# npit/video-learning-tf

Measured on AMD Instinct MI355X. Metric: clips/sec (16-frame 227x227) LRCN train step, higher is better.
Workload: dtype f32; 1 GPU; LRCN AlexNet(fc6)+LSTM(256) 16-frame 227x227x3 clips, 101 classes, UCF-101-shaped synthetic, full train step; global_batch=64, clips_per_gpu=64, frames_per_clip=16, parallelism=dp1, optimizer=sgd+clip_by_global_norm(10), init=reference (sigma 0.05), dist_world_size=1

## Files before the change

### include/vltf.h

```cpp
#ifndef VLTF_H
#define VLTF_H

#include <stddef.h>
#include <stdint.h>

#ifdef __cplusplus
extern "C" {
#endif

typedef void* vl_stream_t;
typedef struct vl_conv_desc vl_conv_desc;

typedef struct vl_step_state {
    int64_t step;
    float lr;
    uint32_t tag_origin;
    float adam_lr;
    uint32_t reserved[3];
} vl_step_state;

const char* vl_last_error(void);
int vl_version(void);
int vl_device_count(void);

int vl_input_prep_u8(const uint8_t* src, float* dst, int n, int raw_h, int raw_w, int out_h, int out_w,
                     const int32_t* crop_y, const int32_t* crop_x, const uint8_t* mirror,
                     const float* mean_bgr, int dst_halo, int dst_phase, vl_stream_t stream);
int vl_nhwc_to_nchw(const float* src, float* dst, int n, int h, int w, int c, int dst_halo, int dst_phase, vl_stream_t stream);
int vl_nchw_to_nhwc(const float* src, float* dst, int n, int c, int h, int w, vl_stream_t stream);

int vl_conv_create(vl_conv_desc** out, int cin, int h, int w, int cout, int kh, int kw, int stride, int groups);
void vl_conv_destroy(vl_conv_desc* d);
int vl_conv_out_hw(const vl_conv_desc* d, int* oh, int* ow);
int vl_conv_set_halo(vl_conv_desc* d, int x_halo, int y_halo, int dy_halo, int dx_halo);
int vl_conv_set_x_phase_split(vl_conv_desc* d, int on);
int vl_conv_x_phase(const vl_conv_desc* d);
int vl_set_conv_math(int math);
int vl_conv_math(void);
int vl_conv_fwd(const vl_conv_desc* d, const float* x, const float* w_hwio, const float* bias, float* y,
                int n, int relu, vl_stream_t stream);
int vl_conv_wt_transpose(const vl_conv_desc* d, const float* w_hwio, float* wt, vl_stream_t stream);
int vl_conv_dgrad(const vl_conv_desc* d, const float* dy, const float* wt, float* dx, const float* relu_mask,
                  int n, vl_stream_t stream);
size_t vl_conv_wgrad_ws_bytes(const vl_conv_desc* d, int n);
int vl_conv_wgrad_fuses_bias(const vl_conv_desc* d);
int vl_conv_wgrad(const vl_conv_desc* d, const float* x, const float* dy, float* dw, float* db, void* ws,
                  size_t ws_bytes, int n, vl_stream_t stream);
size_t vl_c8_bytes(int n, int c, int h, int w, int halo);
int vl_pack_c8(const float* x, void* xb, int n, int c, int h, int w, int x_halo, int xb_halo, vl_stream_t stream);
size_t vl_conv_c8_w_bytes(const vl_conv_desc* d, int bwd);
int vl_conv_c8_pack_w(const vl_conv_desc* d, const float* w_hwio, void* wb, int bwd, vl_stream_t stream);
int vl_conv_c8_fwd(vl_conv_desc* d, const void* xb, const void* wb, const float* bias, float* y, void* yb, int n, int relu,
                   vl_stream_t stream);
int vl_conv_c8_dgrad(vl_conv_desc* d, const void* dyb, const void* wbt, float* dx, void* dxb, const float* relu_mask,
                     const void* relu_mask_c8, int n, vl_stream_t stream);
size_t vl_conv_c8_wgrad_ws_bytes(const vl_conv_desc* d, int n);
int vl_conv_c8_wgrad(vl_conv_desc* d, const void* xb, const void* dyb, float* dw, void* ws, size_t ws_bytes, int n,
                     vl_stream_t stream);
int vl_bias_grad_c8(const void* dyb, float* db, float* ws, int n, int c, int h, int w, int halo, vl_stream_t stream);
int vl_pack_kc8(const float* src, void* dst, int64_t positions, int channels, int64_t pos_stride, int64_t ch_stride, vl_stream_t stream);
size_t vl_gemm_kc8_ws_bytes(int m, int n, int k);
int vl_gemm_kc8(const void* a_kc8, const void* b_kc8, float* c, int m, int n, int k, const float* bias, int relu, void* ws,
                size_t ws_bytes, vl_stream_t stream);
int vl_s2d_c8_from_x0(const vl_conv_desc* d, const float* x0, void* xb, int n, vl_stream_t stream);
int vl_input_prep_u8_s2d(const vl_conv_desc* d, const uint8_t* src, void* xb, int n, int raw_h, int raw_w, const int32_t* crop_y,
                         const int32_t* crop_x, const uint8_t* mirror, const float* mean_bgr, vl_stream_t stream);
int vl_s2d_weights(const vl_conv_desc* d, const float* src, float* dst, int grad, vl_stream_t stream);
int vl_bias_grad_nchw(const float* dy, float* db, float* ws, int n, int c, int hw, vl_stream_t stream);

int vl_lrn_fwd(const float* x, float* y, int n, int c, int hw, int radius, float alpha, float beta, float bias,
               vl_stream_t stream);
int vl_lrn_bwd(const float* x, const float* dy, float* dx, int n, int c, int hw, int radius, float alpha,
               float beta, float bias, int relu_fused, int w, int dx_halo, vl_stream_t stream);

int vl_pool_lrn_bwd(const float* x, const float* dp, const uint8_t* argmax, float* dx, int n, int c, int h, int w,
                    int p_halo, int radius, float alpha, float beta, float bias, int relu_fused, int dx_halo,
                    vl_stream_t stream);

int vl_pool_lrn_bwd_c8(const void* x, int x_packed, const float* dp, const uint8_t* argmax, void* dxb, int n, int c, int h, int w,
                       int p_halo, int radius, float alpha, float beta, float bias, int relu_fused, int dxb_halo, vl_stream_t stream);

int vl_pool_lrn_bwd_test_ranges(int ranges);

int vl_lrn_pool_fwd(const float* x, float* p, uint8_t* argmax, int n, int c, int h, int w, int p_halo, int radius,
                    float alpha, float beta, float bias, vl_stream_t stream);

int vl_lrn_pool_fwd_c8(const void* x, int x_packed, void* pb, uint8_t* argmax, int n, int c, int h, int w, int p_halo, int radius,
                       float alpha, float beta, float bias, vl_stream_t stream);

int vl_maxpool_fwd(const float* x, float* y, uint8_t* argmax, int n, int c, int h, int w, int k, int s,
                   int64_t ys_n, int64_t ys_c, int64_t ys_h, int64_t ys_w, vl_stream_t stream);
int vl_maxpool_bwd(const float* dy, const uint8_t* argmax, float* dx, const float* relu_mask, int n, int c,
                   int h, int w, int k, int s, int64_t ys_n, int64_t ys_c, int64_t ys_h, int64_t ys_w,
                   int dx_halo, vl_stream_t stream);

int vl_gemm(int transa, int transb, int m, int n, int k, const float* a, int64_t lda, const float* b, int64_t ldb,
            float* c, int64_t ldc, const float* bias, int relu, const float* relu_mask, void* ws, size_t ws_bytes,
            vl_stream_t stream);
size_t vl_gemm_split_ws_bytes(int m, int n, int k);
int vl_colsum(const float* a, int64_t lda, float* out, float* ws, int m, int n, vl_stream_t stream);

int vl_lstm_step_fwd(const float* gx, const float* gh, float* act, float* cseq, float* hseq, float* hprev,
                     int batch, int T, int t, int H, float forget_bias, vl_stream_t stream);
int vl_lstm_step_bwd(const float* dout, const float* dh_next, const float* act, const float* cseq, float* dc,
                     float* dz, int batch, int T, int t, int H, vl_stream_t stream);

size_t vl_lstm_seq_ws_bytes(int batch, int T, int H);
int vl_lstm_seq_fwd(const float* gx, const float* kh, const float* h0, const float* c0, float* act, float* cseq, float* hseq,
                    float* hprev, int batch, int T, int H, float forget_bias, void* ws, size_t ws_bytes, vl_stream_t stream);
int vl_lstm_seq_bwd(const float* dout, const float* kh, const float* act, const float* cseq, const float* c0, float* dz,
                    float* dh0, float* dc0, int batch, int T, int H, void* ws, size_t ws_bytes, vl_stream_t stream);
int vl_lstm_seq_fwd_len(const float* gx, const float* kh, const float* h0, const float* c0, float* act, float* cseq, float* hseq,
                        float* hprev, int batch, int T, int H, float forget_bias, const int32_t* seq_len, void* ws, size_t ws_bytes,
                        vl_stream_t stream);
int vl_lstm_seq_bwd_len(const float* dout, const float* kh, const float* act, const float* cseq, const float* c0, float* dz,
                        float* dh0, float* dc0, int batch, int T, int H, const int32_t* seq_len, void* ws, size_t ws_bytes,
                        vl_stream_t stream);
size_t vl_lstm_seq_tag_span(int batch, int T, int H);
int vl_lstm_seq_fwd_st(const float* gx, const float* kh, const float* h0, const float* c0, float* act, float* cseq, float* hseq,
                       float* hprev, int batch, int T, int H, float forget_bias, void* ws, size_t ws_bytes, const vl_step_state* state,
                       uint32_t tag_offset, vl_stream_t stream);
int vl_lstm_seq_bwd_st(const float* dout, const float* kh, const float* act, const float* cseq, const float* c0, float* dz,
                       float* dh0, float* dc0, int batch, int T, int H, void* ws, size_t ws_bytes, const vl_step_state* state,
                       uint32_t tag_offset, vl_stream_t stream);
int vl_lstm_seq_ws_clear(void* ws, size_t ws_bytes, vl_stream_t stream);
int vl_lstm_seq_status(void* ws, int* timed_out);
int vl_lstm_seq_test_hooks(unsigned spin_limit, int mute_workgroup);
int vl_transpose(const float* src, int64_t ld, float* dst, int rows, int cols, vl_stream_t stream);

int vl_temporal_fusion_fwd(const float* x, float* y, int batch, int T, int H, int method, vl_stream_t stream);
int vl_temporal_fusion_bwd(const float* dy, float* dx, int batch, int T, int H, int method, vl_stream_t stream);
int vl_temporal_fusion_fwd_len(const float* x, float* y, int batch, int T, int H, int method, const int32_t* seq_len,
                               vl_stream_t stream);
int vl_temporal_fusion_bwd_len(const float* dy, float* dx, int batch, int T, int H, int method, const int32_t* seq_len,
                               vl_stream_t stream);

typedef struct vl_resize_desc vl_resize_desc;
int vl_resize_create(vl_resize_desc** out, int h, int w, int oh, int ow, int channels);
void vl_resize_destroy(vl_resize_desc* d);
size_t vl_resize_tmp_bytes(const vl_resize_desc* d, int n);
int vl_resize_u8(const vl_resize_desc* d, const uint8_t* src, uint8_t* tmp, uint8_t* dst, int n, vl_stream_t stream);

int vl_copy2d(const float* src, int64_t src_ld, float* dst, int64_t dst_ld, int rows, int cols, vl_stream_t stream);
int vl_eltwise2(const float* a, const float* b, float* out, int64_t count, int op, vl_stream_t stream);
int vl_max2_grad(const float* a, const float* b, const float* d, float* da, float* db, int64_t count, vl_stream_t stream);
int vl_fuse_n(const float* const* ins, int n, float* out, int64_t count, int op, vl_stream_t stream);
int vl_fuse_n_grad(const float* const* ins, int n, const float* d, float* const* dins, int64_t count, int op, vl_stream_t stream);

int vl_dropout_fwd(const float* x, float* y, uint8_t* mask, int64_t count, float keep, uint64_t seed, vl_stream_t stream);
int vl_dropout_bwd(const float* dy, const uint8_t* mask, float* dx, int64_t count, float keep, vl_stream_t stream);
int vl_dropout_fwd_st(const float* x, float* y, uint8_t* mask, int64_t count, float keep, const vl_step_state* state,
                      vl_stream_t stream);

int vl_softmax_xent(const float* logits, const int32_t* labels, float* dlogits, float* stats, float* rows,
                    int batch, int classes, float grad_scale, vl_stream_t stream);
int vl_softmax_xent_len(const float* logits, const int32_t* labels, float* dlogits, float* stats, float* rows,
                        int batch, int classes, float grad_scale, const int32_t* seq_len, int T, vl_stream_t stream);

int vl_sumsq(const float* g, int64_t count, float* out, float* ws, int accumulate, vl_stream_t stream);
int vl_sgd_apply(float* w, const float* g, int64_t count, float lr, float clip_norm, const float* sumsq,
                 float gscale, const uint32_t* skip, vl_stream_t stream);
int vl_adam_apply(float* w, const float* g, float* m, float* v, int64_t count, float lr, float clip_norm,
                  const float* sumsq, float gscale, int step, const uint32_t* skip, vl_stream_t stream);
int vl_status_or(uint32_t* dst, const void* lstm_ws, int init, vl_stream_t stream);

size_t vl_step_state_bytes(void);
int vl_step_state_set(vl_step_state* state, int64_t step, float lr, uint32_t tag_origin, vl_stream_t stream);
int vl_sgd_apply_st(float* w, const float* g, int64_t count, const vl_step_state* state, float clip_norm, const float* sumsq,
                    float gscale, const uint32_t* skip, vl_stream_t stream);
int vl_adam_apply_st(float* w, const float* g, float* m, float* v, int64_t count, const vl_step_state* state, float clip_norm,
                     const float* sumsq, float gscale, const uint32_t* skip, vl_stream_t stream);

int vl_fill(float* p, int64_t count, float value, vl_stream_t stream);
int vl_relu_grad(float* d, const float* y, int64_t count, vl_stream_t stream);

#ifdef __cplusplus
}
#endif
#endif
```

### video-learning-tf_amd/_ffi.py

```python
import ctypes as C
import os

_HERE = os.path.dirname(os.path.abspath(__file__))
LIB_PATH = os.environ.get("VLTF_HIP_LIB") or os.path.join(_HERE, "libvltf_hip.so")

p = C.c_void_p
i32, i64, f32, u32, u64, sz = C.c_int, C.c_int64, C.c_float, C.c_uint32, C.c_uint64, C.c_size_t

SIGNATURES = {
    "vl_last_error": (C.c_char_p, []),
    "vl_version": (i32, []),
    "vl_device_count": (i32, []),
    "vl_input_prep_u8": (i32, [p, p, i32, i32, i32, i32, i32, p, p, p, p, i32, i32, p]),
    "vl_nhwc_to_nchw": (i32, [p, p, i32, i32, i32, i32, i32, i32, p]),
    "vl_nchw_to_nhwc": (i32, [p, p, i32, i32, i32, i32, p]),
    "vl_conv_create": (i32, [C.POINTER(p), i32, i32, i32, i32, i32, i32, i32, i32]),
    "vl_conv_destroy": (None, [p]),
    "vl_conv_out_hw": (i32, [p, C.POINTER(i32), C.POINTER(i32)]),
    "vl_conv_set_halo": (i32, [p, i32, i32, i32, i32]),
    "vl_conv_set_x_phase_split": (i32, [p, i32]),
    "vl_conv_x_phase": (i32, [p]),
    "vl_set_conv_math": (i32, [i32]),
    "vl_conv_math": (i32, []),
    "vl_gemm_split_ws_bytes": (C.c_size_t, [i32, i32, i32]),
    "vl_conv_fwd": (i32, [p, p, p, p, p, i32, i32, p]),
    "vl_conv_wt_transpose": (i32, [p, p, p, p]),
    "vl_conv_dgrad": (i32, [p, p, p, p, p, i32, p]),
    "vl_conv_wgrad_ws_bytes": (sz, [p, i32]),
    "vl_conv_wgrad_fuses_bias": (i32, [p]),
    "vl_conv_wgrad": (i32, [p, p, p, p, p, p, sz, i32, p]),
    "vl_c8_bytes": (sz, [i32, i32, i32, i32, i32]),
    "vl_pack_c8": (i32, [p, p, i32, i32, i32, i32, i32, i32, p]),
    "vl_conv_c8_w_bytes": (sz, [p, i32]),
    "vl_conv_c8_pack_w": (i32, [p, p, p, i32, p]),
    "vl_conv_c8_fwd": (i32, [p, p, p, p, p, p, i32, i32, p]),
    "vl_conv_c8_dgrad": (i32, [p, p, p, p, p, p, p, i32, p]),
    "vl_pack_kc8": (i32, [p, p, i64, i32, i64, i64, p]),
    "vl_gemm_kc8_ws_bytes": (sz, [i32, i32, i32]),
    "vl_gemm_kc8": (i32, [p, p, p, i32, i32, i32, p, i32, p, sz, p]),
    "vl_s2d_c8_from_x0": (i32, [p, p, p, i32, p]),
    "vl_input_prep_u8_s2d": (i32, [p, p, p, i32, i32, i32, p, p, p, p, p]),
    "vl_s2d_weights": (i32, [p, p, p, i32, p]),
    "vl_bias_grad_c8": (i32, [p, p, p, i32, i32, i32, i32, i32, p]),
    "vl_conv_c8_wgrad_ws_bytes": (sz, [p, i32]),
    "vl_conv_c8_wgrad": (i32, [p, p, p, p, p, sz, i32, p]),
    "vl_bias_grad_nchw": (i32, [p, p, p, i32, i32, i32, p]),
    "vl_lrn_fwd": (i32, [p, p, i32, i32, i32, i32, f32, f32, f32, p]),
    "vl_lrn_bwd": (i32, [p, p, p, i32, i32, i32, i32, f32, f32, f32, i32, i32, i32, p]),
    "vl_lrn_pool_fwd": (i32, [p, p, p, i32, i32, i32, i32, i32, i32, f32, f32, f32, p]),
    "vl_pool_lrn_bwd": (i32, [p, p, p, p, i32, i32, i32, i32, i32, i32, f32, f32, f32, i32, i32, p]),
    "vl_pool_lrn_bwd_test_ranges": (i32, [i32]),
    "vl_lrn_pool_fwd_c8": (i32, [p, i32, p, p, i32, i32, i32, i32, i32, i32, f32, f32, f32, p]),
    "vl_pool_lrn_bwd_c8": (i32, [p, i32, p, p, p, i32, i32, i32, i32, i32, i32, f32, f32, f32, i32, i32, p]),
    "vl_maxpool_fwd": (i32, [p, p, p, i32, i32, i32, i32, i32, i32, i64, i64, i64, i64, p]),
    "vl_maxpool_bwd": (i32, [p, p, p, p, i32, i32, i32, i32, i32, i32, i64, i64, i64, i64, i32, p]),
    "vl_gemm": (i32, [i32, i32, i32, i32, i32, p, i64, p, i64, p, i64, p, i32, p, p, sz, p]),
    "vl_colsum": (i32, [p, i64, p, p, i32, i32, p]),
    "vl_lstm_step_fwd": (i32, [p, p, p, p, p, p, i32, i32, i32, i32, f32, p]),
    "vl_lstm_step_bwd": (i32, [p, p, p, p, p, p, i32, i32, i32, i32, p]),
    "vl_lstm_seq_ws_bytes": (sz, [i32, i32, i32]),
    "vl_lstm_seq_fwd": (i32, [p, p, p, p, p, p, p, p, i32, i32, i32, f32, p, sz, p]),
    "vl_lstm_seq_bwd": (i32, [p, p, p, p, p, p, p, p, i32, i32, i32, p, sz, p]),
    "vl_lstm_seq_fwd_len": (i32, [p, p, p, p, p, p, p, p, i32, i32, i32, f32, p, p, sz, p]),
    "vl_lstm_seq_bwd_len": (i32, [p, p, p, p, p, p, p, p, i32, i32, i32, p, p, sz, p]),
    "vl_lstm_seq_tag_span": (sz, [i32, i32, i32]),
    "vl_lstm_seq_fwd_st": (i32, [p, p, p, p, p, p, p, p, i32, i32, i32, f32, p, sz, p, u32, p]),
    "vl_lstm_seq_bwd_st": (i32, [p, p, p, p, p, p, p, p, i32, i32, i32, p, sz, p, u32, p]),
    "vl_lstm_seq_ws_clear": (i32, [p, sz, p]),
    "vl_lstm_seq_status": (i32, [p, C.POINTER(i32)]),
    "vl_lstm_seq_test_hooks": (i32, [C.c_uint, i32]),
    "vl_transpose": (i32, [p, i64, p, i32, i32, p]),
    "vl_temporal_fusion_fwd": (i32, [p, p, i32, i32, i32, i32, p]),
    "vl_temporal_fusion_bwd": (i32, [p, p, i32, i32, i32, i32, p]),
    "vl_temporal_fusion_fwd_len": (i32, [p, p, i32, i32, i32, i32, p, p]),
    "vl_temporal_fusion_bwd_len": (i32, [p, p, i32, i32, i32, i32, p, p]),
    "vl_dropout_fwd": (i32, [p, p, p, i64, f32, u64, p]),
    "vl_dropout_bwd": (i32, [p, p, p, i64, f32, p]),
    "vl_dropout_fwd_st": (i32, [p, p, p, i64, f32, p, p]),
    "vl_softmax_xent": (i32, [p, p, p, p, p, i32, i32, f32, p]),
    "vl_softmax_xent_len": (i32, [p, p, p, p, p, i32, i32, f32, p, i32, p]),
    "vl_sumsq": (i32, [p, i64, p, p, i32, p]),
    "vl_sgd_apply": (i32, [p, p, i64, f32, f32, p, f32, p, p]),
    "vl_adam_apply": (i32, [p, p, p, p, i64, f32, f32, p, f32, i32, p, p]),
    "vl_status_or": (i32, [p, p, i32, p]),
    "vl_step_state_bytes": (sz, []),
    "vl_step_state_set": (i32, [p, i64, f32, u32, p]),
    "vl_sgd_apply_st": (i32, [p, p, i64, p, f32, p, f32, p, p]),
    "vl_adam_apply_st": (i32, [p, p, p, p, i64, p, f32, p, f32, p, p]),
    "vl_fill": (i32, [p, i64, f32, p]),
    "vl_resize_create": (i32, [C.POINTER(p), i32, i32, i32, i32, i32]),
    "vl_resize_destroy": (None, [p]),
    "vl_resize_tmp_bytes": (sz, [p, i32]),
    "vl_resize_u8": (i32, [p, p, p, p, i32, p]),
    "vl_copy2d": (i32, [p, i64, p, i64, i32, i32, p]),
    "vl_eltwise2": (i32, [p, p, p, i64, i32, p]),
    "vl_max2_grad": (i32, [p, p, p, p, p, i64, p]),
    "vl_fuse_n": (i32, [p, i32, p, i64, i32, p]),
    "vl_fuse_n_grad": (i32, [p, i32, p, p, i64, i32, p]),
    "vl_relu_grad": (i32, [p, p, i64, p]),
}


class VltfError(RuntimeError):
    pass


_lib = None


def lib():
    global _lib
    if _lib is None:
        if not os.path.exists(LIB_PATH):
            raise VltfError("libvltf_hip.so not found at %s -- build it with "
                            "`python -c 'import __graft_entry__ as g; g.build()'` "
                            "(there is no CPU fallback)" % LIB_PATH)
        import torch
        tl = os.path.join(os.path.dirname(torch.__file__), "lib", "libamdhip64.so")
        if os.path.exists(tl):
            C.CDLL(tl, mode=C.RTLD_GLOBAL)
        try:
            l = C.CDLL(LIB_PATH)
        except OSError as ex:
            raise VltfError("cannot load %s: %s" % (LIB_PATH, ex))
        for name, (res, args) in SIGNATURES.items():
            try:
                fn = getattr(l, name)
            except AttributeError:
                raise VltfError("libvltf_hip.so does not export %s (stale build?)" % name)
            fn.restype = res
            fn.argtypes = args
        _lib = l
    return _lib


def check(rc, what):
    if rc != 0:
        msg = lib().vl_last_error()
        raise VltfError("%s failed (rc=%d): %s" % (what, rc, msg.decode() if msg else "?"))


def call(name, *args):
    check(getattr(lib(), name)(*args), name)
```

### video-learning-tf_amd/csrc/conv_desc.h

```cpp
#pragma once
#include <hip/hip_runtime.h>
#include <stdint.h>

struct vl_conv_desc {
    int cin, h, w, cout, kh, kw, stride, groups;
    int oh, ow, pt, pl, pb, pr;
    int cig, cog;
    int K;
    int Kd;
    int x_halo, y_halo, dy_halo, dx_halo;
    int x_phase;
    int2* ktab2_fwd;
    int* ktab_fwd;
    int2* ptab2_fwd;
    int2* ptab2_bwd;
    int* ptab_fwd;
    int* ptab_bwd;
    int* rowtab_fwd;
    int* rowtab_bwd;
    int fwd_padded, bwd_padded;
    uint32_t* wsplit_fwd;
    uint32_t* wsplit_bwd;
    int* c8_toff_fwd;
    int* c8_toff_bwd;
};

void conv_c8_free_tables(vl_conv_desc* d);
int conv_c8_build_tables(vl_conv_desc* d);
```

### video-learning-tf_amd/csrc/mfma_gemm.hip

```cpp
#include <stdlib.h>
#include <string.h>

#include "common.h"
#include "conv_desc.h"

typedef float f32x16 __attribute__((ext_vector_type(16)));
typedef const __attribute__((address_space(4))) int* const_int_ptr;
__device__ __forceinline__ const_int_ptr as_const(const int* p) { return (const_int_ptr)(uintptr_t)p; }
static constexpr int NT = 256;
static constexpr int KBLK = 16;

static constexpr uint32_t OOB_OFF = 0xF0000000u;
static constexpr int64_t MAX_BUF_BYTES = 0xE0000000ll;

__device__ __forceinline__ __amdgpu_buffer_rsrc_t make_rsrc(const float* base, int64_t bytes) {
    return __builtin_amdgcn_make_buffer_rsrc(const_cast<float*>(base), 0, (int)(uint32_t)bytes, 0x00020000);
}
__device__ __forceinline__ float buf_load(__amdgpu_buffer_rsrc_t r, uint32_t voff, int soff) {
    return __builtin_bit_cast(float, __builtin_amdgcn_raw_buffer_load_b32(r, (int)voff, soff, 0));
}

template <int BX, int BR>
struct LdsTile {
    static constexpr int STR = BR + 2;
// ... 567 lines not shown
    i32x4 p[3];
};
template <int NPC>
__device__ __forceinline__ void split_pieces(float x0, float x1, int (&out)[3]) {
    f32x2 r = {x0, x1};
#pragma unroll
    for (int k = 0; k < NPC; ++k) {
        const uint32_t h = __builtin_bit_cast(uint32_t, __builtin_convertvector(r, bf16x2));
        out[k] = (int)h;
        if (k + 1 < NPC) r = f32x2{r[0] - __uint_as_float(h << 16), r[1] - __uint_as_float(h & 0xffff0000u)};
    }
}
__device__ constexpr int kProdA[6] = {0, 0, 1, 1, 0, 2};
__device__ constexpr int kProdB[6] = {0, 1, 0, 1, 2, 0};
constexpr int split_products(int math) { return math == 6 ? 6 : math == 3 ? 3 : 1; }
constexpr int split_pieces_of(int math) { return math == 6 ? 3 : math == 3 ? 2 : 1; }
__device__ __forceinline__ f32x16 mfma_bf16(const i32x4& a, const i32x4& b, const f32x16& c) {
    return __builtin_amdgcn_mfma_f32_32x32x16_bf16(__builtin_bit_cast(bf16x8, a), __builtin_bit_cast(bf16x8, b), c, 0, 0, 0);
}

template <int BN, int WM, int WN, int MATH = 0, bool X4 = false>
__global__ __launch_bounds__(NT, 1) void wgrad_dma_kernel(const ConvGeom g, const DyParams d, const EpiRowMajor::Params pe,
                                                          int tiles_i, int tiles_j, int groups, int units, int rtiles,
                                                          int rt_per_split, float* db_slabs, int db_stride) {
    using C = WgradDmaCfg<BN>;
    constexpr int BM = C::BM, STR = C::STR, SA = BM * STR, BUF = C::BUF;
    constexpr int TM = BM / WM / 32, TN = BN / WN / 32;
    constexpr int RA = BM / 4, RB = BN / 4;
    static_assert(WM * WN == 4 && TM * WM * 32 == BM && TN * WN * 32 == BN, "tile shape");
    static_assert(RA + RB <= 10 * 2 * TM * TN, "row fetches must leave the last third of a tile's MFMAs to cover their latency");
    static_assert(!X4 || (MATH != 0 && BN == 128 && BM == 128), "the 16-byte fetch form: split-product modes, 128 x 128 tiles");
    constexpr int GSTR = 258, SA4 = 32 * GSTR, BUF4 = 64 * GSTR;
    extern __shared__ __attribute__((aligned(16))) float ldsw[];

    const int tiles = tiles_i * tiles_j;
    const int k8 = blockIdx.x >> 3;
    const int unit = (k8 / tiles) * 8 + (blockIdx.x & 7);
    if (unit >= units) return;
    const int tile_id = k8 % tiles;
    const int ti_blk = tile_id % tiles_i, tj_blk = tile_id / tiles_i;
    const int zg = unit % groups, zs = unit / groups;
    const int i0 = ti_blk * BM, j0 = tj_blk * BN;
    const int lane = threadIdx.x & 63;
    const int wave = __builtin_amdgcn_readfirstlane(threadIdx.x >> 6);
    const int wi0 = (wave / WN) * (BM / WM), wj0 = (wave % WN) * (BN / WN);

    const i32x4 rs_x = rsrc_words(g.x + (int64_t)zg * g.grp_stride, (g.total - (int64_t)zg * g.grp_stride) * 4);
    const int64_t goff = (int64_t)zg * d.Cog * d.plane;
    const i32x4 rs_dy = rsrc_words(d.dy + goff, (d.total - goff) * 4);
    const int* tab = g.ktab + i0 + wave * RA;
    const uint32_t lds0 = (uint32_t)(uintptr_t)(__attribute__((address_space(3))) float*)ldsw;
    const int row_bytes = (int)(d.plane * 4);
    const int b_row0 = j0 + wave * RB;
    const int b_last = d.Cog - 1;
    const int64_t dy_img = (int64_t)d.Cout_total * d.plane;

    uint32_t voff_x, voff_dy;
    auto decode = [&](int rt) __attribute__((always_inline)) {
        const int m = X4 ? rt * 64 + 4 * (lane & 15) : rt * 64 + lane;
        const bool vm = m < g.M;
        const uint32_t mm = vm ? m : 0;
        const uint32_t n = fd_div(mm, g.dOHW);
        const uint32_t p = mm - n * g.OHW;
        const uint32_t oh = fd_div(p, g.dOW);
        const uint32_t ow = p - oh * g.OW;
        const int ih0 = (int)oh * g.stride - g.pt + g.halo, iw0 = (int)ow * g.col_mul + g.col_add;
        const uint32_t vx = (uint32_t)((int64_t)n * g.img_stride + (int64_t)ih0 * g.Wp + iw0) * 4u;
        const uint32_t vd = (uint32_t)((int64_t)n * dy_img + (int64_t)(oh + d.halo) * d.OWp + ow + d.halo) * 4u;
        voff_x = vm ? vx : OOB_OFF;
        voff_dy = vm ? vd : OOB_OFF;
        asm volatile("" : "+v"(voff_x), "+v"(voff_dy));
    };
    int tabv[RA];
    auto load_table = [&](int rt) __attribute__((always_inline)) {
        const const_int_ptr tt = (const_int_ptr)(uintptr_t)(tab + rt * g.zero);
#pragma unroll
        for (int f = 0; f < RA; ++f) tabv[f] = tt[f];
    };
    auto pin_table = [&]() __attribute__((always_inline)) {
#pragma unroll
        for (int f = 0; f < RA; ++f) asm volatile("" : "+s"(tabv[f]));
    };
    auto dma = [&](const int nb, const int f, int rt_next) __attribute__((always_inline)) {
        const int z = rt_next * g.zero;
        if (f < RA) {
            const uint32_t la = lds0 + (uint32_t)(wave * (RA * STR) + z) * 4u;
            lds_dma_row(rs_x, la + (uint32_t)(nb * BUF + f * STR) * 4u, voff_x, tabv[f]);
        } else {
            const int r = f - RA;
            const uint32_t lb = lds0 + (uint32_t)(SA + wave * (RB * STR) + z) * 4u;
            lds_dma_row(rs_dy, lb + (uint32_t)(nb * BUF + r * STR) * 4u, voff_dy, min(b_row0 + z + r, b_last) * row_bytes);
        }
    };
    uint32_t vrow_a[8], vrow_b[8];
    if constexpr (X4) {
#pragma unroll
        for (int j = 0; j < 8; ++j) {
            const int rl = wave * 8 + j + 32 * (lane >> 4);
            vrow_a[j] = i0 + rl < g.K ? (uint32_t)g.ktab[i0 + rl] : OOB_OFF;
            vrow_b[j] = j0 + rl < d.Cog ? (uint32_t)(j0 + rl) * (uint32_t)row_bytes : OOB_OFF;
        }
    }
    auto dma_x4 = [&](const int nb, const int f, int rt_next) __attribute__((always_inline)) {
        const int z = rt_next * g.zero;
        if (f < 8) {
            const uint32_t vo = (vrow_a[f] == OOB_OFF || voff_x == OOB_OFF) ? OOB_OFF : vrow_a[f] + voff_x;
            lds_dma_row4(rs_x, lds0 + (uint32_t)(nb * BUF4 + (wave * 8 + f) * GSTR + z) * 4u, vo, 0);
        } else {
            const uint32_t vo = (vrow_b[f - 8] == OOB_OFF || voff_dy == OOB_OFF) ? OOB_OFF : vrow_b[f - 8] + voff_dy;
            lds_dma_row4(rs_dy, lds0 + (uint32_t)(nb * BUF4 + SA4 + (wave * 8 + f - 8) * GSTR + z) * 4u, vo, 0);
        }
    };
    const int ones_row = (db_slabs != nullptr && g.K >= i0 && g.K < i0 + BM) ? g.K - i0 : -1;
    auto finish_tile = [&](const int nb) __attribute__((always_inline)) {
        asm volatile("s_waitcnt vmcnt(0)" ::: "memory");
        if constexpr (X4) {
            if (ones_row >= 0 && ((ones_row & 31) >> 3) == wave) ldsw[nb * BUF4 + (ones_row & 31) * GSTR + (ones_row >> 5) * 64 + lane] = 1.0f;
        } else {
            if (ones_row >= 0 && (ones_row / RA) == wave) ldsw[nb * BUF + ones_row * STR + lane] = 1.0f;
        }
        __syncthreads();
    };

    f32x16 acc[TM][TN];
#pragma unroll
    for (int a = 0; a < TM; ++a)
#pragma unroll
        for (int b = 0; b < TN; ++b)
#pragma unroll
            for (int q = 0; q < 16; ++q) acc[a][b][q] = 0.f;

    const int rt0 = zs * rt_per_split;
    const int rt1 = min(rtiles, rt0 + rt_per_split);
    const int ntiles = rt1 - rt0;
    if (ntiles > 0) {
        decode(rt0);
        load_table(rt0);
        pin_table();
        if constexpr (X4) {
#pragma unroll
            for (int f = 0; f < 16; ++f) dma_x4(0, f, rt0);
        } else {
#pragma unroll
            for (int f = 0; f < RA + RB; ++f) dma(0, f, rt0);
        }
        decode(rt0 + 1);
        finish_tile(0);
    }
    const float* fa = ldsw + (wi0 + (lane & 31)) * STR + 2 * (lane >> 5);
    const float* fb = ldsw + SA + (wj0 + (lane & 31)) * STR + 2 * (lane >> 5);

    auto tile = [&](const int cur, int rt_next) __attribute__((always_inline)) {
        float2 af[2][TM], bf[2][TN];
#pragma unroll
        for (int a = 0; a < TM; ++a) af[0][a] = *reinterpret_cast<const float2*>(fa + cur * BUF + a * 32 * STR);
#pragma unroll
        for (int b = 0; b < TN; ++b) bf[0][b] = *reinterpret_cast<const float2*>(fb + cur * BUF + b * 32 * STR);
#pragma unroll
        for (int t = 0; t < 16; ++t) {
            const int c = t & 1, nx = c ^ 1;
            if (t + 1 < 16) {
#pragma unroll
                for (int a = 0; a < TM; ++a) af[nx][a] = *reinterpret_cast<const float2*>(fa + cur * BUF + a * 32 * STR + 4 * (t + 1));
#pragma unroll
                for (int b = 0; b < TN; ++b) bf[nx][b] = *reinterpret_cast<const float2*>(fb + cur * BUF + b * 32 * STR + 4 * (t + 1));
            }
#pragma unroll
            for (int m = 0; m < 2 * TM * TN; ++m) {
                const int a = (m % (TM * TN)) / TN, b = m % TN;
                if (m < TM * TN) acc[a][b] = __builtin_amdgcn_mfma_f32_32x32x2f32(af[c][a].x, bf[c][b].x, acc[a][b], 0, 0, 0);
                else acc[a][b] = __builtin_amdgcn_mfma_f32_32x32x2f32(af[c][a].y, bf[c][b].y, acc[a][b], 0, 0, 0);
                const int f = t * (2 * TM * TN) + m;
                if (f < RA + RB) {
                    dma(cur ^ 1, f, rt_next);
                    __builtin_amdgcn_sched_barrier(0);
                }
            }
            if (t == 10) {
                load_table(rt_next + 1);
                __builtin_amdgcn_sched_barrier(0);
            }
            if (t == 13) {
                int rtn = rt_next + 1;
                asm volatile("" : "+s"(rtn));
                decode(rtn);
                pin_table();
                __builtin_amdgcn_sched_barrier(0);
            }
        }
        finish_tile(cur ^ 1);
    };
    const float* fa3 = ldsw + (wi0 + (lane & 31)) * STR + 8 * (lane >> 5);
    const float* fb3 = ldsw + SA + (wj0 + (lane & 31)) * STR + 8 * (lane >> 5);
    auto tile_split = [&](const int cur, int rt_next) __attribute__((always_inline)) {
        constexpr int NP = split_products(MATH), NPC = split_pieces_of(MATH);
        constexpr int NMS = NP * TM * TN, NTOT = 4 * NMS, NF = X4 ? 16 : RA + RB;
        constexpr int FSPAN = NTOT >= 28 ? NTOT - 14 : NTOT / 2;
        constexpr int FPM = (NF + FSPAN - 1) / FSPAN, FEND = (NF + FPM - 1) / FPM;
        constexpr int LT = FEND > NTOT - 12 ? FEND : NTOT - 12;
        constexpr int PIN = LT + 2 > NTOT - 6 ? LT + 2 : NTOT - 6;
        static_assert(PIN < NTOT, "the tile must leave room to load and pin the next table");
        SplitBf16 As[2][TM], Bs[2][TN];
        auto load_split = [&](const int st, SplitBf16 (&A)[TM], SplitBf16 (&B)[TN]) __attribute__((always_inline)) {
#pragma unroll
            for (int a = 0; a < TM; ++a)
#pragma unroll
                for (int q = 0; q < 4; ++q) {
                    const float2 v = X4 ? *reinterpret_cast<const float2*>(ldsw + cur * BUF4 + (lane & 31) * GSTR + (wi0 / 32 + a) * 64 + 16 * st +
                                                                            8 * (lane >> 5) + 2 * q)
                                        : *reinterpret_cast<const float2*>(fa3 + cur * BUF + a * 32 * STR + 16 * st + 2 * q);
                    int pc[3] = {0, 0, 0};
                    split_pieces<NPC>(v.x, v.y, pc);
#pragma unroll
                    for (int k = 0; k < NPC; ++k) A[a].p[k][q] = pc[k];
                }
#pragma unroll
            for (int b = 0; b < TN; ++b)
#pragma unroll
                for (int q = 0; q < 4; ++q) {
                    const float2 v = X4 ? *reinterpret_cast<const float2*>(ldsw + cur * BUF4 + SA4 + (lane & 31) * GSTR + (wj0 / 32 + b) * 64 +
                                                                            16 * st + 8 * (lane >> 5) + 2 * q)
                                        : *reinterpret_cast<const float2*>(fb3 + cur * BUF + b * 32 * STR + 16 * st + 2 * q);
                    int pc[3] = {0, 0, 0};
                    split_pieces<NPC>(v.x, v.y, pc);
#pragma unroll
                    for (int k = 0; k < NPC; ++k) B[b].p[k][q] = pc[k];
                }
        };
        load_split(0, As[0], Bs[0]);
        static_for<0, 4>([&](auto SI) __attribute__((always_inline)) {
            constexpr int st = decltype(SI)::value, c = st & 1;
            if constexpr (st + 1 < 4) load_split(st + 1, As[c ^ 1], Bs[c ^ 1]);
            static_for<0, NMS>([&](auto MI) __attribute__((always_inline)) {
                constexpr int m = decltype(MI)::value;
                constexpr int prod = m / (TM * TN), a = (m % (TM * TN)) / TN, b = m % TN;
                acc[a][b] = mfma_bf16(As[c][a].p[kProdA[prod]], Bs[c][b].p[kProdB[prod]], acc[a][b]);
                constexpr int idx = st * NMS + m;
                static_for<0, FPM>([&](auto EI) __attribute__((always_inline)) {
                    constexpr int f = idx * FPM + decltype(EI)::value;
                    if constexpr (f < NF) {
                        if constexpr (X4) dma_x4(cur ^ 1, f, rt_next);
                        else dma(cur ^ 1, f, rt_next);
                    }
                });
                __builtin_amdgcn_sched_barrier(0x106);
                if constexpr (idx == LT) load_table(rt_next + 1);
                if constexpr (idx == PIN) {
                    int rtn = rt_next + 1;
                    asm volatile("" : "+s"(rtn));
                    decode(rtn);
                    pin_table();
                }
            });
        });
        finish_tile(cur ^ 1);
    };
    auto run_tile = [&](const int cur, int rt_next) __attribute__((always_inline)) {
        if constexpr (MATH != 0) tile_split(cur, rt_next);
        else tile(cur, rt_next);
    };
    int rt = rt0;
    for (int i = 0; i + 1 < ntiles; i += 2, rt += 2) {
        run_tile(0, rt + 1);
        run_tile(1, rt + 2);
    }
    if (ntiles > 0 && (ntiles & 1)) run_tile(0, rt + 1);

    EpiRowMajor::template apply<TM, TN>(pe, zg, zs, i0 + wi0, j0 + wj0, acc);
    if (ones_row >= 0) {
        float* dbs = db_slabs + (int64_t)zs * db_stride + zg * d.Cog;
        const int lr = ones_row - wi0;
        if (lr >= 0 && lr < BM / WM) {
            const int a = lr >> 5, rr = lr & 31;
            const int q = (rr & 3) + 4 * (rr >> 3);
            if (((rr >> 2) & 1) == (lane >> 5)) {
#pragma unroll
                for (int b = 0; b < TN; ++b) {
                    const int j = j0 + wj0 + 32 * b + (lane & 31);
                    float v = 0.f;
#pragma unroll
                    for (int aa = 0; aa < TM; ++aa)
#pragma unroll
                        for (int qq = 0; qq < 16; ++qq)
                            if (aa == a && qq == q) v = acc[aa][b][qq];
                    if (j < d.Cog) dbs[j] = v;
                }
            }
        }
    }
}

typedef float f32x4 __attribute__((ext_vector_type(4)));
typedef float f32x4u __attribute__((ext_vector_type(4), aligned(4)));

struct ConvDmaParams {
    const float* w;
    int64_t w_ld;
    int64_t w_grp_stride;
    int64_t w_bytes;
    const int* row_tab;
    int nblk;
};

template <int SR>
__global__ __launch_bounds__(NT, 64 / SR) void conv_dma_kernel(const ConvDmaParams pa, const ConvGeom g, const EpiConvNCHW::Params pe,
                                                               int tiles_i, int wide) {
    constexpr int BM = 128, BN = 128;
    constexpr int ABUF = SR * BM, BUF = SR * (BM + BN);
    constexpr int RW = SR / 4;
    constexpr int NF = RW * 4;
    constexpr int NT2 = SR / 4;
    constexpr int FPM = 1;
    static_assert(SR == 64 || SR == 32, "stage depth");
    extern __shared__ __attribute__((aligned(16))) float ldsc[];
    const int bid = xcd_swizzle(blockIdx.x, gridDim.x);
    const int ti_blk = bid % tiles_i, tj_blk = bid / tiles_i;
    const int zg = blockIdx.y;
    const int i0 = ti_blk * BM, j0 = tj_blk * BN;
    const int lane = threadIdx.x & 63;
    const int wave = __builtin_amdgcn_readfirstlane(threadIdx.x >> 6);
    const int wm = wave >> 1, wn = wave & 1;

    const i32x4 rs_w = rsrc_words(pa.w + (int64_t)zg * pa.w_grp_stride, pa.w_bytes - (int64_t)zg * pa.w_grp_stride * 4);
    const i32x4 rs_x = rsrc_words(g.x + (int64_t)zg * g.grp_stride, (g.total - (int64_t)zg * g.grp_stride) * 4);
    uint32_t voff_a[2], voff_b[2];
#pragma unroll
    for (int hf = 0; hf < 2; ++hf) {
        const int co = i0 + hf * 64 + lane;
        voff_a[hf] = co < pe.Cog ? (uint32_t)co * 4u : OOB_OFF;
        const int m = j0 + hf * 64 + lane;
        const bool vm = m < g.M;
        const uint32_t mm = vm ? m : 0;
        const uint32_t n = fd_div(mm, g.dOHW);
        const uint32_t p = mm - n * g.OHW;
        const uint32_t oh = fd_div(p, g.dOW);
        const uint32_t ow = p - oh * g.OW;
        const int ih0 = (int)oh * g.stride - g.pt + g.halo, iw0 = (int)ow * g.col_mul + g.col_add;
        voff_b[hf] = vm ? (uint32_t)((int64_t)n * g.img_stride + (int64_t)ih0 * g.Wp + iw0) * 4u : OOB_OFF;
    }
    const uint32_t lds0 = (uint32_t)(uintptr_t)(__attribute__((address_space(3))) float*)ldsc;
    const int ld_bytes = (int)(pa.w_ld * 4);

    int tabv[RW];
    int row0 = 0;
    bool blk_ok = false;
    const int wrow = wave * RW;
    auto load_table = [&](int st) {
        const int k0 = st * SR + wrow;
        const const_int_ptr tt = as_const(g.ktab) + k0 + st * g.zero;
#pragma unroll
        for (int f = 0; f < RW; ++f) tabv[f] = tt[f];
        row0 = as_const(pa.row_tab)[k0 / KBLK + st * g.zero] + k0 % KBLK;
        blk_ok = k0 / KBLK < pa.nblk;
    };
    auto pin_table = [&]() {
#pragma unroll
        for (int f = 0; f < RW; ++f) asm volatile("" : "+s"(tabv[f]));
        asm volatile("" : "+s"(row0));
    };
    auto dma = [&](const int nb, const int f, int st) {
        const int rr = f >> 2, kind = f & 3, hf = kind & 1;
        const int z = st * g.zero;
        const uint32_t row_lds = lds0 + (uint32_t)(nb * BUF + (wrow + rr) * 128 + hf * 64 + z) * 4u;
        const bool live = blk_ok && st * SR + wrow + rr < g.K;
        if (kind < 2) lds_dma_row(rs_w, row_lds, voff_a[hf], min(row0 + rr, g.K - 1) * ld_bytes);
        else lds_dma_row(rs_x, row_lds + ABUF * 4u, live ? voff_b[hf] : OOB_OFF, tabv[rr]);
    };
    int a_soff = 0;
    auto dma_fast = [&](const int nb, const int f, int st) {
        const int rr = f >> 2, kind = f & 3, hf = kind & 1;
        const uint32_t row_lds = lds0 + (uint32_t)(nb * BUF + (wrow + rr) * 128 + hf * 64 + st * g.zero) * 4u;
        if (f == 0) a_soff = row0 * ld_bytes;
        if (kind < 2) lds_dma_row(rs_w, row_lds, voff_a[hf], a_soff);
        else lds_dma_row(rs_x, row_lds + ABUF * 4u, voff_b[hf], tabv[rr]);
        if (kind == 1) a_soff += ld_bytes;
    };
    auto finish_stage = [&]() {
        asm volatile("s_waitcnt vmcnt(0)" ::: "memory");
        __syncthreads();
    };

    f32x16 acc[2][2];
#pragma unroll
    for (int a = 0; a < 2; ++a)
#pragma unroll
        for (int b = 0; b < 2; ++b)
#pragma unroll
            for (int q = 0; q < 16; ++q) acc[a][b][q] = 0.f;

    const int nstages = (pa.nblk * KBLK + SR - 1) / SR;
    load_table(0);
    pin_table();
#pragma unroll
    for (int f = 0; f < NF; ++f) dma(0, f, 0);
    load_table(1);
    pin_table();
    finish_stage();

    float bias_r[2][16];
#pragma unroll
    for (int a = 0; a < 2; ++a)
#pragma unroll
        for (int q = 0; q < 16; ++q) {
            const int co = i0 + wm * 64 + 2 * ((q & 3) + 8 * (q >> 2) + 4 * (lane >> 5)) + a;
            bias_r[a][q] = (pe.bias && co < pe.Cog) ? pe.bias[zg * pe.Cog + co] : 0.f;
        }

    const float* fa = ldsc + (lane >> 5) * 128 + wm * 64 + 2 * (lane & 31);
    const float* fb = ldsc + ABUF + (lane >> 5) * 128 + wn * 64 + (lane & 31);

    auto stage = [&](const int cur, const bool fast, int st_next) {
        float2 af[2], bf[2], an[2], bn[2];
        auto read_b = [&](int step) {
            const float* q = fb + cur * BUF + step * 256;
            return float2{q[0], q[32]};
        };
        af[0] = *reinterpret_cast<const float2*>(fa + cur * BUF);
        bf[0] = read_b(0);
        af[1] = *reinterpret_cast<const float2*>(fa + cur * BUF + 256);
        bf[1] = read_b(1);
#pragma unroll
        for (int t = 0; t < NT2; ++t) {
            if (t + 1 < NT2) {
#pragma unroll
                for (int u = 0; u < 2; ++u) {
                    an[u] = *reinterpret_cast<const float2*>(fa + cur * BUF + (2 * (t + 1) + u) * 256);
                    bn[u] = read_b(2 * (t + 1) + u);
                }
            }
#pragma unroll
            for (int m = 0; m < 8; ++m) {
                const int u = m >> 2, a = (m >> 1) & 1, b = m & 1;
                acc[a][b] = __builtin_amdgcn_mfma_f32_32x32x2f32(a ? af[u].y : af[u].x, b ? bf[u].y : bf[u].x, acc[a][b], 0, 0, 0);
                const int f = (t * 8 + m) * FPM;
                if (f < NF) {
#pragma unroll
                    for (int e = 0; e < FPM; ++e) {
                        if (fast) dma_fast(cur ^ 1, f + e, st_next);
                        else dma(cur ^ 1, f + e, st_next);
                    }
                    __builtin_amdgcn_sched_barrier(0);
                }
            }
            static_assert(NF / FPM / 8 <= NT2 - 4, "fetches must end before the table is replaced");
            if (t == NT2 - 4) {
                load_table(st_next + 1);
                __builtin_amdgcn_sched_barrier(0);
            }
            if (t == NT2 - 2) {
                pin_table();
                __builtin_amdgcn_sched_barrier(0);
            }
#pragma unroll
            for (int u = 0; u < 2; ++u) {
                af[u] = an[u];
                bf[u] = bn[u];
            }
        }
        finish_stage();
    };
    const int nfull = g.K / SR;
    int st = 0;
    for (; st + 2 < nfull; st += 2) {
        stage(0, true, st + 1);
        stage(1, true, st + 2);
    }
    for (; st < nstages; ++st) {
        if (st & 1) stage(1, false, st + 1);
        else stage(0, false, st + 1);
    }

    if (wide) {
        constexpr int SP = BN + 4;
        float* T = ldsc;
#pragma unroll
        for (int b = 0; b < 2; ++b)
#pragma unroll
            for (int a = 0; a < 2; ++a)
#pragma unroll
                for (int q = 0; q < 16; ++q) {
                    const int i = (q & 3) + 8 * (q >> 2) + 4 * (lane >> 5);
                    float v = acc[a][b][q] + bias_r[a][q];
                    if (pe.relu) v = fmaxf(v, 0.f);
                    T[(wm * 64 + 2 * i + a) * SP + wn * 64 + 32 * b + (lane & 31)] = v;
                }
        __syncthreads();
        const int px = 4 * (lane & 31);
        const int m = j0 + px;
        const uint32_t n = fd_div((uint32_t)min(m, pe.M - 1), pe.dOHW);
        const int p = m - (int)n * pe.OHW;
        const bool run4 = m + 3 < pe.M && p + 3 < pe.OHW;
        const int64_t cbase = ((int64_t)n * pe.Cout_total + (int64_t)zg * pe.Cog) * pe.y_plane + p;
#pragma unroll
        for (int i = 0; i < BM / 8; ++i) {
            const int cl = wave * (BM / 4) + 2 * i + (lane >> 5);
            const int co = i0 + cl;
            const f32x4 v = *reinterpret_cast<const f32x4*>(T + cl * SP + px);
            if (co >= pe.Cog) continue;
            float* dst = pe.y + cbase + (int64_t)co * pe.y_plane;
            if (run4) {
                *reinterpret_cast<f32x4u*>(dst) = v;
            } else {
#pragma unroll
                for (int e = 0; e < 4; ++e) {
                    const int me = m + e;
                    if (me < pe.M) {
                        const uint32_t ne = fd_div((uint32_t)me, pe.dOHW);
                        const int pe_ = me - (int)ne * pe.OHW;
                        pe.y[((int64_t)ne * pe.Cout_total + (int64_t)zg * pe.Cog + co) * pe.y_plane + pe_] = v[e];
                    }
                }
            }
        }
        return;
    }
#pragma unroll
    for (int b = 0; b < 2; ++b) {
        const int m = j0 + wn * 64 + 32 * b + (lane & 31);
        if (m >= pe.M) continue;
        const uint32_t n = fd_div((uint32_t)m, pe.dOHW);
        const uint32_t p = m - n * pe.OHW;
        const uint32_t oh = fd_div(p, pe.dOW);
        const uint32_t ow = p - oh * pe.OW;
        const int64_t c0 = (int64_t)n * pe.Cout_total + (int64_t)zg * pe.Cog;
        const int64_t ybase = c0 * pe.y_plane + (int64_t)(oh + pe.y_halo) * pe.y_wp + ow + pe.y_halo;
        const int64_t mbase = c0 * pe.m_plane + (int64_t)(oh + pe.m_halo) * pe.m_wp + ow + pe.m_halo;
#pragma unroll
        for (int a = 0; a < 2; ++a) {
            float mk[16];
            if (pe.mask) {
#pragma unroll
                for (int q = 0; q < 16; ++q) {
                    const int co = i0 + wm * 64 + 2 * ((q & 3) + 8 * (q >> 2) + 4 * (lane >> 5)) + a;
                    mk[q] = co < pe.Cog ? pe.mask[mbase + (int64_t)co * pe.m_plane] : 0.f;
                }
            }
#pragma unroll
            for (int q = 0; q < 16; ++q) {
                const int i = (q & 3) + 8 * (q >> 2) + 4 * (lane >> 5);
                const int co = i0 + wm * 64 + 2 * i + a;
                if (co < pe.Cog) {
                    float v = acc[a][b][q] + bias_r[a][q];
                    if (pe.relu) v = fmaxf(v, 0.f);
                    if (pe.mask) v = mk[q] > 0.f ? v : 0.f;
                    pe.y[ybase + (int64_t)co * pe.y_plane] = v;
                }
            }
        }
    }
}


__global__ void conv_wsplit_kernel(const float* __restrict__ w, int64_t w_ld, int64_t w_grp_stride, const int* __restrict__ row_tab,
                                   int K, int Cog, int CogP, int nstages, int planes, uint32_t* __restrict__ out) {
    const int st = blockIdx.x, zg = blockIdx.y;
    const int row0 = row_tab[st];
    uint32_t* o = out + ((int64_t)zg * nstages + st) * planes * 8 * CogP;
    for (int idx = threadIdx.x; idx < 8 * CogP; idx += blockDim.x) {
        const int q = idx & 3, co = (idx >> 2) % CogP, h = idx / (4 * CogP);
        const int r = 8 * h + 2 * q, p = st * 16 + r;
        float x0 = 0.f, x1 = 0.f;
        if (co < Cog) {
            const float* src = w + (int64_t)(row0 + r) * w_ld + zg * w_grp_stride + co;
            if (p < K) x0 = src[0];
            if (p + 1 < K) x1 = src[w_ld];
        }
        int pc[3] = {0, 0, 0};
        split_pieces<3>(x0, x1, pc);
        for (int k = 0; k < planes; ++k) o[(int64_t)((2 * k + h) * CogP + co) * 4 + q] = (uint32_t)pc[k];
    }
}

struct ConvRingParams {
    const uint32_t* wsplit;
    int CogP;
    int nstages;
};

template <int MATH, int BM>
__global__ __launch_bounds__(512, 1) void conv_ring_kernel(const ConvRingParams pa, const ConvGeom g, const EpiConvNCHW::Params pe,
                                                           int tiles_i, int OWp, int Mp, FastDiv dOHWp, FastDiv dOWp) {
    constexpr int BN = BM == 128 ? 256 : 512, SR = 16, NBUF = BM == 128 ? 5 : 4;
    constexpr int NH = BN / 256;
    static_assert(BM == 128 || BM == 64, "channel tile");
    constexpr int NPL = MATH == 6 ? 3 : 2;
    constexpr int ABUF = NPL * 8 * BM, BUF = ABUF + SR * BN;
    constexpr int NAF = (NPL * 2 * (BM / 64) + 7) / 8;
    constexpr int FW = NAF + 2 * NH;
    constexpr int VMW = (NBUF - 3) * FW;
    constexpr int NP = split_products(MATH), NPC = split_pieces_of(MATH);
    constexpr int NM = (BM / 32) * (BN / 256) * NP;
    static_assert(SR == KBLK, "one stage = one block of the reduction order");
    extern __shared__ __attribute__((aligned(16))) float ldsr[];
    const int bid = xcd_swizzle(blockIdx.x, gridDim.x);
    const int ti_blk = bid % tiles_i, tj_blk = bid / tiles_i;
    const int zg = blockIdx.y;
    const int i0 = ti_blk * BM, j0 = tj_blk * BN;
    const int lane = threadIdx.x & 63;
    const int wave = __builtin_amdgcn_readfirstlane(threadIdx.x >> 6);
    constexpr int TA = BM / 32, TB = BN / 8 / 32, WPX = 32 * TB;
    const int OHWp = g.OHW / g.OW * OWp;
    const int nstages = pa.nstages;

    const int64_t stage_dw = (int64_t)NPL * 8 * pa.CogP;
    const uint32_t* wbase = pa.wsplit + (int64_t)zg * nstages * stage_dw;
    const i32x4 rs_w = rsrc_words(reinterpret_cast<const float*>(wbase), nstages * stage_dw * 4);
    constexpr int NPIECE = NPL * 2 * (BM / 64);
    int piece[NAF];
    uint32_t voff_a[NAF];
#pragma unroll
    for (int e = 0; e < NAF; ++e) {
        piece[e] = e == 0 ? wave % NPIECE : 8 + (wave & 3);
        voff_a[e] = BM == 128 ? (uint32_t)(((piece[e] >> 1) * pa.CogP + i0 + (piece[e] & 1) * 64 + lane) * 16)
                              : (uint32_t)((piece[e] * pa.CogP + i0 + lane) * 16);
    }
    const int stage_bytes = (int)(stage_dw * 4);
    const i32x4 rs_x = rsrc_words(g.x + (int64_t)zg * g.grp_stride, (g.total - (int64_t)zg * g.grp_stride) * 4);
    uint32_t voff_b[NH];
#pragma unroll
    for (int hf = 0; hf < NH; ++hf) {
        const int m = j0 + 256 * hf + 4 * lane;
        const bool vm = m < Mp;
        const uint32_t mm = vm ? m : 0;
        const uint32_t n = fd_div(mm, dOHWp);
        const uint32_t p = mm - n * OHWp;
        const uint32_t oh = fd_div(p, dOWp);
        const uint32_t ow = p - oh * OWp;
        const int ih0 = (int)oh * g.stride - g.pt + g.halo, iw0 = (int)ow * g.col_mul + g.col_add;
        voff_b[hf] = vm ? (uint32_t)((int64_t)n * g.img_stride + (int64_t)ih0 * g.Wp + iw0) * 4u : OOB_OFF;
    }
    const uint32_t lds0 = (uint32_t)(uintptr_t)(__attribute__((address_space(3))) float*)ldsr;

    int tab0 = 0, tab1 = 0;
    const int wrow = wave * 2;
    auto load_table = [&](int st) __attribute__((always_inline)) {
        const int sc = min(st, nstages - 1) + st * g.zero;
        const const_int_ptr tt = as_const(g.ktab) + sc * SR + wrow;
        tab0 = tt[0];
        tab1 = tt[1];
    };
    auto pin_table = [&]() __attribute__((always_inline)) {
        asm volatile("" : "+s"(tab0));
        asm volatile("" : "+s"(tab1));
    };
    auto dma = [&](const uint32_t wr, const int f, int st) __attribute__((always_inline)) {
        if (f < NAF) {
            lds_dma_row4(rs_w, lds0 + wr + (uint32_t)piece[f] * 1024u, voff_a[f], st * stage_bytes);
        } else {
            const int r = (f - NAF) / NH, hf = (f - NAF) % NH;
            const bool live = st * SR + wrow + r < g.K;
            lds_dma_row4(rs_x, lds0 + wr + (uint32_t)(ABUF + (wrow + r) * BN + 256 * hf) * 4u, live ? voff_b[hf] : OOB_OFF,
                         r == 0 ? tab0 : tab1);
        }
    };
    auto dma_fast = [&](const uint32_t wr, const int f, int st) __attribute__((always_inline)) {
        if (f < NAF) {
            lds_dma_row4(rs_w, lds0 + wr + (uint32_t)piece[f] * 1024u, voff_a[f], st * stage_bytes);
        } else {
            const int r = (f - NAF) / NH, hf = (f - NAF) % NH;
            lds_dma_row4(rs_x, lds0 + wr + (uint32_t)(ABUF + (wrow + r) * BN + 256 * hf) * 4u, voff_b[hf], r == 0 ? tab0 : tab1);
        }
    };

    f32x16 acc[TA][TB];
#pragma unroll
    for (int a = 0; a < TA; ++a)
#pragma unroll
        for (int b = 0; b < TB; ++b)
#pragma unroll
            for (int q = 0; q < 16; ++q) acc[a][b][q] = 0.f;

    const float* fa = ldsr + ((lane >> 5) * BM + (lane & 31)) * 4;
    const float* fb = ldsr + ABUF + (lane >> 5) * 8 * BN + wave * WPX + (lane & 31);
    struct Raw {
        float b[TB][8];
    };
    auto load_raw = [&](int rd, Raw& r) __attribute__((always_inline)) {
#pragma unroll
        for (int j = 0; j < 8; ++j) {
            const float* q = fb + rd + j * BN;
#pragma unroll
            for (int b = 0; b < TB; ++b) r.b[b][j] = q[32 * b];
        }
    };
    auto load_a = [&](int rd, SplitBf16 (&A)[TA]) __attribute__((always_inline)) {
#pragma unroll
        for (int a = 0; a < TA; ++a) {
#pragma unroll
            for (int k = 0; k < NPC; ++k) A[a].p[k] = *reinterpret_cast<const i32x4*>(fa + rd + k * 2 * BM * 4 + a * 32 * 4);
        }
    };
    auto split = [&](const Raw& r, SplitBf16 (&B)[TB]) __attribute__((always_inline)) {
#pragma unroll
        for (int j = 0; j < 4; ++j)
#pragma unroll
            for (int b = 0; b < TB; ++b) {
                int pc[3] = {0, 0, 0};
                split_pieces<NPC>(r.b[b][2 * j], r.b[b][2 * j + 1], pc);
#pragma unroll
                for (int k = 0; k < NPC; ++k) B[b].p[k][j] = pc[k];
            }
    };

    for (int s0 = 0; s0 < NBUF; ++s0) {
        load_table(s0);
        pin_table();
        if (s0 < nstages) {
#pragma unroll
            for (int f = 0; f < FW; ++f) dma((uint32_t)(s0 * BUF * 4), f, s0);
        }
    }
    load_table(NBUF);
    pin_table();
    if (nstages >= NBUF) asm volatile("s_waitcnt vmcnt(%0)" ::"n"(VMW) : "memory");
    else asm volatile("s_waitcnt vmcnt(0)" ::: "memory");
    __syncthreads();
    SplitBf16 A[TA] = {}, B[TB] = {}, An[TA] = {}, Bn[TB] = {};
    Raw R0 = {}, R1 = {};
    load_a(0, A);
    load_raw(0, R0);
    load_raw(BUF, R1);
    split(R0, B);
    asm volatile("s_waitcnt lgkmcnt(0)" ::: "memory");
    __syncthreads();

    int rda = BUF, rdb = 2 * BUF;
    uint32_t wr = 0;
    constexpr int D = NBUF;
    auto stage = [&](const bool fast, int st, SplitBf16 (&Ac)[TA], SplitBf16 (&Bc)[TB], SplitBf16 (&An)[TA], SplitBf16 (&Bn)[TB],
                     const Raw& Rc, Raw& Rn) __attribute__((always_inline)) {
        load_a(rda, An);
        load_raw(rdb, Rn);
        static_for<0, (NM > FW ? NM : FW)>([&](auto MI) __attribute__((always_inline)) {
            constexpr int m = decltype(MI)::value;
            if constexpr (m < NM) {
                constexpr int prod = m / (TA * TB), a = (m % (TA * TB)) / TB, b = m % TB;
                acc[a][b] = mfma_bf16(Ac[a].p[kProdA[prod]], Bc[b].p[kProdB[prod]], acc[a][b]);
            }
            if constexpr (m < FW) {
                if (fast) dma_fast(wr, m, st + D);
                else if (st + D < nstages) dma(wr, m, st + D);
            }
            __builtin_amdgcn_sched_barrier(0x106);
        });
        split(Rc, Bn);
        load_table(st + D + 1);
        pin_table();
        rda = rda + BUF == NBUF * BUF ? 0 : rda + BUF;
        rdb = rdb + BUF == NBUF * BUF ? 0 : rdb + BUF;
        wr = wr + BUF * 4 == NBUF * BUF * 4 ? 0u : wr + BUF * 4;
    };
    auto finish = [&](int st) __attribute__((always_inline)) {
        const int after = min(st + D, nstages - 1) - (st + 3);
        if (after >= 2 && NBUF - 3 >= 2) asm volatile("s_waitcnt vmcnt(%0) lgkmcnt(0)" ::"n"(2 * FW) : "memory");
        else if (after >= 1) asm volatile("s_waitcnt vmcnt(%0) lgkmcnt(0)" ::"n"(FW) : "memory");
        else asm volatile("s_waitcnt vmcnt(0) lgkmcnt(0)" ::: "memory");
        __syncthreads();
    };
    const int nfull = g.K / SR;
    int st = 0;
    for (; st + 1 + D < nfull; st += 2) {
        stage(true, st, A, B, An, Bn, R1, R0);
        asm volatile("s_waitcnt vmcnt(%0) lgkmcnt(0)" ::"n"(VMW) : "memory");
        __syncthreads();
        stage(true, st + 1, An, Bn, A, B, R0, R1);
        asm volatile("s_waitcnt vmcnt(%0) lgkmcnt(0)" ::"n"(VMW) : "memory");
        __syncthreads();
    }
    for (; st < nstages; st += 2) {
        stage(false, st, A, B, An, Bn, R1, R0);
        finish(st);
        if (st + 1 < nstages) {
            stage(false, st + 1, An, Bn, A, B, R0, R1);
            finish(st + 1);
        }
    }

#pragma unroll
    for (int b = 0; b < TB; ++b) {
        const int m = j0 + wave * WPX + 32 * b + (lane & 31);
        if (m >= Mp) continue;
        const uint32_t n = fd_div((uint32_t)m, dOHWp);
        const uint32_t p = m - n * OHWp;
        const uint32_t oh = fd_div(p, dOWp);
        const uint32_t ow = p - oh * OWp;
        if ((int)ow >= pe.OW) continue;
        const int64_t c0 = (int64_t)n * pe.Cout_total + (int64_t)zg * pe.Cog;
        const int64_t ybase = c0 * pe.y_plane + (int64_t)(oh + pe.y_halo) * pe.y_wp + ow + pe.y_halo;
        const int64_t mbase = c0 * pe.m_plane + (int64_t)(oh + pe.m_halo) * pe.m_wp + ow + pe.m_halo;
#pragma unroll
        for (int a = 0; a < TA; ++a) {
#pragma unroll
            for (int q = 0; q < 16; ++q) {
                const int i = (q & 3) + 8 * (q >> 2) + 4 * (lane >> 5);
                const int co = i0 + 32 * a + i;
                if (co < pe.Cog) {
                    float v = acc[a][b][q];
                    if (pe.bias) v += pe.bias[zg * pe.Cog + co];
                    if (pe.relu) v = fmaxf(v, 0.f);
                    if (pe.mask) v = pe.mask[mbase + (int64_t)co * pe.m_plane] > 0.f ? v : 0.f;
                    pe.y[ybase + (int64_t)co * pe.y_plane] = v;
                }
            }
        }
    }
}

template <int MATH>
__global__ __launch_bounds__(256, 2) void conv_ring4_kernel(const ConvRingParams pa, const ConvGeom g, const EpiConvNCHW::Params pe,
                                                            int tiles_i, int OWp, int Mp, FastDiv dOHWp, FastDiv dOWp) {
    constexpr int BM = 128, BN = 256, SR = 16, NBUF = 3, D = 3;
    constexpr int ABUF = SR * BM, BUF = SR * (BM + BN);
    constexpr int TA = 4, TB = 2, WPX = 64;
    constexpr int FW = 6;
    constexpr int NP = split_products(MATH), NPC = split_pieces_of(MATH);
    static_assert(NPC <= 2, "the two-workgroup form has LDS for two weight planes");
    constexpr int NM = TA * TB * NP;
    static_assert(SR == KBLK, "one stage = one block of the reduction order");
    extern __shared__ __attribute__((aligned(16))) float ldsq[];
    const int bid = xcd_swizzle(blockIdx.x, gridDim.x);
    const int ti_blk = bid % tiles_i, tj_blk = bid / tiles_i;
    const int zg = blockIdx.y;
    const int i0 = ti_blk * BM, j0 = tj_blk * BN;
    const int lane = threadIdx.x & 63;
    const int wave = __builtin_amdgcn_readfirstlane(threadIdx.x >> 6);
    const int OHWp = g.OHW / g.OW * OWp;
    const int nstages = pa.nstages;

    const int64_t stage_dw = (int64_t)16 * pa.CogP;
    const uint32_t* wbase = pa.wsplit + (int64_t)zg * nstages * stage_dw;
    const i32x4 rs_w = rsrc_words(reinterpret_cast<const float*>(wbase), nstages * stage_dw * 4);
    uint32_t voff_a[2];
#pragma unroll
    for (int hf = 0; hf < 2; ++hf) voff_a[hf] = (uint32_t)((wave * pa.CogP + i0 + hf * 64 + lane) * 16);
    const int stage_bytes = (int)(stage_dw * 4);
    const i32x4 rs_x = rsrc_words(g.x + (int64_t)zg * g.grp_stride, (g.total - (int64_t)zg * g.grp_stride) * 4);
    uint32_t voff_b;
    {
        const int m = j0 + 4 * lane;
        const bool vm = m < Mp;
        const uint32_t mm = vm ? m : 0;
        const uint32_t n = fd_div(mm, dOHWp);
        const uint32_t p = mm - n * OHWp;
        const uint32_t oh = fd_div(p, dOWp);
        const uint32_t ow = p - oh * OWp;
        const int ih0 = (int)oh * g.stride - g.pt + g.halo, iw0 = (int)ow * g.col_mul + g.col_add;
        voff_b = vm ? (uint32_t)((int64_t)n * g.img_stride + (int64_t)ih0 * g.Wp + iw0) * 4u : OOB_OFF;
    }
    const uint32_t lds0 = (uint32_t)(uintptr_t)(__attribute__((address_space(3))) float*)ldsq;

    int tab[4] = {0, 0, 0, 0};
    const int wrow = wave * 4;
    auto load_table = [&](int st) __attribute__((always_inline)) {
        const int sc = min(st, nstages - 1) + st * g.zero;
        const const_int_ptr tt = as_const(g.ktab) + sc * SR + wrow;
#pragma unroll
        for (int r = 0; r < 4; ++r) tab[r] = tt[r];
    };
    auto pin_table = [&]() __attribute__((always_inline)) {
#pragma unroll
        for (int r = 0; r < 4; ++r) asm volatile("" : "+s"(tab[r]));
    };
    auto dma = [&](const uint32_t wr, const int f, int st, const bool fast) __attribute__((always_inline)) {
        if (f < 2) {
            lds_dma_row4(rs_w, lds0 + wr + (uint32_t)(2 * wave + f) * 1024u, voff_a[f], st * stage_bytes);
        } else {
            const int r = f - 2;
            const bool live = fast || st * SR + wrow + r < g.K;
            lds_dma_row4(rs_x, lds0 + wr + (uint32_t)(ABUF + (wrow + r) * BN) * 4u, live ? voff_b : OOB_OFF, tab[r]);
        }
    };

    f32x16 acc[TA][TB];
#pragma unroll
    for (int a = 0; a < TA; ++a)
#pragma unroll
        for (int b = 0; b < TB; ++b)
#pragma unroll
            for (int q = 0; q < 16; ++q) acc[a][b][q] = 0.f;

    const float* fa = ldsq + ((lane >> 5) * BM + (lane & 31)) * 4;
    const float* fb = ldsq + ABUF + (lane >> 5) * 8 * BN + wave * WPX + (lane & 31);
    auto load_ops = [&](int rd, SplitBf16 (&A)[TA], float (&rb)[TB][8]) __attribute__((always_inline)) {
#pragma unroll
        for (int a = 0; a < TA; ++a) {
#pragma unroll
            for (int k = 0; k < NPC; ++k) A[a].p[k] = *reinterpret_cast<const i32x4*>(fa + rd + k * 2 * BM * 4 + a * 32 * 4);
        }
#pragma unroll
        for (int j = 0; j < 8; ++j)
#pragma unroll
            for (int b = 0; b < TB; ++b) rb[b][j] = fb[rd + j * BN + 32 * b];
    };
    auto split = [&](const float (&rb)[TB][8], SplitBf16 (&B)[TB]) __attribute__((always_inline)) {
#pragma unroll
        for (int j = 0; j < 4; ++j)
#pragma unroll
            for (int b = 0; b < TB; ++b) {
                int pc[3] = {0, 0, 0};
                split_pieces<NPC>(rb[b][2 * j], rb[b][2 * j + 1], pc);
#pragma unroll
                for (int k = 0; k < NPC; ++k) B[b].p[k][j] = pc[k];
            }
    };

    for (int s0 = 0; s0 < NBUF; ++s0) {
        load_table(s0);
        pin_table();
        if (s0 < nstages) {
#pragma unroll
            for (int f = 0; f < FW; ++f) dma((uint32_t)(s0 * BUF * 4), f, s0, false);
        }
    }
    load_table(NBUF);
    pin_table();
    if (nstages >= NBUF) asm volatile("s_waitcnt vmcnt(%0)" ::"n"(2 * FW) : "memory");
    else asm volatile("s_waitcnt vmcnt(0)" ::: "memory");
    __syncthreads();
    SplitBf16 A[TA] = {}, B[TB] = {}, An[TA] = {}, Bn[TB] = {};
    {
        float rb[TB][8];
        load_ops(0, A, rb);
        split(rb, B);
    }
    if (nstages >= NBUF) asm volatile("s_waitcnt vmcnt(%0) lgkmcnt(0)" ::"n"(FW) : "memory");
    else asm volatile("s_waitcnt vmcnt(0) lgkmcnt(0)" ::: "memory");
    __syncthreads();

    int rd = BUF;
    uint32_t wr = 0;
    auto stage = [&](const bool fast, int st, SplitBf16 (&Ac)[TA], SplitBf16 (&Bc)[TB], SplitBf16 (&An)[TA], SplitBf16 (&Bn)[TB])
                     __attribute__((always_inline)) {
        float rb[TB][8];
        load_ops(rd, An, rb);
        static_assert(NM >= FW, "a fetch rides on each of the first FW MFMAs");
        static_for<0, NM>([&](auto MI) __attribute__((always_inline)) {
            constexpr int m = decltype(MI)::value;
            constexpr int prod = m / (TA * TB), a = (m % (TA * TB)) / TB, b = m % TB;
            acc[a][b] = mfma_bf16(Ac[a].p[kProdA[prod]], Bc[b].p[kProdB[prod]], acc[a][b]);
            if constexpr (m < FW) {
                if (fast || st + D < nstages) dma(wr, m, st + D, fast);
            }
            __builtin_amdgcn_sched_barrier(0x106);
        });
        split(rb, Bn);
        load_table(st + D + 1);
        pin_table();
        rd = rd + BUF == NBUF * BUF ? 0 : rd + BUF;
        wr = wr + BUF * 4 == NBUF * BUF * 4 ? 0u : wr + BUF * 4;
    };
    auto finish = [&](int st) __attribute__((always_inline)) {
        if (min(st + D, nstages - 1) - (st + 2) >= 1) asm volatile("s_waitcnt vmcnt(%0) lgkmcnt(0)" ::"n"(FW) : "memory");
        else asm volatile("s_waitcnt vmcnt(0) lgkmcnt(0)" ::: "memory");
        __syncthreads();
    };
    const int nfull = g.K / SR;
    int st = 0;
    for (; st + 1 + D < nfull; st += 2) {
        stage(true, st, A, B, An, Bn);
        asm volatile("s_waitcnt vmcnt(%0) lgkmcnt(0)" ::"n"(FW) : "memory");
        __syncthreads();
        stage(true, st + 1, An, Bn, A, B);
        asm volatile("s_waitcnt vmcnt(%0) lgkmcnt(0)" ::"n"(FW) : "memory");
        __syncthreads();
    }
    for (; st < nstages; st += 2) {
        stage(false, st, A, B, An, Bn);
        finish(st);
        if (st + 1 < nstages) {
            stage(false, st + 1, An, Bn, A, B);
            finish(st + 1);
        }
    }

#pragma unroll
    for (int b = 0; b < TB; ++b) {
        const int m = j0 + wave * WPX + 32 * b + (lane & 31);
        if (m >= Mp) continue;
        const uint32_t n = fd_div((uint32_t)m, dOHWp);
        const uint32_t p = m - n * OHWp;
        const uint32_t oh = fd_div(p, dOWp);
        const uint32_t ow = p - oh * OWp;
        if ((int)ow >= pe.OW) continue;
        const int64_t c0 = (int64_t)n * pe.Cout_total + (int64_t)zg * pe.Cog;
        const int64_t ybase = c0 * pe.y_plane + (int64_t)(oh + pe.y_halo) * pe.y_wp + ow + pe.y_halo;
        const int64_t mbase = c0 * pe.m_plane + (int64_t)(oh + pe.m_halo) * pe.m_wp + ow + pe.m_halo;
#pragma unroll
        for (int a = 0; a < TA; ++a) {
#pragma unroll
            for (int q = 0; q < 16; ++q) {
                const int i = (q & 3) + 8 * (q >> 2) + 4 * (lane >> 5);
                const int co = i0 + 32 * a + i;
                if (co < pe.Cog) {
                    float v = acc[a][b][q];
                    if (pe.bias) v += pe.bias[zg * pe.Cog + co];
                    if (pe.relu) v = fmaxf(v, 0.f);
                    if (pe.mask) v = pe.mask[mbase + (int64_t)co * pe.m_plane] > 0.f ? v : 0.f;
                    pe.y[ybase + (int64_t)co * pe.y_plane] = v;
                }
            }
        }
    }
}

template <int WAYS>
__global__ __launch_bounds__(256) void reduce_slabs_kernel(const float* __restrict__ ws, float* __restrict__ out, int64_t count, int splits,
                                                          int64_t slab_stride, const float* __restrict__ bias, int ncols, int64_t ldc,
                                                          int relu, const float* __restrict__ mask) {
    __shared__ float part[3][64];
    const int lane = threadIdx.x & 63, w = threadIdx.x >> 6;
    constexpr int EPB = WAYS == 4 ? 64 : 256;
    const int per = WAYS == 4 ? (splits + 3) >> 2 : splits;
    const int z0 = WAYS == 4 ? w * per : 0, z1 = min(splits, z0 + per);
    for (int64_t e0 = (int64_t)blockIdx.x * EPB; e0 < count; e0 += (int64_t)gridDim.x * EPB) {
        const int64_t e = e0 + (WAYS == 4 ? lane : (int)threadIdx.x);
        float s = 0.f;
        if (e < count) {
            const float* p = ws + (int64_t)z0 * slab_stride + e;
            int z = z0;
            for (; z + 4 <= z1; z += 4, p += 4 * slab_stride) {
                const float a = p[0], b = p[slab_stride], c = p[2 * slab_stride], d = p[3 * slab_stride];
                s += a; s += b; s += c; s += d;
            }
            for (; z < z1; ++z, p += slab_stride) s += p[0];
        }
        if constexpr (WAYS == 4) {
            if (w > 0) part[w - 1][lane] = s;
            __syncthreads();
            if (w == 0) s = (s + part[0][lane]) + (part[1][lane] + part[2][lane]);
        }
        if ((WAYS == 1 || w == 0) && e < count) {
            int64_t o = e;
            if (ncols > 0) {
                const int64_t row = e / ncols;
                const int col = (int)(e - row * ncols);
                if (bias) s += bias[col];
                o = row * ldc + col;
            }
            if (relu) s = fmaxf(s, 0.f);
            if (mask) s = mask[o] > 0.f ? s : 0.f;
            out[o] = s;
        }
        if constexpr (WAYS == 4) __syncthreads();
    }
}

static void launch_reduce_slabs(hipStream_t s, const float* ws, float* out, int64_t count, int splits, int64_t slab_stride, const float* bias,
                                int ncols, int64_t ldc, int relu, const float* mask) {
    static const int force = vl_exp_env("VL_REDUCE_WAYS") ? atoi(vl_exp_env("VL_REDUCE_WAYS")) : 0;
    const bool four = force ? force == 4 : (splits >= 16 && count * 4 <= (int64_t)splits * 65536);
    if (four) {
        const int blocks = (int)((count + 63) / 64 < 16384 ? (count + 63) / 64 : 16384);
        hipLaunchKernelGGL(reduce_slabs_kernel<4>, dim3(blocks), dim3(256), 0, s, ws, out, count, splits, slab_stride, bias, ncols, ldc, relu, mask);
    } else {
        const int blocks = (int)((count + 255) / 256 < 4096 ? (count + 255) / 256 : 4096);
        hipLaunchKernelGGL(reduce_slabs_kernel<1>, dim3(blocks), dim3(256), 0, s, ws, out, count, splits, slab_stride, bias, ncols, ldc, relu, mask);
    }
}

static const bool kConvStaged = vl_exp_env("VL_CONV_STAGED") != nullptr;
static const bool kGemmNoSplit = vl_exp_env("VL_GEMM_NOSPLIT") != nullptr;
static const bool kConvNoWideStore = vl_exp_env("VL_CONV_NO_WIDE_STORE") != nullptr;
static const bool kConvNoTailSplit = vl_exp_env("VL_CONV_NO_TAIL_SPLIT") != nullptr;
static const bool kConvNoLoadPick = vl_exp_env("VL_CONV_NO_LOAD_PICK") != nullptr;
static const bool kWgradDword = vl_exp_env("VL_WGRAD_DWORD") != nullptr;
static const bool kRing8 = vl_exp_env("VL_CONV_RING8") != nullptr;

static int g_conv_math = [] {
    const char* e = vl_exp_env("VL_CONV_MATH");
    return e == nullptr ? 0 : strcmp(e, "bf16x3") == 0 ? 3 : strcmp(e, "bf16x6") == 0 ? 6 : strcmp(e, "bf16") == 0 ? 1 : 0;
}();

extern "C" int vl_set_conv_math(int math) {
    VL_CHECK(math == 0 || math == 1 || math == 3 || math == 6, "vl_set_conv_math: 0 (fp32), 1 (bf16), 3 (bf16x3) or 6 (bf16x6)");
    g_conv_math = math;
    return 0;
}

extern "C" int vl_conv_math(void) { return g_conv_math; }


static void tf_same_pad(int in, int k, int s, int* out, int* before, int* after) {
    *out = (in + s - 1) / s;
    int total = (*out - 1) * s + k - in;
    if (total < 0) total = 0;
    *before = total / 2;
    *after = total - *before;
}


static void k_to_row(int k, int kh, int kw, int cg, bool permuted, int* ky, int* kx, int* c) {
    if (permuted) {
        const int cl = k % KBLK, t = k / KBLK;
        *kx = t % kw;
        *ky = (t / kw) % kh;
        *c = (t / (kw * kh)) * KBLK + cl;
    } else {
        *c = k % cg;
        *kx = (k / cg) % kw;
        *ky = k / (cg * kw);
    }
}

static void free_dev(void* p) {
    if (p) (void)hipFree(p);
}

template <class T>
static int upload(T** dev, const T* host, size_t count) {
    free_dev(*dev);
    *dev = nullptr;
    hipError_t e = hipMalloc((void**)dev, sizeof(T) * count);
    if (e == hipSuccess) e = hipMemcpy(*dev, host, sizeof(T) * count, hipMemcpyHostToDevice);
    return e == hipSuccess ? 0 : 2;
}

static int build_ktabs(int** dev1, int2** dev2, int** rowtab, int kh, int kw, int cg, int H, int W, int halo, bool permuted,
                       int phase = 1, int col_shift = 0) {
    const int K = kh * kw * cg;
    const int pad = ((K + 127) / 128) * 128 + 256;
    const int Wp = phase > 1 ? (W + 2 * halo + phase - 1) / phase : W + 2 * halo;
    const int64_t Pp = (int64_t)(H + 2 * halo) * Wp;
    const int ntiles = pad / KBLK;
    int* h1 = (int*)malloc(sizeof(int) * pad);
    int2* h2 = (int2*)malloc(sizeof(int2) * pad);
    int* h3 = (int*)malloc(sizeof(int) * ntiles);
    if (!h1 || !h2 || !h3) {
        free(h1);
        free(h2);
        free(h3);
        return 1;
    }
    for (int k = 0; k < pad; ++k) {
        if (k < K) {
            int ky, kx, c;
            k_to_row(k, kh, kw, cg, permuted, &ky, &kx, &c);
            int64_t off = ((int64_t)c * Pp + (int64_t)ky * Wp + kx) * 4;
            if (phase > 1) off = (((int64_t)c * phase + (kx + col_shift) % phase) * Pp + (int64_t)ky * Wp + (kx + col_shift) / phase) * 4;
            h1[k] = (int)off;
            h2[k].x = (int)off;
            h2[k].y = (ky << 16) | kx;
            if (k % KBLK == 0) h3[k / KBLK] = (ky * kw + kx) * cg + c;
        } else {
            h1[k] = 0;
            h2[k].x = 0;
            h2[k].y = 0x4000 << 16;
            if (k % KBLK == 0) h3[k / KBLK] = 0;
        }
    }
    int rc = upload(dev1, h1, pad);
    if (rc == 0) rc = upload(dev2, h2, pad);
    if (rc == 0 && rowtab) rc = upload(rowtab, h3, ntiles);
    free(h1);
    free(h2);
    free(h3);
    return rc;
}

static int rebuild_tables(vl_conv_desc* d) {
    d->fwd_padded = d->x_halo >= d->pt && d->x_halo >= d->pb && d->x_halo >= d->pl && d->x_halo >= d->pr;
    if (!d->fwd_padded) d->x_phase = 1;
    const int ph = d->x_phase > 1 ? d->x_phase : 1, shift = d->x_halo - d->pl;
    int rc = build_ktabs(&d->ktab_fwd, &d->ktab2_fwd, nullptr, d->kh, d->kw, d->cig, d->h, d->w, d->x_halo, false, ph, shift);
    if (rc == 0)
        rc = build_ktabs(&d->ptab_fwd, &d->ptab2_fwd, &d->rowtab_fwd, d->kh, d->kw, d->cig, d->h, d->w, d->x_halo, d->cig % KBLK == 0, ph,
                         shift);
    if (rc == 0 && d->stride == 1) {
        rc = build_ktabs(&d->ptab_bwd, &d->ptab2_bwd, &d->rowtab_bwd, d->kh, d->kw, d->cog, d->oh, d->ow, d->dy_halo, d->cog % KBLK == 0);
        const int need = (d->kh - 1 - d->pt > d->pt ? d->kh - 1 - d->pt : d->pt);
        const int needw = (d->kw - 1 - d->pl > d->pl ? d->kw - 1 - d->pl : d->pl);
        d->bwd_padded = d->dy_halo >= need && d->dy_halo >= needw;
    }
    if (rc == 0) rc = conv_c8_build_tables(d);
    return rc;
}

extern "C" int vl_conv_create(vl_conv_desc** out, int cin, int h, int w, int cout, int kh, int kw, int stride, int groups) {
    VL_CHECK(out, "vl_conv_create: null out");
    VL_CHECK(cin > 0 && cout > 0 && h > 0 && w > 0 && kh > 0 && kw > 0 && stride > 0 && groups > 0, "vl_conv_create: bad geometry");
    VL_CHECK(cin % groups == 0 && cout % groups == 0, "vl_conv_create: channels not divisible by groups");
    VL_CHECK(h < 0x4000 && w < 0x4000 && kh < 256 && kw < 256, "vl_conv_create: plane too large");
    vl_conv_desc* d = (vl_conv_desc*)calloc(1, sizeof(vl_conv_desc));
    VL_CHECK(d, "vl_conv_create: out of host memory");
    d->cin = cin; d->h = h; d->w = w; d->cout = cout; d->kh = kh; d->kw = kw; d->stride = stride; d->groups = groups;
    tf_same_pad(h, kh, stride, &d->oh, &d->pt, &d->pb);
    tf_same_pad(w, kw, stride, &d->ow, &d->pl, &d->pr);
    d->cig = cin / groups;
    d->cog = cout / groups;
    d->K = kh * kw * d->cig;
    d->Kd = kh * kw * d->cog;
    const size_t sf = (size_t)groups * ceil_div(d->K, KBLK) * 24 * (ceil_div(d->cog, 128) * 128) * 4;
    const size_t sb = (size_t)groups * ceil_div(d->Kd, KBLK) * 24 * (ceil_div(d->cig, 128) * 128) * 4;
    const bool images = sf <= (64u << 20) && sb <= (64u << 20);
    if (rebuild_tables(d) || (images && (hipMalloc((void**)&d->wsplit_fwd, sf) != hipSuccess || hipMalloc((void**)&d->wsplit_bwd, sb) != hipSuccess))) {
        vl_conv_destroy(d);
        vl_set_error("vl_conv_create: device table allocation failed");
        return 2;
    }
    *out = d;
    return 0;
}

extern "C" int vl_conv_set_halo(vl_conv_desc* d, int x_halo, int y_halo, int dy_halo, int dx_halo) {
    VL_CHECK(d, "vl_conv_set_halo: null descriptor");
    VL_CHECK(x_halo >= 0 && y_halo >= 0 && dy_halo >= 0 && dx_halo >= 0 && x_halo < 64 && y_halo < 64 && dy_halo < 64 && dx_halo < 64,
             "vl_conv_set_halo: bad halo");
    d->x_halo = x_halo; d->y_halo = y_halo; d->dy_halo = dy_halo; d->dx_halo = dx_halo;
    VL_CHECK(rebuild_tables(d) == 0, "vl_conv_set_halo: device table allocation failed");
    return 0;
}

extern "C" int vl_conv_set_x_phase_split(vl_conv_desc* d, int on) {
    VL_CHECK(d, "vl_conv_set_x_phase_split: null descriptor");
    VL_CHECK(!on || d->fwd_padded, "vl_conv_set_x_phase_split: needs the padded x layout (set the halo first)");
    d->x_phase = (on && d->stride > 1) ? d->stride : 1;
    VL_CHECK(rebuild_tables(d) == 0, "vl_conv_set_x_phase_split: device table allocation failed");
    return 0;
}

extern "C" int vl_conv_x_phase(const vl_conv_desc* d) { return d && d->x_phase > 1 ? d->x_phase : 1; }

extern "C" void vl_conv_destroy(vl_conv_desc* d) {
    if (!d) return;
    free_dev(d->ktab_fwd);
    free_dev(d->ktab2_fwd);
    free_dev(d->ptab_fwd);
    free_dev(d->ptab2_fwd);
    free_dev(d->ptab_bwd);
    free_dev(d->ptab2_bwd);
    free_dev(d->rowtab_fwd);
    free_dev(d->rowtab_bwd);
    free_dev(d->wsplit_fwd);
    free_dev(d->wsplit_bwd);
    conv_c8_free_tables(d);
    free(d);
}

extern "C" int vl_conv_out_hw(const vl_conv_desc* d, int* oh, int* ow) {
    VL_CHECK(d, "vl_conv_out_hw: null descriptor");
    if (oh) *oh = d->oh;
    if (ow) *ow = d->ow;
    return 0;
}

struct ConvOut {
    float* y;
    const float* bias;
    const float* mask;
    int relu;
    int y_halo, m_halo, OH, OW;
};

template <int BM, int WM, int WN, bool PADDED>
static int launch_conv(const ConvGeom& g, const float* w, int64_t w_ld, int w_grp_stride, const int* row_tab, int Cog,
                       int Cout_total, const ConvOut& o, hipStream_t s) {
    constexpr int BN = 128, BR = KBLK;
    using LA = ConvWeightKX<BM, BR>;
    using LB = ConvGather<BN, BR, PADDED>;
    typename LA::Params pa{w, w_ld, Cog, g.K, (int64_t)w_grp_stride, row_tab};
    EpiConvNCHW::Params pe;
    pe.y = o.y; pe.bias = o.bias; pe.mask = o.mask; pe.relu = o.relu;
    pe.Cog = Cog; pe.Cout_total = Cout_total; pe.OHW = g.OHW; pe.OW = g.OW; pe.M = g.M;
    pe.dOHW = g.dOHW; pe.dOW = g.dOW;
    pe.y_halo = o.y_halo; pe.y_wp = o.OW + 2 * o.y_halo; pe.y_plane = (int64_t)(o.OH + 2 * o.y_halo) * pe.y_wp;
    pe.m_halo = o.m_halo; pe.m_wp = o.OW + 2 * o.m_halo; pe.m_plane = (int64_t)(o.OH + 2 * o.m_halo) * pe.m_wp;
    const int tiles_i = ceil_div(Cog, BM), tiles_j = ceil_div(g.M, BN);
    const int rtiles = ceil_div(g.K, BR);
    dim3 grid(tiles_i * tiles_j, (unsigned)(Cout_total / Cog), 1);
    hipLaunchKernelGGL((mfma_contract<BM, BN, BR, WM, WN, LA, LB, EpiConvNCHW>), grid, dim3(NT), 0, s, pa, g, pe,
                       tiles_i, rtiles, rtiles);
    VL_LAUNCH_CHECK();
    return 0;
}


template <int TA>
__global__ __launch_bounds__(NT, 2) void conv_dma16_kernel(const ConvDmaParams pa, const ConvGeom g, const EpiConvNCHW::Params pe,
                                                           int tiles_i, int wide) {
    constexpr int BM = 16 * TA, BN = 128, SR = 32;
    constexpr int NA = (BM + 63) / 64;
    constexpr int SA = NA * 64 + 16, SB = 144;
    constexpr int ABUF = SR * SA, BUF = SR * (SA + SB);
    constexpr int RW = SR / 4, FPR = NA + 2, NF = RW * FPR, NSTEP = SR / 4;
    constexpr int NM = 2 * TA;
    extern __shared__ __attribute__((aligned(16))) float ldsc[];
    const int bid = xcd_swizzle(blockIdx.x, gridDim.x);
    const int ti_blk = bid % tiles_i, tj_blk = bid / tiles_i;
    const int zg = blockIdx.y;
    const int i0 = ti_blk * BM, j0 = tj_blk * BN;
    const int lane = threadIdx.x & 63;
    const int wave = __builtin_amdgcn_readfirstlane(threadIdx.x >> 6);

    const i32x4 rs_w = rsrc_words(pa.w + (int64_t)zg * pa.w_grp_stride, pa.w_bytes - (int64_t)zg * pa.w_grp_stride * 4);
    const i32x4 rs_x = rsrc_words(g.x + (int64_t)zg * g.grp_stride, (g.total - (int64_t)zg * g.grp_stride) * 4);
    uint32_t voff_a[NA];
#pragma unroll
    for (int hf = 0; hf < NA; ++hf) {
        const int cl = hf * 64 + lane;
        voff_a[hf] = (cl < BM && i0 + cl < pe.Cog) ? (uint32_t)(i0 + cl) * 4u : OOB_OFF;
    }
    uint32_t voff_b[2];
#pragma unroll
    for (int hf = 0; hf < 2; ++hf) {
        const int m = j0 + hf * 64 + lane;
        const bool vm = m < g.M;
        const uint32_t mm = vm ? m : 0;
        const uint32_t n = fd_div(mm, g.dOHW);
        const uint32_t p = mm - n * g.OHW;
        const uint32_t oh = fd_div(p, g.dOW);
        const uint32_t ow = p - oh * g.OW;
        const int ih0 = (int)oh * g.stride - g.pt + g.halo, iw0 = (int)ow * g.col_mul + g.col_add;
        voff_b[hf] = vm ? (uint32_t)((int64_t)n * g.img_stride + (int64_t)ih0 * g.Wp + iw0) * 4u : OOB_OFF;
    }
    float bias_r[TA][4];
#pragma unroll
    for (int a = 0; a < TA; ++a)
#pragma unroll
        for (int q = 0; q < 4; ++q) {
            const int co = i0 + 16 * a + 4 * (lane >> 4) + q;
            bias_r[a][q] = (pe.bias && co < pe.Cog) ? pe.bias[zg * pe.Cog + co] : 0.f;
        }
    const uint32_t lds0 = (uint32_t)(uintptr_t)(__attribute__((address_space(3))) float*)ldsc;
    const int ld_bytes = (int)(pa.w_ld * 4);

    int tabv[RW];
    int row0 = 0;
    bool blk_ok = false;
    const int wrow = wave * RW;
    auto load_table = [&](int st) {
        const int k0 = st * SR + wrow;
        const const_int_ptr tt = as_const(g.ktab) + k0 + st * g.zero;
#pragma unroll
        for (int f = 0; f < RW; ++f) tabv[f] = tt[f];
        row0 = as_const(pa.row_tab)[k0 / KBLK + st * g.zero] + k0 % KBLK;
        blk_ok = k0 / KBLK < pa.nblk;
    };
    auto pin_table = [&]() {
#pragma unroll
        for (int f = 0; f < RW; ++f) asm volatile("" : "+s"(tabv[f]));
        asm volatile("" : "+s"(row0));
    };
    auto dma = [&](const int nb, const int f, int st) {
        const int rr = f / FPR, kind = f % FPR;
        const int z = st * g.zero;
        const bool live = blk_ok && st * SR + wrow + rr < g.K;
        if (kind < NA) {
            lds_dma_row(rs_w, lds0 + (uint32_t)(nb * BUF + (wrow + rr) * SA + kind * 64 + z) * 4u, voff_a[kind],
                        min(row0 + rr, g.K - 1) * ld_bytes);
        } else {
            const int hf = kind - NA;
            lds_dma_row(rs_x, lds0 + (uint32_t)(nb * BUF + ABUF + (wrow + rr) * SB + hf * 64 + z) * 4u, live ? voff_b[hf] : OOB_OFF,
                        tabv[rr]);
        }
    };
    int a_soff = 0;
    auto dma_fast = [&](const int nb, const int f, int st) {
        const int rr = f / FPR, kind = f % FPR;
        const int z = st * g.zero;
        if (f == 0) a_soff = row0 * ld_bytes;
        if (kind < NA) {
            lds_dma_row(rs_w, lds0 + (uint32_t)(nb * BUF + (wrow + rr) * SA + kind * 64 + z) * 4u, voff_a[kind], a_soff);
        } else {
            const int hf = kind - NA;
            lds_dma_row(rs_x, lds0 + (uint32_t)(nb * BUF + ABUF + (wrow + rr) * SB + hf * 64 + z) * 4u, voff_b[hf], tabv[rr]);
        }
        if (kind == NA - 1) a_soff += ld_bytes;
    };
    auto finish_stage = [&]() {
        asm volatile("s_waitcnt vmcnt(0)" ::: "memory");
        __syncthreads();
    };

    f32x4 acc[TA][2];
#pragma unroll
    for (int a = 0; a < TA; ++a)
#pragma unroll
        for (int b = 0; b < 2; ++b)
#pragma unroll
            for (int q = 0; q < 4; ++q) acc[a][b][q] = 0.f;

    const int nstages = (pa.nblk * KBLK + SR - 1) / SR;
    load_table(0);
    pin_table();
#pragma unroll
    for (int f = 0; f < NF; ++f) dma(0, f, 0);
    load_table(1);
    pin_table();
    finish_stage();

    const float* fa = ldsc + (lane >> 4) * SA + (lane & 15);
    const float* fb = ldsc + ABUF + (lane >> 4) * SB + wave * 32 + (lane & 15);

    auto stage = [&](const int cur, const bool fast, int st_next, const int nsteps) {
        float af[2][TA], bf[2][2];
        auto read = [&](int step, float (&a)[TA], float (&b)[2]) {
            const float* pa_ = fa + cur * BUF + step * 4 * SA;
            const float* pb_ = fb + cur * BUF + step * 4 * SB;
#pragma unroll
            for (int i = 0; i < TA; ++i) a[i] = pa_[16 * i];
#pragma unroll
            for (int i = 0; i < 2; ++i) b[i] = pb_[16 * i];
        };
        read(0, af[0], bf[0]);
#pragma unroll
        for (int t = 0; t < NSTEP; ++t) {
            const int c = t & 1;
            if (t + 1 < NSTEP) read(t + 1, af[c ^ 1], bf[c ^ 1]);
            if (t < nsteps) {
#pragma unroll
                for (int m = 0; m < NM; ++m) {
                    const int a = m >> 1, b = m & 1;
                    acc[a][b] = __builtin_amdgcn_mfma_f32_16x16x4f32(af[c][a], bf[c][b], acc[a][b], 0, 0, 0);
                    const int f = t * NM + m;
                    if (f < NF) {
                        if (fast) dma_fast(cur ^ 1, f, st_next);
                        else dma(cur ^ 1, f, st_next);
                        __builtin_amdgcn_sched_barrier(0);
                    }
                }
            } else {
#pragma unroll
                for (int m = 0; m < NM; ++m) {
                    const int f = t * NM + m;
                    if (f < NF) dma(cur ^ 1, f, st_next);
                }
            }
            static_assert(NF <= NM * (NSTEP - 3), "fetches must end before the table is replaced");
            if (t == NSTEP - 3) {
                load_table(st_next + 1);
                __builtin_amdgcn_sched_barrier(0);
            }
            if (t == NSTEP - 1) {
                pin_table();
                __builtin_amdgcn_sched_barrier(0);
            }
        }
        finish_stage();
    };
    const int nfull = g.K / SR;
    const int last_steps = (g.K - (nstages - 1) * SR + 3) / 4;
    int st = 0;
    for (; st + 2 < nfull; st += 2) {
        stage(0, true, st + 1, NSTEP);
        stage(1, true, st + 2, NSTEP);
    }
    for (; st < nstages; ++st) {
        const int ns = st == nstages - 1 ? last_steps : NSTEP;
        if (st & 1) stage(1, false, st + 1, ns);
        else stage(0, false, st + 1, ns);
    }

    if (wide) {
        constexpr int SP = BN + 4;
        float* T = ldsc;
#pragma unroll
        for (int b = 0; b < 2; ++b)
#pragma unroll
            for (int a = 0; a < TA; ++a)
#pragma unroll
                for (int q = 0; q < 4; ++q) {
                    float v = acc[a][b][q] + bias_r[a][q];
                    if (pe.relu) v = fmaxf(v, 0.f);
                    T[(16 * a + 4 * (lane >> 4) + q) * SP + wave * 32 + 16 * b + (lane & 15)] = v;
                }
        __syncthreads();
        const int px = 4 * (lane & 31);
        const int m = j0 + px;
        const uint32_t n = fd_div((uint32_t)min(m, pe.M - 1), pe.dOHW);
        const int p = m - (int)n * pe.OHW;
        const bool run4 = m + 3 < pe.M && p + 3 < pe.OHW;
        const int64_t cbase = ((int64_t)n * pe.Cout_total + (int64_t)zg * pe.Cog) * pe.y_plane + p;
#pragma unroll
        for (int i = 0; i < BM / 8; ++i) {
            const int cl = wave * (BM / 4) + 2 * i + (lane >> 5);
            const int co = i0 + cl;
            const f32x4 v = *reinterpret_cast<const f32x4*>(T + cl * SP + px);
            if (co >= pe.Cog) continue;
            float* dst = pe.y + cbase + (int64_t)co * pe.y_plane;
            if (run4) {
                *reinterpret_cast<f32x4u*>(dst) = v;
            } else {
#pragma unroll
                for (int e = 0; e < 4; ++e) {
                    const int me = m + e;
                    if (me < pe.M) {
                        const uint32_t ne = fd_div((uint32_t)me, pe.dOHW);
                        const int pe_ = me - (int)ne * pe.OHW;
                        pe.y[((int64_t)ne * pe.Cout_total + (int64_t)zg * pe.Cog + co) * pe.y_plane + pe_] = v[e];
                    }
                }
            }
        }
        return;
    }
#pragma unroll
    for (int b = 0; b < 2; ++b) {
        const int m = j0 + wave * 32 + 16 * b + (lane & 15);
        if (m >= pe.M) continue;
        const uint32_t n = fd_div((uint32_t)m, pe.dOHW);
        const uint32_t p = m - n * pe.OHW;
        const uint32_t oh = fd_div(p, pe.dOW);
        const uint32_t ow = p - oh * pe.OW;
        const int64_t c0 = (int64_t)n * pe.Cout_total + (int64_t)zg * pe.Cog;
        const int64_t ybase = c0 * pe.y_plane + (int64_t)(oh + pe.y_halo) * pe.y_wp + ow + pe.y_halo;
        const int64_t mbase = c0 * pe.m_plane + (int64_t)(oh + pe.m_halo) * pe.m_wp + ow + pe.m_halo;
        float mk[TA][4];
        if (pe.mask) {
#pragma unroll
            for (int a = 0; a < TA; ++a)
#pragma unroll
                for (int q = 0; q < 4; ++q) {
                    const int co = i0 + 16 * a + 4 * (lane >> 4) + q;
                    mk[a][q] = co < pe.Cog ? pe.mask[mbase + (int64_t)co * pe.m_plane] : 0.f;
                }
        }
#pragma unroll
        for (int a = 0; a < TA; ++a) {
#pragma unroll
            for (int q = 0; q < 4; ++q) {
                const int co = i0 + 16 * a + 4 * (lane >> 4) + q;
                if (co < pe.Cog) {
                    float v = acc[a][b][q] + bias_r[a][q];
                    if (pe.relu) v = fmaxf(v, 0.f);
                    if (pe.mask) v = mk[a][q] > 0.f ? v : 0.f;
                    pe.y[ybase + (int64_t)co * pe.y_plane] = v;
                }
            }
        }
    }
}


static int device_cus();

template <int BM>
static int launch_conv_dma(const ConvGeom& g, const float* w, int64_t w_ld, int w_grp_stride, const int* row_tab, int Cog,
                           int Cout_total, const ConvOut& o, hipStream_t s) {
    constexpr int BN = 128, SR = 32;
    constexpr size_t lds = BM == 128 ? (size_t)BM * (BN + 4) * sizeof(float)
                                     : (size_t)2 * SR * ((BM + 63) / 64 * 64 + 16 + 144) * sizeof(float);
    static_assert(BM != 128 || (size_t)2 * SR * (BM + BN) * sizeof(float) <= (size_t)BM * (BN + 4) * sizeof(float), "stage buffers fit");
    ConvDmaParams pa{w, w_ld, (int64_t)w_grp_stride, (int64_t)g.K * w_ld * 4, row_tab, ceil_div(g.K, KBLK)};
    EpiConvNCHW::Params pe;
    pe.y = o.y; pe.bias = o.bias; pe.mask = o.mask; pe.relu = o.relu;
    pe.Cog = Cog; pe.Cout_total = Cout_total; pe.OHW = g.OHW; pe.OW = g.OW; pe.M = g.M;
    pe.dOHW = g.dOHW; pe.dOW = g.dOW;
    pe.y_halo = o.y_halo; pe.y_wp = o.OW + 2 * o.y_halo; pe.y_plane = (int64_t)(o.OH + 2 * o.y_halo) * pe.y_wp;
    pe.m_halo = o.m_halo; pe.m_wp = o.OW + 2 * o.m_halo; pe.m_plane = (int64_t)(o.OH + 2 * o.m_halo) * pe.m_wp;
    static bool attr_set = false;
    if (!attr_set) {
        const void* kern;
        if constexpr (BM == 128) kern = reinterpret_cast<const void*>(conv_dma_kernel<SR>);
        else kern = reinterpret_cast<const void*>(conv_dma16_kernel<BM / 16>);
        VL_HIP(hipFuncSetAttribute(kern, hipFuncAttributeMaxDynamicSharedMemorySize, (int)lds));
        attr_set = true;
    }
    const int tiles_i = ceil_div(Cog, BM), tiles_j = ceil_div(g.M, BN);
    dim3 grid(tiles_i * tiles_j, (unsigned)(Cout_total / Cog), 1);
    const int wide = (o.y_halo == 0 && !o.mask && !kConvNoWideStore && (size_t)BM * (BN + 4) * sizeof(float) <= lds) ? 1 : 0;
    if constexpr (BM == 128) {
        hipLaunchKernelGGL(conv_dma_kernel<SR>, grid, dim3(NT), lds, s, pa, g, pe, tiles_i, wide);
    } else {
        hipLaunchKernelGGL((conv_dma16_kernel<BM / 16>), grid, dim3(NT), lds, s, pa, g, pe, tiles_i, wide);
    }
    VL_LAUNCH_CHECK();
    return 0;
}

template <int BM>
static int launch_conv_ring(const ConvGeom& g, const float* w, int64_t w_ld, int w_grp_stride, const int* row_tab, int Cog,
                            int Cout_total, const ConvOut& o, uint32_t* wsplit, hipStream_t s) {
    constexpr int BN = BM == 128 ? 256 : 512;
    const int math = g_conv_math, planes = math == 6 ? 3 : 2;
    const int groups = Cout_total / Cog, nstages = ceil_div(g.K, KBLK), CogP = ceil_div(Cog, BM) * BM;
    hipLaunchKernelGGL(conv_wsplit_kernel, dim3(nstages, groups), dim3(256), 0, s, w, w_ld, (int64_t)w_grp_stride, row_tab, g.K, Cog,
                       CogP, nstages, planes, wsplit);
    VL_LAUNCH_CHECK();
    ConvRingParams pa{wsplit, CogP, nstages};
    EpiConvNCHW::Params pe;
    pe.y = o.y; pe.bias = o.bias; pe.mask = o.mask; pe.relu = o.relu;
    pe.Cog = Cog; pe.Cout_total = Cout_total; pe.OHW = g.OHW; pe.OW = g.OW; pe.M = g.M;
    pe.dOHW = g.dOHW; pe.dOW = g.dOW;
    pe.y_halo = o.y_halo; pe.y_wp = o.OW + 2 * o.y_halo; pe.y_plane = (int64_t)(o.OH + 2 * o.y_halo) * pe.y_wp;
    pe.m_halo = o.m_halo; pe.m_wp = o.OW + 2 * o.m_halo; pe.m_plane = (int64_t)(o.OH + 2 * o.m_halo) * pe.m_wp;
    const int OH = g.OHW / g.OW, OWp = (g.OW + 3) / 4 * 4, Mp = g.M / g.OW * OWp;
    const int tiles_i = ceil_div(Cog, BM), tiles_j = ceil_div(Mp, BN);
    dim3 grid(tiles_i * tiles_j, (unsigned)groups, 1);
    if (BM == 128 && math != 6 && !kRing8) {
        constexpr size_t lds4 = (size_t)3 * 16 * (128 + 256) * sizeof(float);
        static bool attr4[2] = {false, false};
        const int v4 = math == 3;
        auto k4 = v4 ? conv_ring4_kernel<3> : conv_ring4_kernel<1>;
        if (!attr4[v4]) {
            VL_HIP(hipFuncSetAttribute(reinterpret_cast<const void*>(k4), hipFuncAttributeMaxDynamicSharedMemorySize, (int)lds4));
            attr4[v4] = true;
        }
        hipLaunchKernelGGL(k4, grid, dim3(256), lds4, s, pa, g, pe, tiles_i, OWp, Mp, make_fastdiv(OH * OWp), make_fastdiv(OWp));
        VL_LAUNCH_CHECK();
        return 0;
    }
    const size_t lds = (size_t)(BM == 128 ? 5 : 4) * (planes * 8 * BM + 16 * BN) * sizeof(float);
    static bool attr_set[3] = {false, false, false};
    const int v8 = math == 6 ? 2 : math == 3 ? 1 : 0;
    auto kern = v8 == 2 ? conv_ring_kernel<6, BM> : v8 == 1 ? conv_ring_kernel<3, BM> : conv_ring_kernel<1, BM>;
    if (!attr_set[v8]) {
        VL_HIP(hipFuncSetAttribute(reinterpret_cast<const void*>(kern), hipFuncAttributeMaxDynamicSharedMemorySize, (int)lds));
        attr_set[v8] = true;
    }
    hipLaunchKernelGGL(kern, grid, dim3(512), lds, s, pa, g, pe, tiles_i, OWp, Mp, make_fastdiv(OH * OWp), make_fastdiv(OWp));
    VL_LAUNCH_CHECK();
    return 0;
}

template <bool PADDED>
static int dispatch_conv(const ConvGeom& g, const float* w, int64_t w_ld, int w_grp_stride, const int* row_tab, int Cog,
                         int Cout_total, const ConvOut& o, uint32_t* wsplit, hipStream_t s) {
    const int w128 = ceil_div(Cog, 128) * 128, w96 = ceil_div(Cog, 96) * 96, w64 = ceil_div(Cog, 64) * 64;
    if (g_conv_math != 0 && PADDED && g.col_mul == 1 && wsplit != nullptr) {
        if (Cog >= 96) return launch_conv_ring<128>(g, w, w_ld, w_grp_stride, row_tab, Cog, Cout_total, o, wsplit, s);
        if (Cog >= 40 && Cog <= 64) return launch_conv_ring<64>(g, w, w_ld, w_grp_stride, row_tab, Cog, Cout_total, o, wsplit, s);
    }
    const int64_t px = ceil_div(g.M, 128), cus = device_cus(), ngrp = Cout_total / Cog;
    const bool few = px * ceil_div(Cog, 128) * ngrp < 8 * cus;
    if (PADDED && few && (int64_t)g.K * w_ld * 4 < MAX_BUF_BYTES && !kConvStaged && !kConvNoLoadPick) {
        const int widths[3] = {128, 96, 48};
        auto pick = [&](int64_t pxt, int64_t& load) {
            int b = 0;
            for (int i = 0; i < 3; ++i) {
                const int64_t l = ceil_div(pxt * ceil_div(Cog, widths[i]) * ngrp, cus) * widths[i];
                if (i == 0 || l < load) { b = i; load = l; }
            }
            return b;
        };
        auto run = [&](int wi, const ConvGeom& gg, const ConvOut& oo) {
            if (wi == 0) return launch_conv_dma<128>(gg, w, w_ld, w_grp_stride, row_tab, Cog, Cout_total, oo, s);
            if (wi == 1) return launch_conv_dma<96>(gg, w, w_ld, w_grp_stride, row_tab, Cog, Cout_total, oo, s);
            return launch_conv_dma<48>(gg, w, w_ld, w_grp_stride, row_tab, Cog, Cout_total, oo, s);
        };
        int64_t best_load = 0;
        const int best = pick(px, best_load);
        const int nimg = g.M / g.OHW;
        const int64_t wgs_per_px = (int64_t)ceil_div(Cog, widths[best]) * ngrp;
        const int64_t rounds = px * wgs_per_px / cus;
        if (rounds >= 6 && !kConvNoTailSplit) {
            const int64_t px_a = rounds * cus / wgs_per_px;
            const int n_a = (int)(px_a * 128 / g.OHW);
            const int n_b = nimg - n_a;
            if (n_a > 0 && n_b > 0) {
                int64_t load_b = 0;
                const int64_t px_b = ceil_div((int64_t)n_b * g.OHW, 128);
                const int wb = pick(px_b, load_b);
                const int64_t load_a = ceil_div(ceil_div((int64_t)n_a * g.OHW, 128) * wgs_per_px, cus) * widths[best];
                if ((load_a + (load_b > 64 ? load_b : 64) + 16) * 100 <= best_load * 95) {
                    ConvGeom ga = g, gb = g;
                    ga.M = n_a * g.OHW; ga.total = g.img_stride * n_a;
                    gb.x = g.x + (int64_t)n_a * g.img_stride; gb.M = n_b * g.OHW; gb.total = g.img_stride * n_b;
                    ConvOut ob = o;
                    ob.y = o.y + (int64_t)n_a * Cout_total * (o.OH + 2 * o.y_halo) * (o.OW + 2 * o.y_halo);
                    if (o.mask) ob.mask = o.mask + (int64_t)n_a * Cout_total * (o.OH + 2 * o.m_halo) * (o.OW + 2 * o.m_halo);
                    if (int rc = run(best, ga, o)) return rc;
                    return run(wb, gb, ob);
                }
            }
        }
        return run(best, g, o);
    }
    if (w128 <= w96 && w128 <= w64) {
        if (PADDED && (int64_t)g.K * w_ld * 4 < MAX_BUF_BYTES && !kConvStaged) {
            return launch_conv_dma<128>(g, w, w_ld, w_grp_stride, row_tab, Cog, Cout_total, o, s);
        }
        return launch_conv<128, 2, 2, PADDED>(g, w, w_ld, w_grp_stride, row_tab, Cog, Cout_total, o, s);
    }
    if (PADDED && ceil_div(Cog, 48) * 48 < w64 && ceil_div(Cog, 48) * 48 < w96 &&
        (int64_t)g.K * w_ld * 4 < MAX_BUF_BYTES && !kConvStaged)
        return launch_conv_dma<48>(g, w, w_ld, w_grp_stride, row_tab, Cog, Cout_total, o, s);
    if (w96 <= w64) {
        if (PADDED && (int64_t)g.K * w_ld * 4 < MAX_BUF_BYTES && !kConvStaged)
            return launch_conv_dma<96>(g, w, w_ld, w_grp_stride, row_tab, Cog, Cout_total, o, s);
        return launch_conv<96, 1, 4, PADDED>(g, w, w_ld, w_grp_stride, row_tab, Cog, Cout_total, o, s);
    }
    return launch_conv<64, 1, 4, PADDED>(g, w, w_ld, w_grp_stride, row_tab, Cog, Cout_total, o, s);
}

static void fill_geom(ConvGeom& g, const float* x, int n, int cin_total, int cig, int H, int W, int halo, int OH, int OW,
                      int stride, int pt, int pl, int K, const int* tab, const int2* tab2, int phase = 1) {
    g.x = x; g.ktab = tab; g.ktab2 = tab2; g.K = K; g.M = n * OH * OW; g.H = H; g.W = W;
    g.halo = halo;
    g.Wp = phase > 1 ? (W + 2 * halo + phase - 1) / phase : W + 2 * halo;
    g.col_mul = phase > 1 ? 1 : stride;
    g.col_add = phase > 1 ? 0 : halo - pl;
    g.stride = stride; g.pt = pt; g.pl = pl; g.OHW = OH * OW; g.OW = OW;
    g.dOHW = make_fastdiv(g.OHW); g.dOW = make_fastdiv(g.OW);
    const int64_t Pp = (int64_t)(H + 2 * halo) * g.Wp;
    g.img_stride = (int64_t)cin_total * phase * Pp;
    g.grp_stride = (int64_t)cig * phase * Pp;
    g.total = g.img_stride * n;
    g.zero = 0;
}

extern "C" int vl_conv_fwd(const vl_conv_desc* d, const float* x, const float* w, const float* bias, float* y, int n,
                           int relu, vl_stream_t stream) {
    VL_CHECK(d && x && w && y, "vl_conv_fwd: null argument");
    VL_CHECK(n > 0 && (int64_t)n * d->oh * d->ow < (1ll << 31), "vl_conv_fwd: bad batch %d", n);
    ConvGeom g;
    fill_geom(g, x, n, d->cin, d->cig, d->h, d->w, d->x_halo, d->oh, d->ow, d->stride, d->pt, d->pl, d->K, d->ptab_fwd, d->ptab2_fwd,
              d->x_phase > 1 ? d->x_phase : 1);
    VL_CHECK(g.total * 4 < MAX_BUF_BYTES, "vl_conv_fwd: input of %lld elements exceeds the buffer-offset range", (long long)g.total);
    ConvOut o{y, bias, nullptr, relu, d->y_halo, 0, d->oh, d->ow};
    if (d->fwd_padded) return dispatch_conv<true>(g, w, d->cout, d->cog, d->rowtab_fwd, d->cog, d->cout, o, d->wsplit_fwd, (hipStream_t)stream);
    return dispatch_conv<false>(g, w, d->cout, d->cog, d->rowtab_fwd, d->cog, d->cout, o, d->wsplit_fwd, (hipStream_t)stream);
}

__global__ __launch_bounds__(256) void conv_wt_transpose_kernel(const float* __restrict__ w, float* __restrict__ wt, int KH, int KW,
                                                                int cig, int cog, int groups) {
    __shared__ float tile[64][65];
    const int cin = cig * groups, cout = cog * groups;
    const int tci = (cig + 63) / 64, tco = (cog + 63) / 64;
    int b = blockIdx.x;
    const int co0 = (b % tco) * 64; b /= tco;
    const int ci0 = (b % tci) * 64; b /= tci;
    const int g = b % groups;       b /= groups;
    const int kx = b % KW, ky = b / KW;
    const int lx = threadIdx.x & 63, ly = threadIdx.x >> 6;
    const float* src = w + ((int64_t)(ky * KW + kx) * cig) * cout + g * cog;
    for (int r = ly; r < 64; r += 4) {
        const int ci = ci0 + r, co = co0 + lx;
        if (ci < cig && co < cog) tile[r][lx] = src[(int64_t)ci * cout + co];
    }
    __syncthreads();
    float* dst = wt + ((int64_t)((KH - 1 - ky) * KW + (KW - 1 - kx)) * cog) * cin + g * cig;
    for (int r = ly; r < 64; r += 4) {
        const int co = co0 + r, ci = ci0 + lx;
        if (co < cog && ci < cig) dst[(int64_t)co * cin + ci] = tile[lx][r];
    }
}

extern "C" int vl_conv_wt_transpose(const vl_conv_desc* d, const float* w, float* wt, vl_stream_t stream) {
    VL_CHECK(d && w && wt, "vl_conv_wt_transpose: null argument");
    const int blocks = d->kh * d->kw * d->groups * ((d->cig + 63) / 64) * ((d->cog + 63) / 64);
    hipLaunchKernelGGL(conv_wt_transpose_kernel, dim3(blocks), dim3(256), 0, (hipStream_t)stream, w, wt, d->kh, d->kw, d->cig,
                       d->cog, d->groups);
    VL_LAUNCH_CHECK();
    return 0;
}

extern "C" int vl_conv_dgrad(const vl_conv_desc* d, const float* dy, const float* wt, float* dx, const float* relu_mask,
                             int n, vl_stream_t stream) {
    VL_CHECK(d && dy && wt && dx, "vl_conv_dgrad: null argument");
    VL_CHECK(d->stride == 1, "vl_conv_dgrad: only stride-1 layers (conv1 needs no input gradient)");
    VL_CHECK(n > 0 && (int64_t)n * d->h * d->w < (1ll << 31), "vl_conv_dgrad: bad batch %d", n);
    ConvGeom g;
    fill_geom(g, dy, n, d->cout, d->cog, d->oh, d->ow, d->dy_halo, d->h, d->w, 1, d->kh - 1 - d->pt, d->kw - 1 - d->pl, d->Kd,
              d->ptab_bwd, d->ptab2_bwd);
    VL_CHECK(g.total * 4 < MAX_BUF_BYTES, "vl_conv_dgrad: dy of %lld elements exceeds the buffer-offset range", (long long)g.total);
    ConvOut o{dx, nullptr, relu_mask, 0, d->dx_halo, d->x_halo, d->h, d->w};
    if (d->bwd_padded) return dispatch_conv<true>(g, wt, d->cin, d->cig, d->rowtab_bwd, d->cig, d->cin, o, d->wsplit_bwd, (hipStream_t)stream);
    return dispatch_conv<false>(g, wt, d->cin, d->cig, d->rowtab_bwd, d->cig, d->cin, o, d->wsplit_bwd, (hipStream_t)stream);
}

static void dy_params(const vl_conv_desc* d, const ConvGeom& g, const float* dy, DyParams& pb) {
    pb.dy = dy; pb.M = g.M; pb.OHW = g.OHW; pb.OW = g.OW; pb.Cog = d->cog; pb.Cout_total = d->cout; pb.halo = d->dy_halo;
    pb.OWp = d->ow + 2 * d->dy_halo; pb.dOHW = g.dOHW; pb.dOW = g.dOW;
    pb.plane = (int64_t)(d->oh + 2 * d->dy_halo) * pb.OWp;
    pb.total = (int64_t)d->cout * pb.plane * (g.M / g.OHW);
    pb.zero = 0;
}

static int reduce_wgrad(const vl_conv_desc* d, float* dw, const float* ws, int splits, hipStream_t s) {
    const int64_t slab = (int64_t)d->K * d->cout;
    if (splits > 1) {
        launch_reduce_slabs(s, ws, dw, slab, splits, slab, nullptr, 0, 0, 0, nullptr);
        VL_LAUNCH_CHECK();
    }
    return 0;
}

template <int BN, int WM, int WN>
static int launch_wgrad(const vl_conv_desc* d, const ConvGeom& g, const float* dy, float* dw, float* ws, int splits,
                        hipStream_t s) {
    constexpr int BM = 128, BR = 32;
    using LA = WgradGather<BM, BR, false>;
    using LB = DyRows<BN, BR>;
    DyParams pb;
    dy_params(d, g, dy, pb);
    const int64_t slab = (int64_t)d->K * d->cout;
    EpiRowMajor::Params pe{splits > 1 ? ws : dw, d->cout, d->K, d->cog, nullptr, nullptr, 0, d->cog, splits > 1 ? slab : 0};
    const int tiles_i = ceil_div(d->K, BM), tiles_j = ceil_div(d->cog, BN);
    const int rtiles = ceil_div(g.M, BR);
    dim3 grid(tiles_i * tiles_j, d->groups, splits);
    hipLaunchKernelGGL((mfma_contract<BM, BN, BR, WM, WN, LA, LB, EpiRowMajor>), grid, dim3(NT), 0, s, g, pb, pe, tiles_i, rtiles,
                       ceil_div(rtiles, splits));
    VL_LAUNCH_CHECK();
    return reduce_wgrad(d, dw, ws, splits, s);
}

template <int BN, int WM, int WN>
static int launch_wgrad_dma(const vl_conv_desc* d, const ConvGeom& g, const float* dy, float* dw, float* db, float* ws, int splits,
                            hipStream_t s) {
    using C = WgradDmaCfg<BN>;
    DyParams pb;
    dy_params(d, g, dy, pb);
    const int64_t slab = (int64_t)d->K * d->cout;
    EpiRowMajor::Params pe{splits > 1 ? ws : dw, d->cout, d->K, d->cog, nullptr, nullptr, 0, d->cog, splits > 1 ? slab : 0};
    const int tiles_i = ceil_div(d->K, C::BM), tiles_j = ceil_div(d->cog, BN);
    const int rtiles = ceil_div(g.M, C::BR);
    static bool attr_set[8] = {false, false, false, false, false, false, false, false};
    int v = g_conv_math == 6 ? 3 : g_conv_math == 3 ? 2 : g_conv_math == 1 ? 1 : 0;
    auto kern = v == 3 ? wgrad_dma_kernel<BN, WM, WN, 6> : v == 2 ? wgrad_dma_kernel<BN, WM, WN, 3>
              : v == 1 ? wgrad_dma_kernel<BN, WM, WN, 1> : wgrad_dma_kernel<BN, WM, WN, 0>;
    if constexpr (BN == 128) {
        if (v != 0 && g.OW % 4 == 0 && g.col_mul == 1 && !kWgradDword) {
            kern = v == 3 ? wgrad_dma_kernel<BN, WM, WN, 6, true> : v == 2 ? wgrad_dma_kernel<BN, WM, WN, 3, true> : wgrad_dma_kernel<BN, WM, WN, 1, true>;
            v += 4;
        }
    }
    if (!attr_set[v]) {
        VL_HIP(hipFuncSetAttribute(reinterpret_cast<const void*>(kern), hipFuncAttributeMaxDynamicSharedMemorySize, (int)C::LDS_BYTES));
        attr_set[v] = true;
    }
    float* db_slabs = db ? (splits > 1 ? ws + (int64_t)splits * slab : db) : nullptr;
    const int units = d->groups * splits;
    dim3 grid((unsigned)(ceil_div(units, 8) * 8 * tiles_i * tiles_j), 1, 1);
    hipLaunchKernelGGL(kern, grid, dim3(NT), C::LDS_BYTES, s, g, pb, pe, tiles_i, tiles_j, d->groups, units, rtiles,
                       ceil_div(rtiles, splits), db_slabs, d->cout);
    VL_LAUNCH_CHECK();
    if (db && splits > 1) {
        launch_reduce_slabs(s, db_slabs, db, (int64_t)d->cout, splits, (int64_t)d->cout, nullptr, 0, 0, 0, nullptr);
        VL_LAUNCH_CHECK();
    }
    return reduce_wgrad(d, dw, ws, splits, s);
}

static int device_cus() {
    static int cus = 0;
    if (!cus) {
        int dev = 0;
        hipDeviceProp_t p;
        if (hipGetDevice(&dev) == hipSuccess && hipGetDeviceProperties(&p, dev) == hipSuccess) cus = p.multiProcessorCount;
        if (cus <= 0) cus = 256;
    }
    return cus;
}

static int wgrad_splits(const vl_conv_desc* d, int n) {
    const int64_t M = (int64_t)n * d->oh * d->ow;
    const int tiles = ceil_div(d->K, 128) * ceil_div(d->cog, d->cog % 128 == 0 ? 128 : 96) * d->groups;
    if (!d->fwd_padded) {
        const int rtiles = ceil_div(M, 32);
        int splits = ceil_div(2048, tiles);
        return splits > rtiles ? rtiles : (splits < 1 ? 1 : splits);
    }
    const int rtiles = ceil_div(M, 64);
    static const int forced = vl_exp_env("VL_WGRAD_SPLITS") ? atoi(vl_exp_env("VL_WGRAD_SPLITS")) : 0;
    if (forced >= 1 && forced <= rtiles) return forced;
    const int per_xcd = device_cus() / 8 > 0 ? device_cus() / 8 : 1;
    const int64_t slab_bytes = ((int64_t)d->K + 1) * d->cout * 4;
    int best = 1;
    int64_t best_cost = -1;
    for (int s = 1; s <= rtiles && s <= 4096; ++s) {
        if (s > 1 && slab_bytes * s > (512ll << 20)) break;
        const bool balanced = ((int64_t)d->groups * s) % 8 == 0;
        const int64_t wgs_xcd = (int64_t)ceil_div((int64_t)d->groups * s, 8) * (tiles / d->groups);
        const int64_t cost = (int64_t)ceil_div(wgs_xcd, per_xcd) * (ceil_div(rtiles, s) + 2) + (balanced ? 0 : 1);
        if (best_cost < 0 || cost < best_cost) {
            best_cost = cost;
            best = s;
        }
    }
    return best;
}

extern "C" size_t vl_conv_wgrad_ws_bytes(const vl_conv_desc* d, int n) {
    if (!d || n <= 0) return 0;
    return (size_t)wgrad_splits(d, n) * ((size_t)d->K + 1) * d->cout * sizeof(float);
}

extern "C" int vl_conv_wgrad_fuses_bias(const vl_conv_desc* d) { return d && d->fwd_padded && d->K % 128 != 0 ? 1 : 0; }

extern "C" int vl_conv_wgrad(const vl_conv_desc* d, const float* x, const float* dy, float* dw, float* db, void* ws,
                             size_t ws_bytes, int n, vl_stream_t stream) {
    VL_CHECK(d && x && dy && dw, "vl_conv_wgrad: null argument");
    VL_CHECK(!db || vl_conv_wgrad_fuses_bias(d), "vl_conv_wgrad: no fused bias gradient for this layer (see vl_conv_wgrad_fuses_bias)");
    VL_CHECK(n > 0 && (int64_t)n * d->oh * d->ow < (1ll << 31), "vl_conv_wgrad: bad batch %d", n);
    const int splits = wgrad_splits(d, n);
    VL_CHECK(splits == 1 || (ws && ws_bytes >= vl_conv_wgrad_ws_bytes(d, n)), "vl_conv_wgrad: workspace too small (%zu < %zu)",
             ws_bytes, vl_conv_wgrad_ws_bytes(d, n));
    ConvGeom g;
    fill_geom(g, x, n, d->cin, d->cig, d->h, d->w, d->x_halo, d->oh, d->ow, d->stride, d->pt, d->pl, d->K, d->ktab_fwd, d->ktab2_fwd,
              d->x_phase > 1 ? d->x_phase : 1);
    const int64_t dy_total = (int64_t)n * d->cout * (d->oh + 2 * d->dy_halo) * (d->ow + 2 * d->dy_halo);
    VL_CHECK(g.total * 4 < MAX_BUF_BYTES && dy_total * 4 < MAX_BUF_BYTES, "vl_conv_wgrad: operand exceeds the buffer-offset range");
    hipStream_t s = (hipStream_t)stream;
    if (d->cog % 128 == 0) {
        if (d->fwd_padded) return launch_wgrad_dma<128, 2, 2>(d, g, dy, dw, db, (float*)ws, splits, s);
        return launch_wgrad<128, 2, 2>(d, g, dy, dw, (float*)ws, splits, s);
    }
    if (d->fwd_padded) return launch_wgrad_dma<96, 4, 1>(d, g, dy, dw, db, (float*)ws, splits, s);
    return launch_wgrad<96, 4, 1>(d, g, dy, dw, (float*)ws, splits, s);
}

template <int BM, int WM, int WN, class LA, class LB>
static int launch_gemm(int m, int n, int k, const float* a, int64_t lda, const float* b, int64_t ldb, float* c, int64_t ldc,
                       const float* bias, int relu, const float* mask, float* ws, int splits, hipStream_t s) {
    constexpr int BN = 128, BR = 16;
    typename LA::Params pa{a, lda, m, k, 0};
    typename LB::Params pb{b, ldb, n, k, 0};
    const int tiles_i = ceil_div(m, BM), tiles_j = ceil_div(n, BN);
    const int rtiles = ceil_div(k, BR);
    const int per = ceil_div(rtiles, splits);
    EpiRowMajor::Params pe;
    if (splits > 1)
        pe = EpiRowMajor::Params{ws, n, m, n, nullptr, nullptr, 0, 0, (int64_t)m * n};
    else
        pe = EpiRowMajor::Params{c, ldc, m, n, bias, mask, relu, 0, 0};
    dim3 grid(tiles_i * tiles_j, 1, splits);
    hipLaunchKernelGGL((mfma_contract<BM, BN, BR, WM, WN, LA, LB, EpiRowMajor>), grid, dim3(NT), 0, s, pa, pb, pe, tiles_i, rtiles, per);
    VL_LAUNCH_CHECK();
    if (splits > 1) {
        const int64_t cnt = (int64_t)m * n;
        launch_reduce_slabs(s, ws, c, cnt, splits, cnt, bias, n, ldc, relu, mask);
        VL_LAUNCH_CHECK();
    }
    return 0;
}

template <int BM, int WM, int WN>
static int dispatch_gemm_t(int ta, int tb, int m, int n, int k, const float* a, int64_t lda, const float* b, int64_t ldb,
                           float* c, int64_t ldc, const float* bias, int relu, const float* mask, float* ws, int splits,
                           hipStream_t s) {
    constexpr int BN = 128, BR = 16;
    if (!ta && !tb) return launch_gemm<BM, WM, WN, DenseXK<BM, BR>, DenseKX<BN, BR>>(m, n, k, a, lda, b, ldb, c, ldc, bias, relu, mask, ws, splits, s);
    if (!ta && tb) return launch_gemm<BM, WM, WN, DenseXK<BM, BR>, DenseXK<BN, BR>>(m, n, k, a, lda, b, ldb, c, ldc, bias, relu, mask, ws, splits, s);
    if (ta && !tb) return launch_gemm<BM, WM, WN, DenseKX<BM, BR>, DenseKX<BN, BR>>(m, n, k, a, lda, b, ldb, c, ldc, bias, relu, mask, ws, splits, s);
    return launch_gemm<BM, WM, WN, DenseKX<BM, BR>, DenseXK<BN, BR>>(m, n, k, a, lda, b, ldb, c, ldc, bias, relu, mask, ws, splits, s);
}

__global__ void gemm_split_image_kernel(const float* __restrict__ x, int64_t sk, int64_t sr, int K, int R, int Rp, int planes,
                                        uint32_t* __restrict__ out) {
    const int st = blockIdx.y;
    uint32_t* o = out + (int64_t)st * planes * 8 * Rp;
    const int r0 = blockIdx.x * 64;
    if (sk == 1) {
        const int rr = threadIdx.x >> 2, kq = threadIdx.x & 3, r = r0 + rr, k0 = st * 16 + 4 * kq;
        float v[4] = {0.f, 0.f, 0.f, 0.f};
        if (r < R) {
#pragma unroll
            for (int e = 0; e < 4; ++e)
                if (k0 + e < K) v[e] = x[(int64_t)r * sr + k0 + e];
        }
        const int h = kq >> 1;
#pragma unroll
        for (int e = 0; e < 2; ++e) {
            int pc[3] = {0, 0, 0};
            split_pieces<3>(v[2 * e], v[2 * e + 1], pc);
            const int q = (kq & 1) * 2 + e;
            for (int pl = 0; pl < planes; ++pl) o[(int64_t)((2 * pl + h) * Rp + r) * 4 + q] = (uint32_t)pc[pl];
        }
    } else {
        for (int idx = threadIdx.x; idx < 8 * 64; idx += blockDim.x) {
            const int rr = idx & 63, hq = idx >> 6, h = hq >> 2, q = hq & 3, r = r0 + rr, k = st * 16 + 8 * h + 2 * q;
            float x0 = 0.f, x1 = 0.f;
            if (r < R) {
                if (k < K) x0 = x[(int64_t)k * sk + r];
                if (k + 1 < K) x1 = x[(int64_t)(k + 1) * sk + r];
            }
            int pc[3] = {0, 0, 0};
            split_pieces<3>(x0, x1, pc);
            for (int pl = 0; pl < planes; ++pl) o[(int64_t)((2 * pl + h) * Rp + r) * 4 + q] = (uint32_t)pc[pl];
        }
    }
}

struct GemmSplitParams {
    const uint32_t* ia;
    const uint32_t* ib;
    int Mp, Np, nstages, stages_per_split;
    float* c;
    int64_t ldc, slab_stride;
    const float* bias;
    const float* mask;
    int relu, m, n, splits;
};

template <int MATH>
__global__ __launch_bounds__(256, MATH == 6 ? 1 : 2) void gemm_split_kernel(const GemmSplitParams P) {
    constexpr int BM = 128, BN = 256, NBUF = 3, D = 3, TA = 4, TB = 2;
    constexpr int NP = split_products(MATH), NPC = split_pieces_of(MATH), NPL = MATH == 6 ? 3 : 2;
    constexpr int APC = NPL * 2 * 2, BPC = NPL * 2 * 4;
    constexpr int ABUF = APC * 256, BUF = (APC + BPC) * 256;
    constexpr int FA = APC / 4, FB = BPC / 4, FW = FA + FB;
    constexpr int NM = TA * TB * NP;
    static_assert(NM >= FW, "a fetch rides on each of the first FW MFMAs");
    extern __shared__ __attribute__((aligned(16))) float ldsg[];
    const int tiles_i = P.Mp / BM;
    const int bid = xcd_swizzle(blockIdx.x, gridDim.x);
    const int i0 = (bid % tiles_i) * BM, j0 = (bid / tiles_i) * BN;
    const int zs = blockIdx.z;
    const int lane = threadIdx.x & 63;
    const int wave = __builtin_amdgcn_readfirstlane(threadIdx.x >> 6);
    const int s_begin = zs * P.stages_per_split;
    const int nst = min(P.nstages, s_begin + P.stages_per_split) - s_begin;

    const int64_t sdw_a = (int64_t)NPL * 8 * P.Mp, sdw_b = (int64_t)NPL * 8 * P.Np;
    const i32x4 rs_a = rsrc_words(reinterpret_cast<const float*>(P.ia), P.nstages * sdw_a * 4);
    const i32x4 rs_b = rsrc_words(reinterpret_cast<const float*>(P.ib), P.nstages * sdw_b * 4);
    uint32_t voff[FW];
#pragma unroll
    for (int f = 0; f < FA; ++f) {
        const int p = wave * FA + f;
        voff[f] = (uint32_t)(((p >> 1) * P.Mp + i0 + (p & 1) * 64 + lane) * 16);
    }
#pragma unroll
    for (int f = 0; f < FB; ++f) {
        const int p = wave * FB + f;
        voff[FA + f] = (uint32_t)(((p >> 2) * P.Np + j0 + (p & 3) * 64 + lane) * 16);
    }
    const uint32_t lds0 = (uint32_t)(uintptr_t)(__attribute__((address_space(3))) float*)ldsg;
    const int sb_a = (int)(sdw_a * 4), sb_b = (int)(sdw_b * 4);
    auto dma = [&](const uint32_t wr, const int f, int st) __attribute__((always_inline)) {
        if (f < FA) lds_dma_row4(rs_a, lds0 + wr + (uint32_t)(wave * FA + f) * 1024u, voff[f], st * sb_a);
        else lds_dma_row4(rs_b, lds0 + wr + (uint32_t)(ABUF * 4 + (wave * FB + f - FA) * 1024), voff[f], st * sb_b);
    };

    f32x16 acc[TA][TB];
#pragma unroll
    for (int a = 0; a < TA; ++a)
#pragma unroll
        for (int b = 0; b < TB; ++b)
#pragma unroll
            for (int q = 0; q < 16; ++q) acc[a][b][q] = 0.f;

    const float* fa = ldsg + ((lane >> 5) * BM + (lane & 31)) * 4;
    const float* fb = ldsg + ABUF + ((lane >> 5) * BN + wave * 64 + (lane & 31)) * 4;
    auto load_ops = [&](int rd, SplitBf16 (&A)[TA], SplitBf16 (&B)[TB]) __attribute__((always_inline)) {
#pragma unroll
        for (int k = 0; k < NPC; ++k) {
#pragma unroll
            for (int a = 0; a < TA; ++a) A[a].p[k] = *reinterpret_cast<const i32x4*>(fa + rd + k * 2 * BM * 4 + a * 32 * 4);
#pragma unroll
            for (int b = 0; b < TB; ++b) B[b].p[k] = *reinterpret_cast<const i32x4*>(fb + rd + k * 2 * BN * 4 + b * 32 * 4);
        }
    };

    for (int s0 = 0; s0 < NBUF; ++s0) {
        if (s0 < nst) {
#pragma unroll
            for (int f = 0; f < FW; ++f) dma((uint32_t)(s0 * BUF * 4), f, s_begin + s0);
        }
    }
    if (nst >= NBUF) asm volatile("s_waitcnt vmcnt(%0)" ::"n"(2 * FW) : "memory");
    else asm volatile("s_waitcnt vmcnt(0)" ::: "memory");
    __syncthreads();
    SplitBf16 A[TA] = {}, B[TB] = {}, An[TA] = {}, Bn[TB] = {};
    load_ops(0, A, B);
    if (nst >= NBUF) asm volatile("s_waitcnt vmcnt(%0) lgkmcnt(0)" ::"n"(FW) : "memory");
    else asm volatile("s_waitcnt vmcnt(0) lgkmcnt(0)" ::: "memory");
    __syncthreads();

    int rd = BUF;
    uint32_t wr = 0;
// ... 130 lines not shown
```

### video-learning-tf_amd/ops.py

```python
import ctypes as C

import torch

from . import _ffi

F32 = torch.float32


def stream():
    return torch.cuda.current_stream().cuda_stream


def _p(t):
    return None if t is None else t.data_ptr()


def _f32(*ts):
    for t in ts:
        if t is None:
            continue
        if not (t.is_cuda and t.dtype == F32):
            raise _ffi.VltfError("expected a CUDA/HIP float32 tensor, got %s on %s" % (t.dtype, t.device))


# ... 304 lines not shown

def lrn_pool_fwd(x, p, argmax, p_halo=0, radius=2, alpha=2e-5, beta=0.75, bias=1.0):
    _f32(x, p); _dense(x, p, argmax)
    n, c, h, w = x.shape
    want = (n, c, pool_out(h) + 2 * p_halo, pool_out(w) + 2 * p_halo)
    if tuple(p.shape) != want or tuple(argmax.shape) != want:
        raise _ffi.VltfError("lrn_pool_fwd: shape mismatch x=%s p=%s argmax=%s" % (tuple(x.shape), tuple(p.shape), tuple(argmax.shape)))
    _ffi.call("vl_lrn_pool_fwd", _p(x), _p(p), _p(argmax), n, c, h, w, p_halo, radius, alpha, beta, bias, stream())


def _x_or_packed(x, c):
    if x.dtype == torch.bfloat16:
        if x.dim() != 5 or x.shape[4] != 8 or c is None or x.shape[1] != (c + 7) // 8 or not x.is_contiguous():
            raise _ffi.VltfError("packed pool input must be a contiguous bf16 [n][c/8][h][w][8] tensor and needs channels=")
        return 1, x.shape[0], x.shape[2], x.shape[3]
    _f32(x)
    return 0, x.shape[0], x.shape[2], x.shape[3]


def lrn_pool_fwd_c8(x, pb, argmax, p_halo=0, radius=2, alpha=2e-5, beta=0.75, bias=1.0, channels=None):
    _dense(x, pb, argmax)
    c = channels if channels is not None else x.shape[1]
    packed, n, h, w = _x_or_packed(x, c)
    oh, ow = pool_out(h), pool_out(w)
    if pb.dtype != torch.bfloat16 or tuple(pb.shape) != c8_shape(n, c, oh, ow, p_halo) or \
            tuple(argmax.shape) != (n, c, oh + 2 * p_halo, ow + 2 * p_halo):
        raise _ffi.VltfError("lrn_pool_fwd_c8: shape mismatch x=%s pb=%s argmax=%s" % (tuple(x.shape), tuple(pb.shape), tuple(argmax.shape)))
    _ffi.call("vl_lrn_pool_fwd_c8", _p(x), packed, _p(pb), _p(argmax), n, c, h, w, p_halo, radius, alpha, beta, bias, stream())


def pool_lrn_bwd(x, dp, argmax, dx, p_halo=0, dx_halo=0, radius=2, alpha=2e-5, beta=0.75, bias=1.0, relu_fused=True):
    _f32(x, dp, dx); _dense(x, dp, argmax, dx)
    n, c, h, w = x.shape
    oh, ow = pool_out(h), pool_out(w)
    if tuple(dp.shape) != (n, c, oh + 2 * p_halo, ow + 2 * p_halo) or tuple(argmax.shape) != tuple(dp.shape) or \
            tuple(dx.shape) != (n, c, h + 2 * dx_halo, w + 2 * dx_halo):
        raise _ffi.VltfError("pool_lrn_bwd: shape mismatch x=%s dp=%s dx=%s" % (tuple(x.shape), tuple(dp.shape), tuple(dx.shape)))
    _ffi.call("vl_pool_lrn_bwd", _p(x), _p(dp), _p(argmax), _p(dx), n, c, h, w, p_halo, radius, alpha, beta, bias, int(relu_fused),
              dx_halo, stream())


def pool_lrn_bwd_test_ranges(ranges=0):
    _ffi.call("vl_pool_lrn_bwd_test_ranges", int(ranges))


def pool_lrn_bwd_c8(x, dp, argmax, dxb, p_halo=0, dxb_halo=0, radius=2, alpha=2e-5, beta=0.75, bias=1.0, relu_fused=True):
    _f32(dp); _dense(x, dp, argmax, dxb)
    c = dp.shape[1]
    packed, n, h, w = _x_or_packed(x, c)
    oh, ow = pool_out(h), pool_out(w)
    if tuple(dp.shape) != (n, c, oh + 2 * p_halo, ow + 2 * p_halo) or tuple(argmax.shape) != tuple(dp.shape) or \
            dxb.dtype != torch.bfloat16 or tuple(dxb.shape) != c8_shape(n, c, h, w, dxb_halo):
        raise _ffi.VltfError("pool_lrn_bwd_c8: shape mismatch x=%s dp=%s dxb=%s" % (tuple(x.shape), tuple(dp.shape), tuple(dxb.shape)))
    _ffi.call("vl_pool_lrn_bwd_c8", _p(x), packed, _p(dp), _p(argmax), _p(dxb), n, c, h, w, p_halo, radius, alpha, beta, bias, int(relu_fused),
              dxb_halo, stream())


def gemm(a, b, c, m, n, k, transa=False, transb=False, lda=None, ldb=None, ldc=None, bias=None, relu=False,
         relu_mask=None, ws=None):
    _f32(a, b, c, bias, relu_mask)
    lda = lda if lda is not None else (m if transa else k)
    ldb = ldb if ldb is not None else (k if transb else n)
    ldc = ldc if ldc is not None else n
    nbytes = 0 if ws is None else ws.numel() * ws.element_size()
    _ffi.call("vl_gemm", int(transa), int(transb), m, n, k, _p(a), lda, _p(b), ldb, _p(c), ldc, _p(bias), int(relu),
              _p(relu_mask), _p(ws), nbytes, stream())


def gemm_split_ws_bytes(m, n, k):
    return int(_ffi.lib().vl_gemm_split_ws_bytes(int(m), int(n), int(k)))


def colsum(a, out, ws, m, n, lda=None):
    _f32(a, out, ws)
    if ws.numel() < 64 * n:
        raise _ffi.VltfError("colsum: workspace needs 64*n floats")
    _ffi.call("vl_colsum", _p(a), lda if lda is not None else n, _p(out), _p(ws), m, n, stream())


def lstm_step_fwd(gx, gh, act, cseq, hseq, hprev, batch, T, t, H, forget_bias=1.0):
    _f32(gx, gh, act, cseq, hseq, hprev)
    _ffi.call("vl_lstm_step_fwd", _p(gx), _p(gh), _p(act), _p(cseq), _p(hseq), _p(hprev), batch, T, t, H, forget_bias,
              stream())


def lstm_step_bwd(dout, dh_next, act, cseq, dc, dz, batch, T, t, H):
    _f32(dout, dh_next, act, cseq, dc, dz)
    _ffi.call("vl_lstm_step_bwd", _p(dout), _p(dh_next), _p(act), _p(cseq), _p(dc), _p(dz), batch, T, t, H, stream())


def lstm_seq_ws(batch, T, H, device):
    n = int(_ffi.lib().vl_lstm_seq_ws_bytes(int(batch), int(T), int(H)))
    return torch.zeros((n + 3) // 4, dtype=torch.float32, device=device)


def _seq_len(seq_len, batch, what):
    if not (torch.is_tensor(seq_len) and seq_len.dtype == torch.int32 and seq_len.is_cuda and seq_len.is_contiguous()
            and seq_len.numel() >= batch):
        raise _ffi.VltfError("%s: seq_len must be a contiguous int32 device tensor of at least %d entries" % (what, batch))
    return seq_len


def lstm_seq_fwd(gx, kh, act, cseq, hseq, hprev, batch, T, H, forget_bias=1.0, ws=None, h0=None, c0=None, seq_len=None):
    _f32(gx, kh, act, cseq, hseq, hprev, h0, c0, ws)
    if ws is None:
        raise _ffi.VltfError("lstm_seq_fwd: a workspace from lstm_seq_ws() is required")
    if seq_len is not None:
        _ffi.call("vl_lstm_seq_fwd_len", _p(gx), _p(kh), _p(h0), _p(c0), _p(act), _p(cseq), _p(hseq), _p(hprev), batch, T, H,
                  forget_bias, _p(_seq_len(seq_len, batch, "lstm_seq_fwd")), _p(ws), ws.numel() * 4, stream())
        return
    _ffi.call("vl_lstm_seq_fwd", _p(gx), _p(kh), _p(h0), _p(c0), _p(act), _p(cseq), _p(hseq), _p(hprev), batch, T, H, forget_bias,
              _p(ws), ws.numel() * 4, stream())


def lstm_seq_bwd(dout, kh, act, cseq, dz, batch, T, H, ws=None, c0=None, dh0=None, dc0=None, seq_len=None):
    _f32(dout, kh, act, cseq, dz, c0, dh0, dc0, ws)
    if ws is None:
        raise _ffi.VltfError("lstm_seq_bwd: a workspace from lstm_seq_ws() is required")
    if seq_len is not None:
        _ffi.call("vl_lstm_seq_bwd_len", _p(dout), _p(kh), _p(act), _p(cseq), _p(c0), _p(dz), _p(dh0), _p(dc0), batch, T, H,
                  _p(_seq_len(seq_len, batch, "lstm_seq_bwd")), _p(ws), ws.numel() * 4, stream())
        return
    _ffi.call("vl_lstm_seq_bwd", _p(dout), _p(kh), _p(act), _p(cseq), _p(c0), _p(dz), _p(dh0), _p(dc0), batch, T, H, _p(ws),
              ws.numel() * 4, stream())


def lstm_seq_tag_span(batch, T, H):
    return int(_ffi.lib().vl_lstm_seq_tag_span(int(batch), int(T), int(H)))


def lstm_seq_fwd_st(gx, kh, act, cseq, hseq, hprev, batch, T, H, forget_bias=1.0, ws=None, state=None, tag_offset=0, h0=None, c0=None):
    _f32(gx, kh, act, cseq, hseq, hprev, h0, c0, ws)
    if ws is None or state is None:
        raise _ffi.VltfError("lstm_seq_fwd_st: a workspace from lstm_seq_ws() and a step state are required")
    _ffi.call("vl_lstm_seq_fwd_st", _p(gx), _p(kh), _p(h0), _p(c0), _p(act), _p(cseq), _p(hseq), _p(hprev), batch, T, H, forget_bias,
              _p(ws), ws.numel() * 4, _state(state), int(tag_offset), stream())


def lstm_seq_bwd_st(dout, kh, act, cseq, dz, batch, T, H, ws=None, state=None, tag_offset=0, c0=None, dh0=None, dc0=None):
    _f32(dout, kh, act, cseq, dz, c0, dh0, dc0, ws)
    if ws is None or state is None:
        raise _ffi.VltfError("lstm_seq_bwd_st: a workspace from lstm_seq_ws() and a step state are required")
    _ffi.call("vl_lstm_seq_bwd_st", _p(dout), _p(kh), _p(act), _p(cseq), _p(c0), _p(dz), _p(dh0), _p(dc0), batch, T, H, _p(ws),
              ws.numel() * 4, _state(state), int(tag_offset), stream())


def lstm_seq_ws_clear(ws):
    _f32(ws)
    _ffi.call("vl_lstm_seq_ws_clear", _p(ws), ws.numel() * 4, stream())


def lstm_seq_timed_out(ws):
    v = C.c_int(0)
    _ffi.call("vl_lstm_seq_status", _p(ws), C.byref(v))
    return bool(v.value)


def lstm_seq_check(*workspaces):
    bad = [i for i, ws in enumerate(workspaces) if ws is not None and lstm_seq_timed_out(ws)]
    if bad:
        raise _ffi.VltfError("LSTM cluster kernel timed out waiting for its peer workgroups (workspace %s): the recurrence needs "
                             "every workgroup resident at once and another kernel was holding compute units; this step's results "
                             "are invalid" % bad)


def lstm_seq_test_hooks(spin_limit=0, mute_workgroup=-1):
    _ffi.call("vl_lstm_seq_test_hooks", int(spin_limit), int(mute_workgroup))


def transpose(src, dst, rows, cols, ld=None):
    _f32(src, dst)
    _ffi.call("vl_transpose", _p(src), ld if ld is not None else cols, _p(dst), rows, cols, stream())


FUSION_CODE = {"avg": 0, "last": 1}


def temporal_fusion_fwd(x, y, batch, T, H, method, seq_len=None):
    _f32(x, y)
    if seq_len is not None:
        _ffi.call("vl_temporal_fusion_fwd_len", _p(x), _p(y), batch, T, H, FUSION_CODE[method],
                  _p(_seq_len(seq_len, batch, "temporal_fusion_fwd")), stream())
        return
    _ffi.call("vl_temporal_fusion_fwd", _p(x), _p(y), batch, T, H, FUSION_CODE[method], stream())


def temporal_fusion_bwd(dy, dx, batch, T, H, method, seq_len=None):
    _f32(dy, dx)
    if seq_len is not None:
        _ffi.call("vl_temporal_fusion_bwd_len", _p(dy), _p(dx), batch, T, H, FUSION_CODE[method],
                  _p(_seq_len(seq_len, batch, "temporal_fusion_bwd")), stream())
        return
    _ffi.call("vl_temporal_fusion_bwd", _p(dy), _p(dx), batch, T, H, FUSION_CODE[method], stream())


def dropout_fwd(x, y, mask, keep, seed):
    _f32(x, y)
    _ffi.call("vl_dropout_fwd", _p(x), _p(y), _p(mask), x.numel(), keep, seed, stream())


def dropout_fwd_st(x, y, mask, keep, state):
    _f32(x, y)
    _ffi.call("vl_dropout_fwd_st", _p(x), _p(y), _p(mask), x.numel(), keep, _state(state), stream())


def dropout_bwd(dy, mask, dx, keep):
    _f32(dy, dx)
    _ffi.call("vl_dropout_bwd", _p(dy), _p(mask), _p(dx), dy.numel(), keep, stream())


def softmax_xent(logits, labels, dlogits, stats, grad_scale, rows=None, seq_len=None, T=None):
    _f32(logits, dlogits, stats); _dense(logits, labels, dlogits)
    if labels.dtype != torch.int32:
        raise _ffi.VltfError("softmax_xent: labels must be int32 one-hot")
    b, c = logits.shape
    if rows is not None:
        _f32(rows)
        if rows.numel() < 2 * b:
            raise _ffi.VltfError("softmax_xent: rows workspace needs 2*batch floats")
    if seq_len is not None:
        if not T or T < 1 or b % int(T):
            raise _ffi.VltfError("softmax_xent: seq_len needs T with rows = clips * T (rows %d, T %s)" % (b, T))
        _ffi.call("vl_softmax_xent_len", _p(logits), _p(labels), _p(dlogits), _p(stats), _p(rows), b, c, grad_scale,
                  _p(_seq_len(seq_len, b // int(T), "softmax_xent")), int(T), stream())
        return
    _ffi.call("vl_softmax_xent", _p(logits), _p(labels), _p(dlogits), _p(stats), _p(rows), b, c, grad_scale, stream())


def sumsq(g, out, ws, accumulate=False):
    _f32(g, out, ws)
    if ws.numel() < 1024:
        raise _ffi.VltfError("sumsq: workspace needs 1024 floats")
    _ffi.call("vl_sumsq", _p(g), g.numel(), _p(out), _p(ws), int(accumulate), stream())


def _skip_word(skip):
    if skip is not None and not (skip.is_cuda and skip.dtype == torch.int32 and skip.numel() >= 1):
        raise _ffi.VltfError("skip must be a CUDA/HIP int32 tensor (one word)")
    return _p(skip)


def sgd_apply(w, g, lr, clip_norm=0.0, sumsq_t=None, gscale=1.0, skip=None):
    _f32(w, g, sumsq_t)
    _ffi.call("vl_sgd_apply", _p(w), _p(g), w.numel(), lr, clip_norm, _p(sumsq_t), gscale, _skip_word(skip), stream())


def adam_apply(w, g, m, v, lr, step, clip_norm=0.0, sumsq_t=None, gscale=1.0, skip=None):
    _f32(w, g, m, v, sumsq_t)
    _ffi.call("vl_adam_apply", _p(w), _p(g), _p(m), _p(v), w.numel(), lr, clip_norm, _p(sumsq_t), gscale, step, _skip_word(skip), stream())


def step_state(device):
    n = int(_ffi.lib().vl_step_state_bytes())
    return torch.zeros((n + 3) // 4, dtype=torch.int32, device=device)


def _state(state):
    if state is None or not (state.is_cuda and state.dtype == torch.int32 and state.numel() * 4 >= int(_ffi.lib().vl_step_state_bytes())):
        raise _ffi.VltfError("expected a step state from step_state()")
    return _p(state)


def step_state_set(state, step, lr, tag_origin):
    _ffi.call("vl_step_state_set", _state(state), int(step), lr, int(tag_origin), stream())


def sgd_apply_st(w, g, state, clip_norm=0.0, sumsq_t=None, gscale=1.0, skip=None):
    _f32(w, g, sumsq_t)
    _ffi.call("vl_sgd_apply_st", _p(w), _p(g), w.numel(), _state(state), clip_norm, _p(sumsq_t), gscale, _skip_word(skip), stream())


def adam_apply_st(w, g, m, v, state, clip_norm=0.0, sumsq_t=None, gscale=1.0, skip=None):
    _f32(w, g, m, v, sumsq_t)
    _ffi.call("vl_adam_apply_st", _p(w), _p(g), _p(m), _p(v), w.numel(), _state(state), clip_norm, _p(sumsq_t), gscale, _skip_word(skip),
              stream())


def step_guard(skip, *lstm_workspaces):
    _skip_word(skip)
    first = True
    for ws in lstm_workspaces:
        if ws is not None:
            _ffi.call("vl_status_or", _p(skip), _p(ws), int(first), stream())
            first = False
    return skip


def fill(t, value):
    _f32(t)
    _ffi.call("vl_fill", _p(t), t.numel(), value, stream())


CONV_MATH = {"f32": 0, "bf16": 1, "bf16x3": 3, "bf16x6": 6}


def set_conv_math(name):
    if name not in CONV_MATH:
        raise _ffi.VltfError("conv math must be one of %s, not %r" % (sorted(CONV_MATH), name))
    _ffi.call("vl_set_conv_math", CONV_MATH[name])


def conv_math():
    return {v: k for k, v in CONV_MATH.items()}[int(_ffi.lib().vl_conv_math())]


def relu_grad(d, y, count=None):
    _f32(d, y); _dense(d, y)
    _ffi.call("vl_relu_grad", _p(d), _p(y), d.numel() if count is None else int(count), stream())


def copy2d(src, dst, rows, cols, src_ld=None, dst_ld=None):
    _f32(src, dst)
    _ffi.call("vl_copy2d", _p(src), cols if src_ld is None else int(src_ld), _p(dst), cols if dst_ld is None else int(dst_ld),
              int(rows), int(cols), stream())


ELTWISE_OP = {"add": 0, "avg": 1, "maximum": 2}


def eltwise2(a, b, out, op, count=None):
    _f32(a, b, out)
    _ffi.call("vl_eltwise2", _p(a), _p(b), _p(out), a.numel() if count is None else int(count), ELTWISE_OP[op], stream())


def max2_grad(a, b, d, da, db, count=None):
    _f32(a, b, d, da, db)
    _ffi.call("vl_max2_grad", _p(a), _p(b), _p(d), _p(da), _p(db), a.numel() if count is None else int(count), stream())


FUSE_OP = {"avg": 0, "maximum": 1}


def _ptr_list(ts):
    arr = (C.c_void_p * len(ts))()
    for i, t in enumerate(ts):
        arr[i] = None if t is None else t.data_ptr()
    return arr


def fuse_n(ins, out, method, count=None):
    _f32(out, *ins)
    if not 1 <= len(ins) <= 8:
        raise _ffi.VltfError("fuse_n: 1..8 inputs, got %d" % len(ins))
    _ffi.call("vl_fuse_n", _ptr_list(ins), len(ins), _p(out), ins[0].numel() if count is None else int(count), FUSE_OP[method], stream())


def fuse_n_grad(ins, d, dins, method, count=None):
    _f32(d, *[t for t in list(ins) + list(dins) if t is not None])
    if len(ins) != len(dins) or not 1 <= len(ins) <= 8:
        raise _ffi.VltfError("fuse_n_grad: 1..8 inputs and as many gradient slots")
    _ffi.call("vl_fuse_n_grad", _ptr_list(ins), len(ins), _p(d), _ptr_list(dins), d.numel() if count is None else int(count),
              FUSE_OP[method], stream())


class Resize:

    def __init__(self, h, w, oh, ow):
        self.h, self.w, self.oh, self.ow = int(h), int(w), int(oh), int(ow)
        self._d = C.c_void_p()
        _ffi.check(_ffi.lib().vl_resize_create(C.byref(self._d), self.h, self.w, self.oh, self.ow, 3), "vl_resize_create")
        self._tmp = None

    def __del__(self):
        try:
            if self._d:
                _ffi.lib().vl_resize_destroy(self._d)
                self._d = None
        except Exception:
            pass

    def tmp_bytes(self, n):
        return int(_ffi.lib().vl_resize_tmp_bytes(self._d, int(n)))

    def __call__(self, src, dst=None, tmp=None):
        if src.dtype != torch.uint8 or not src.is_cuda or not src.is_contiguous() or tuple(src.shape[1:]) != (self.h, self.w, 3):
            raise _ffi.VltfError("resize: expected contiguous device uint8 [n, %d, %d, 3], got %s" % (self.h, self.w, tuple(src.shape)))
        n = src.shape[0]
        if dst is None:
            dst = torch.empty((n, self.oh, self.ow, 3), dtype=torch.uint8, device=src.device)
        elif dst.dtype != torch.uint8 or tuple(dst.shape) != (n, self.oh, self.ow, 3) or not dst.is_contiguous():
            raise _ffi.VltfError("resize: destination must be contiguous uint8 %s" % ((n, self.oh, self.ow, 3),))
        need = self.tmp_bytes(n)
        if need and tmp is not None:
            if tmp.dtype != torch.uint8 or not tmp.is_cuda or tmp.numel() < need:
                raise _ffi.VltfError("resize: tmp must be a device uint8 tensor of >= %d bytes" % need)
        elif need:
            if self._tmp is None or self._tmp.numel() < need:
                self._tmp = torch.empty(need, dtype=torch.uint8, device=src.device)
            tmp = self._tmp
        _ffi.call("vl_resize_u8", self._d, _p(src), _p(tmp) if need else None, _p(dst), n, stream())
        return dst
```

Baseline: 1871 clips/s.

## Split conv output rows into padding classes with trimmed K tables

```diff
diff --git a/include/vltf.h b/include/vltf.h
--- a/include/vltf.h
+++ b/include/vltf.h
@@ -37,6 +37,7 @@
 int vl_conv_x_phase(const vl_conv_desc* d);
 int vl_set_conv_math(int math);
 int vl_conv_math(void);
+int vl_conv_set_row_classes(int on);
 int vl_conv_fwd(const vl_conv_desc* d, const float* x, const float* w_hwio, const float* bias, float* y,
                 int n, int relu, vl_stream_t stream);
 int vl_conv_wt_transpose(const vl_conv_desc* d, const float* w_hwio, float* wt, vl_stream_t stream);
diff --git a/video-learning-tf_amd/_ffi.py b/video-learning-tf_amd/_ffi.py
--- a/video-learning-tf_amd/_ffi.py
+++ b/video-learning-tf_amd/_ffi.py
@@ -22,6 +22,7 @@
     "vl_conv_x_phase": (i32, [p]),
     "vl_set_conv_math": (i32, [i32]),
     "vl_conv_math": (i32, []),
+    "vl_conv_set_row_classes": (i32, [i32]),
     "vl_gemm_split_ws_bytes": (C.c_size_t, [i32, i32, i32]),
     "vl_conv_fwd": (i32, [p, p, p, p, p, i32, i32, p]),
     "vl_conv_wt_transpose": (i32, [p, p, p, p]),
diff --git a/video-learning-tf_amd/csrc/conv_desc.h b/video-learning-tf_amd/csrc/conv_desc.h
--- a/video-learning-tf_amd/csrc/conv_desc.h
+++ b/video-learning-tf_amd/csrc/conv_desc.h
@@ -1,6 +1,15 @@
 #pragma once
 #include <hip/hip_runtime.h>
 #include <stdint.h>
+
+struct vl_conv_rowcls {
+    int ncls;
+    int oh0[5];
+    int rows[5];
+    int K[5];
+    int tab0[5];
+    int rt0[5];
+};
 
 struct vl_conv_desc {
     int cin, h, w, cout, kh, kw, stride, groups;
@@ -19,6 +28,7 @@
     int* rowtab_fwd;
     int* rowtab_bwd;
     int fwd_padded, bwd_padded;
+    vl_conv_rowcls rc_fwd, rc_bwd;
     uint32_t* wsplit_fwd;
     uint32_t* wsplit_bwd;
     int* c8_toff_fwd;
diff --git a/video-learning-tf_amd/csrc/mfma_gemm.hip b/video-learning-tf_amd/csrc/mfma_gemm.hip
--- a/video-learning-tf_amd/csrc/mfma_gemm.hip
+++ b/video-learning-tf_amd/csrc/mfma_gemm.hip
@@ -893,8 +893,58 @@
     int nblk;
 };
 
+struct ConvRowClasses {
+    int ncls;
+    int wg0[6];
+    int S[5];
+    int oh0[5], RW[5];
+    FastDiv dRW[5];
+    int K[5], tab0[5], rt0[5];
+};
+
+struct ConvTile {
+    int bid;
+    int S, oh0, RW;
+    FastDiv dRW;
+    int K, nblk;
+    const int* ktab;
+    const int* row_tab;
+};
+
+__device__ __forceinline__ ConvTile conv_pick_tile(const ConvRowClasses& rc, const ConvGeom& g, const ConvDmaParams& pa) {
+    const int id = blockIdx.x;
+    int w0 = 0, w1 = rc.wg0[1], S = rc.S[0], oh0 = rc.oh0[0], RW = rc.RW[0], K = rc.K[0], tab0 = rc.tab0[0], rt0 = rc.rt0[0];
+    FastDiv dRW = rc.dRW[0];
+#pragma unroll
+    for (int c = 1; c < 5; ++c) {
+        if (c < rc.ncls && id >= rc.wg0[c]) {
+            w0 = rc.wg0[c]; w1 = rc.wg0[c + 1]; S = rc.S[c]; oh0 = rc.oh0[c]; RW = rc.RW[c]; K = rc.K[c]; tab0 = rc.tab0[c]; rt0 = rc.rt0[c];
+            dRW = rc.dRW[c];
+        }
+    }
+    ConvTile t;
+    t.bid = xcd_swizzle(id - w0, w1 - w0);
+    t.S = S; t.oh0 = oh0; t.RW = RW; t.dRW = dRW; t.K = K; t.nblk = (K + KBLK - 1) / KBLK;
+    t.ktab = g.ktab + tab0;
+    t.row_tab = pa.row_tab + rt0;
+    return t;
+}
+
+struct ConvPixel {
+    uint32_t n, p, oh, ow;
+};
+__device__ __forceinline__ ConvPixel conv_tile_pixel(const ConvTile& t, uint32_t m, const FastDiv& dOW, int OW) {
+    ConvPixel q;
+    q.n = fd_div(m, t.dRW);
+    q.p = m - q.n * t.RW;
+    const uint32_t r = fd_div(q.p, dOW);
+    q.ow = q.p - r * OW;
+    q.oh = r + t.oh0;
+    return q;
+}
+
 template <int SR>
-__global__ __launch_bounds__(NT, 64 / SR) void conv_dma_kernel(const ConvDmaParams pa, const ConvGeom g, const EpiConvNCHW::Params pe,
+__global__ __launch_bounds__(NT, 64 / SR) void conv_dma_kernel(const ConvDmaParams pa, const ConvGeom g, const EpiConvNCHW::Params pe, const ConvRowClasses rc,
                                                                int tiles_i, int wide) {
     constexpr int BM = 128, BN = 128;
     constexpr int ABUF = SR * BM, BUF = SR * (BM + BN);
@@ -904,8 +954,8 @@
     constexpr int FPM = 1;
     static_assert(SR == 64 || SR == 32, "stage depth");
     extern __shared__ __attribute__((aligned(16))) float ldsc[];
-    const int bid = xcd_swizzle(blockIdx.x, gridDim.x);
-    const int ti_blk = bid % tiles_i, tj_blk = bid / tiles_i;
+    const ConvTile tl = conv_pick_tile(rc, g, pa);
+    const int ti_blk = tl.bid % tiles_i, tj_blk = tl.bid / tiles_i;
     const int zg = blockIdx.y;
     const int i0 = ti_blk * BM, j0 = tj_blk * BN;
     const int lane = threadIdx.x & 63;
@@ -920,14 +970,10 @@
         const int co = i0 + hf * 64 + lane;
         voff_a[hf] = co < pe.Cog ? (uint32_t)co * 4u : OOB_OFF;
         const int m = j0 + hf * 64 + lane;
-        const bool vm = m < g.M;
-        const uint32_t mm = vm ? m : 0;
-        const uint32_t n = fd_div(mm, g.dOHW);
-        const uint32_t p = mm - n * g.OHW;
-        const uint32_t oh = fd_div(p, g.dOW);
-        const uint32_t ow = p - oh * g.OW;
-        const int ih0 = (int)oh * g.stride - g.pt + g.halo, iw0 = (int)ow * g.col_mul + g.col_add;
-        voff_b[hf] = vm ? (uint32_t)((int64_t)n * g.img_stride + (int64_t)ih0 * g.Wp + iw0) * 4u : OOB_OFF;
+        const bool vm = m < tl.S;
+        const ConvPixel q = conv_tile_pixel(tl, vm ? m : 0, g.dOW, g.OW);
+        const int ih0 = (int)q.oh * g.stride - g.pt + g.halo, iw0 = (int)q.ow * g.col_mul + g.col_add;
+        voff_b[hf] = vm ? (uint32_t)((int64_t)q.n * g.img_stride + (int64_t)ih0 * g.Wp + iw0) * 4u : OOB_OFF;
     }
     const uint32_t lds0 = (uint32_t)(uintptr_t)(__attribute__((address_space(3))) float*)ldsc;
     const int ld_bytes = (int)(pa.w_ld * 4);
@@ -938,11 +984,11 @@
     const int wrow = wave * RW;
     auto load_table = [&](int st) {
         const int k0 = st * SR + wrow;
-        const const_int_ptr tt = as_const(g.ktab) + k0 + st * g.zero;
+        const const_int_ptr tt = as_const(tl.ktab) + k0 + st * g.zero;
 #pragma unroll
         for (int f = 0; f < RW; ++f) tabv[f] = tt[f];
-        row0 = as_const(pa.row_tab)[k0 / KBLK + st * g.zero] + k0 % KBLK;
-        blk_ok = k0 / KBLK < pa.nblk;
+        row0 = as_const(tl.row_tab)[k0 / KBLK + st * g.zero] + k0 % KBLK;
+        blk_ok = k0 / KBLK < tl.nblk;
     };
     auto pin_table = [&]() {
 #pragma unroll
@@ -953,7 +999,7 @@
         const int rr = f >> 2, kind = f & 3, hf = kind & 1;
         const int z = st * g.zero;
         const uint32_t row_lds = lds0 + (uint32_t)(nb * BUF + (wrow + rr) * 128 + hf * 64 + z) * 4u;
-        const bool live = blk_ok && st * SR + wrow + rr < g.K;
+        const bool live = blk_ok && st * SR + wrow + rr < tl.K;
         if (kind < 2) lds_dma_row(rs_w, row_lds, voff_a[hf], min(row0 + rr, g.K - 1) * ld_bytes);
         else lds_dma_row(rs_x, row_lds + ABUF * 4u, live ? voff_b[hf] : OOB_OFF, tabv[rr]);
     };
@@ -979,7 +1025,7 @@
 #pragma unroll
             for (int q = 0; q < 16; ++q) acc[a][b][q] = 0.f;
 
-    const int nstages = (pa.nblk * KBLK + SR - 1) / SR;
+    const int nstages = (tl.nblk * KBLK + SR - 1) / SR;
     load_table(0);
     pin_table();
 #pragma unroll
@@ -1050,7 +1096,7 @@
         }
         finish_stage();
     };
-    const int nfull = g.K / SR;
+    const int nfull = tl.K / SR;
     int st = 0;
     for (; st + 2 < nfull; st += 2) {
         stage(0, true, st + 1);
@@ -1078,10 +1124,10 @@
         __syncthreads();
         const int px = 4 * (lane & 31);
         const int m = j0 + px;
-        const uint32_t n = fd_div((uint32_t)min(m, pe.M - 1), pe.dOHW);
-        const int p = m - (int)n * pe.OHW;
-        const bool run4 = m + 3 < pe.M && p + 3 < pe.OHW;
-        const int64_t cbase = ((int64_t)n * pe.Cout_total + (int64_t)zg * pe.Cog) * pe.y_plane + p;
+        const uint32_t n = fd_div((uint32_t)min(m, tl.S - 1), tl.dRW);
+        const int p = m - (int)n * tl.RW;
+        const bool run4 = m + 3 < tl.S && p + 3 < tl.RW; 
+        const int64_t cbase = ((int64_t)n * pe.Cout_total + (int64_t)zg * pe.Cog) * pe.y_plane + tl.oh0 * pe.OW + p;
 #pragma unroll
         for (int i = 0; i < BM / 8; ++i) {
             const int cl = wave * (BM / 4) + 2 * i + (lane >> 5);
@@ -1095,9 +1141,9 @@
 #pragma unroll
                 for (int e = 0; e < 4; ++e) {
                     const int me = m + e;
-                    if (me < pe.M) {
-                        const uint32_t ne = fd_div((uint32_t)me, pe.dOHW);
-                        const int pe_ = me - (int)ne * pe.OHW;
+                    if (me < tl.S) {
+                        const uint32_t ne = fd_div((uint32_t)me, tl.dRW);
+                        const int pe_ = me - (int)ne * tl.RW + tl.oh0 * pe.OW;
                         pe.y[((int64_t)ne * pe.Cout_total + (int64_t)zg * pe.Cog + co) * pe.y_plane + pe_] = v[e];
                     }
                 }
@@ -1108,14 +1154,11 @@
 #pragma unroll
     for (int b = 0; b < 2; ++b) {
         const int m = j0 + wn * 64 + 32 * b + (lane & 31);
-        if (m >= pe.M) continue;
-        const uint32_t n = fd_div((uint32_t)m, pe.dOHW);
-        const uint32_t p = m - n * pe.OHW;
-        const uint32_t oh = fd_div(p, pe.dOW);
-        const uint32_t ow = p - oh * pe.OW;
-        const int64_t c0 = (int64_t)n * pe.Cout_total + (int64_t)zg * pe.Cog;
-        const int64_t ybase = c0 * pe.y_plane + (int64_t)(oh + pe.y_halo) * pe.y_wp + ow + pe.y_halo;
-        const int64_t mbase = c0 * pe.m_plane + (int64_t)(oh + pe.m_halo) * pe.m_wp + ow + pe.m_halo;
+        if (m >= tl.S) continue;
+        const ConvPixel px = conv_tile_pixel(tl, m, pe.dOW, pe.OW);
+        const int64_t c0 = (int64_t)px.n * pe.Cout_total + (int64_t)zg * pe.Cog;
+        const int64_t ybase = c0 * pe.y_plane + (int64_t)(px.oh + pe.y_halo) * pe.y_wp + px.ow + pe.y_halo;
+        const int64_t mbase = c0 * pe.m_plane + (int64_t)(px.oh + pe.m_halo) * pe.m_wp + px.ow + pe.m_halo;
 #pragma unroll
         for (int a = 0; a < 2; ++a) {
             float mk[16];
@@ -1670,6 +1713,13 @@
 
 extern "C" int vl_conv_math(void) { return g_conv_math; }
 
+static int g_conv_row_classes = 1;
+
+extern "C" int vl_conv_set_row_classes(int on) {
+    g_conv_row_classes = on ? 1 : 0;
+    return 0;
+}
+
 
 static void tf_same_pad(int in, int k, int s, int* out, int* before, int* after) {
     *out = (in + s - 1) / s;
@@ -1707,15 +1757,34 @@
 }
 
 static int build_ktabs(int** dev1, int2** dev2, int** rowtab, int kh, int kw, int cg, int H, int W, int halo, bool permuted,
-                       int phase = 1, int col_shift = 0) {
+                       int phase = 1, int col_shift = 0, vl_conv_rowcls* rc = nullptr, int pt = 0, int OHout = 0) {
     const int K = kh * kw * cg;
     const int pad = ((K + 127) / 128) * 128 + 256;
     const int Wp = phase > 1 ? (W + 2 * halo + phase - 1) / phase : W + 2 * halo;
     const int64_t Pp = (int64_t)(H + 2 * halo) * Wp;
     const int ntiles = pad / KBLK;
-    int* h1 = (int*)malloc(sizeof(int) * pad);
+    int ncls = 0, c_oh0[5], c_rows[5], c_lo[5], c_hi[5];
+    if (rc) {
+        rc->ncls = 0;
+        if (permuted && kh > 1 && phase == 1 && rowtab) {
+            for (int o = 0; o < OHout; ++o) {
+                const int lo = pt - o > 0 ? pt - o : 0, hi = H - 1 + pt - o < kh - 1 ? H - 1 + pt - o : kh - 1;
+                if (lo > hi) { ncls = 0; break; }
+                if (ncls > 0 && c_lo[ncls - 1] == lo && c_hi[ncls - 1] == hi) {
+                    ++c_rows[ncls - 1];
+                } else {
+                    if (ncls == 5) { ncls = 0; break; }
+                    c_oh0[ncls] = o; c_rows[ncls] = 1; c_lo[ncls] = lo; c_hi[ncls] = hi;
+                    ++ncls;
+                }
+            }
+            if (ncls < 2) ncls = 0;
+        }
+    }
+    const int slots = ncls + 1;
+    int* h1 = (int*)calloc((size_t)pad * slots, sizeof(int));
     int2* h2 = (int2*)malloc(sizeof(int2) * pad);
-    int* h3 = (int*)malloc(sizeof(int) * ntiles);
+    int* h3 = (int*)calloc((size_t)ntiles * slots, sizeof(int));
     if (!h1 || !h2 || !h3) {
         free(h1);
         free(h2);
@@ -1739,13 +1808,44 @@
             if (k % KBLK == 0) h3[k / KBLK] = 0;
         }
     }
-    int rc = upload(dev1, h1, pad);
-    if (rc == 0) rc = upload(dev2, h2, pad);
-    if (rc == 0 && rowtab) rc = upload(rowtab, h3, ntiles);
+    size_t n1 = pad, n3 = ntiles;
+    if (ncls) {
+        int order[5];
+        for (int i = 0; i < ncls; ++i) order[i] = i;
+        for (int i = 1; i < ncls; ++i)
+            for (int j = i; j > 0 && c_hi[order[j]] - c_lo[order[j]] > c_hi[order[j - 1]] - c_lo[order[j - 1]]; --j) {
+                const int t = order[j]; order[j] = order[j - 1]; order[j - 1] = t;
+            }
+        for (int i = 0; i < ncls; ++i) {
+            const int c = order[i], Kc = (c_hi[c] - c_lo[c] + 1) * kw * cg;
+            rc->oh0[i] = c_oh0[c]; rc->rows[i] = c_rows[c]; rc->K[i] = Kc;
+            if (Kc == K) {
+                rc->tab0[i] = 0; rc->rt0[i] = 0;
+                continue;
+            }
+            rc->tab0[i] = (int)n1; rc->rt0[i] = (int)n3;
+            int kc = 0;
+            for (int k = 0; k < K; ++k) {
+                int ky, kx, ch;
+                k_to_row(k, kh, kw, cg, true, &ky, &kx, &ch);
+                if (ky < c_lo[c] || ky > c_hi[c]) continue;
+                h1[n1 + kc] = h1[k];
+                if (kc % KBLK == 0) h3[n3 + kc / KBLK] = h3[k / KBLK];
+                ++kc;
+            }
+            n1 += ((Kc + 127) / 128) * 128 + 256;
+            n3 += (((Kc + 127) / 128) * 128 + 256) / KBLK;
+        }
+        rc->ncls = ncls;
+    }
+    int rcode = upload(dev1, h1, n1);
+    if (rcode == 0) rcode = upload(dev2, h2, pad);
+    if (rcode == 0 && rowtab) rcode = upload(rowtab, h3, n3);
+    if (rcode && rc) rc->ncls = 0;
     free(h1);
     free(h2);
     free(h3);
-    return rc;
+    return rcode;
 }
 
 static int rebuild_tables(vl_conv_desc* d) {
@@ -1755,9 +1855,10 @@
     int rc = build_ktabs(&d->ktab_fwd, &d->ktab2_fwd, nullptr, d->kh, d->kw, d->cig, d->h, d->w, d->x_halo, false, ph, shift);
     if (rc == 0)
         rc = build_ktabs(&d->ptab_fwd, &d->ptab2_fwd, &d->rowtab_fwd, d->kh, d->kw, d->cig, d->h, d->w, d->x_halo, d->cig % KBLK == 0, ph,
-                         shift);
+                         shift, d->stride == 1 ? &d->rc_fwd : nullptr, d->pt, d->oh);
     if (rc == 0 && d->stride == 1) {
-        rc = build_ktabs(&d->ptab_bwd, &d->ptab2_bwd, &d->rowtab_bwd, d->kh, d->kw, d->cog, d->oh, d->ow, d->dy_halo, d->cog % KBLK == 0);
+        rc = build_ktabs(&d->ptab_bwd, &d->ptab2_bwd, &d->rowtab_bwd, d->kh, d->kw, d->cog, d->oh, d->ow, d->dy_halo, d->cog % KBLK == 0, 1,
+                         0, &d->rc_bwd, d->kh - 1 - d->pt, d->h);
         const int need = (d->kh - 1 - d->pt > d->pt ? d->kh - 1 - d->pt : d->pt);
         const int needw = (d->kw - 1 - d->pl > d->pl ? d->kw - 1 - d->pl : d->pl);
         d->bwd_padded = d->dy_halo >= need && d->dy_halo >= needw;
@@ -1866,7 +1967,7 @@
 
 
 template <int TA>
-__global__ __launch_bounds__(NT, 2) void conv_dma16_kernel(const ConvDmaParams pa, const ConvGeom g, const EpiConvNCHW::Params pe,
+__global__ __launch_bounds__(NT, 2) void conv_dma16_kernel(const ConvDmaParams pa, const ConvGeom g, const EpiConvNCHW::Params pe, const ConvRowClasses rc,
                                                            int tiles_i, int wide) {
     constexpr int BM = 16 * TA, BN = 128, SR = 32;
     constexpr int NA = (BM + 63) / 64;
@@ -1875,8 +1976,8 @@
     constexpr int RW = SR / 4, FPR = NA + 2, NF = RW * FPR, NSTEP = SR / 4;
     constexpr int NM = 2 * TA;
     extern __shared__ __attribute__((aligned(16))) float ldsc[];
-    const int bid = xcd_swizzle(blockIdx.x, gridDim.x);
-    const int ti_blk = bid % tiles_i, tj_blk = bid / tiles_i;
+    const ConvTile tl = conv_pick_tile(rc, g, pa);
+    const int ti_blk = tl.bid % tiles_i, tj_blk = tl.bid / tiles_i;
     const int zg = blockIdx.y;
     const int i0 = ti_blk * BM, j0 = tj_blk * BN;
     const int lane = threadIdx.x & 63;
@@ -1894,14 +1995,10 @@
 #pragma unroll
     for (int hf = 0; hf < 2; ++hf) {
         const int m = j0 + hf * 64 + lane;
-        const bool vm = m < g.M;
-        const uint32_t mm = vm ? m : 0;
-        const uint32_t n = fd_div(mm, g.dOHW);
-        const uint32_t p = mm - n * g.OHW;
-        const uint32_t oh = fd_div(p, g.dOW);
-        const uint32_t ow = p - oh * g.OW;
-        const int ih0 = (int)oh * g.stride - g.pt + g.halo, iw0 = (int)ow * g.col_mul + g.col_add;
-        voff_b[hf] = vm ? (uint32_t)((int64_t)n * g.img_stride + (int64_t)ih0 * g.Wp + iw0) * 4u : OOB_OFF;
+        const bool vm = m < tl.S;
+        const ConvPixel q = conv_tile_pixel(tl, vm ? m : 0, g.dOW, g.OW);
+        const int ih0 = (int)q.oh * g.stride - g.pt + g.halo, iw0 = (int)q.ow * g.col_mul + g.col_add;
+        voff_b[hf] = vm ? (uint32_t)((int64_t)q.n * g.img_stride + (int64_t)ih0 * g.Wp + iw0) * 4u : OOB_OFF;
     }
     float bias_r[TA][4];
 #pragma unroll
@@ -1920,11 +2017,11 @@
     const int wrow = wave * RW;
     auto load_table = [&](int st) {
         const int k0 = st * SR + wrow;
-        const const_int_ptr tt = as_const(g.ktab) + k0 + st * g.zero;
+        const const_int_ptr tt = as_const(tl.ktab) + k0 + st * g.zero;
 #pragma unroll
         for (int f = 0; f < RW; ++f) tabv[f] = tt[f];
-        row0 = as_const(pa.row_tab)[k0 / KBLK + st * g.zero] + k0 % KBLK;
-        blk_ok = k0 / KBLK < pa.nblk;
+        row0 = as_const(tl.row_tab)[k0 / KBLK + st * g.zero] + k0 % KBLK;
+        blk_ok = k0 / KBLK < tl.nblk;
     };
     auto pin_table = [&]() {
 #pragma unroll
@@ -1934,7 +2031,7 @@
     auto dma = [&](const int nb, const int f, int st) {
         const int rr = f / FPR, kind = f % FPR;
         const int z = st * g.zero;
-        const bool live = blk_ok && st * SR + wrow + rr < g.K;
+        const bool live = blk_ok && st * SR + wrow + rr < tl.K;
         if (kind < NA) {
             lds_dma_row(rs_w, lds0 + (uint32_t)(nb * BUF + (wrow + rr) * SA + kind * 64 + z) * 4u, voff_a[kind],
                         min(row0 + rr, g.K - 1) * ld_bytes);
@@ -1970,7 +2067,7 @@
 #pragma unroll
             for (int q = 0; q < 4; ++q) acc[a][b][q] = 0.f;
 
-    const int nstages = (pa.nblk * KBLK + SR - 1) / SR;
+    const int nstages = (tl.nblk * KBLK + SR - 1) / SR;
     load_table(0);
     pin_table();
 #pragma unroll
@@ -2028,8 +2125,8 @@
         }
         finish_stage();
     };
-    const int nfull = g.K / SR;
-    const int last_steps = (g.K - (nstages - 1) * SR + 3) / 4;
+    const int nfull = tl.K / SR;
+    const int last_steps = (tl.K - (nstages - 1) * SR + 3) / 4;
     int st = 0;
     for (; st + 2 < nfull; st += 2) {
         stage(0, true, st + 1, NSTEP);
@@ -2057,10 +2154,10 @@
         __syncthreads();
         const int px = 4 * (lane & 31);
         const int m = j0 + px;
-        const uint32_t n = fd_div((uint32_t)min(m, pe.M - 1), pe.dOHW);
-        const int p = m - (int)n * pe.OHW;
-        const bool run4 = m + 3 < pe.M && p + 3 < pe.OHW;
-        const int64_t cbase = ((int64_t)n * pe.Cout_total + (int64_t)zg * pe.Cog) * pe.y_plane + p;
+        const uint32_t n = fd_div((uint32_t)min(m, tl.S - 1), tl.dRW);
+        const int p = m - (int)n * tl.RW;
+        const bool run4 = m + 3 < tl.S && p + 3 < tl.RW;
+        const int64_t cbase = ((int64_t)n * pe.Cout_total + (int64_t)zg * pe.Cog) * pe.y_plane + tl.oh0 * pe.OW + p;
 #pragma unroll
         for (int i = 0; i < BM / 8; ++i) {
             const int cl = wave * (BM / 4) + 2 * i + (lane >> 5);
@@ -2074,9 +2171,9 @@
 #pragma unroll
                 for (int e = 0; e < 4; ++e) {
                     const int me = m + e;
-                    if (me < pe.M) {
-                        const uint32_t ne = fd_div((uint32_t)me, pe.dOHW);
-                        const int pe_ = me - (int)ne * pe.OHW;
+                    if (me < tl.S) {
+                        const uint32_t ne = fd_div((uint32_t)me, tl.dRW);
+                        const int pe_ = me - (int)ne * tl.RW + tl.oh0 * pe.OW;
                         pe.y[((int64_t)ne * pe.Cout_total + (int64_t)zg * pe.Cog + co) * pe.y_plane + pe_] = v[e];
                     }
                 }
@@ -2087,14 +2184,11 @@
 #pragma unroll
     for (int b = 0; b < 2; ++b) {
         const int m = j0 + wave * 32 + 16 * b + (lane & 15);
-        if (m >= pe.M) continue;
-        const uint32_t n = fd_div((uint32_t)m, pe.dOHW);
-        const uint32_t p = m - n * pe.OHW;
-        const uint32_t oh = fd_div(p, pe.dOW);
-        const uint32_t ow = p - oh * pe.OW;
-        const int64_t c0 = (int64_t)n * pe.Cout_total + (int64_t)zg * pe.Cog;
-        const int64_t ybase = c0 * pe.y_plane + (int64_t)(oh + pe.y_halo) * pe.y_wp + ow + pe.y_halo;
-        const int64_t mbase = c0 * pe.m_plane + (int64_t)(oh + pe.m_halo) * pe.m_wp + ow + pe.m_halo;
+        if (m >= tl.S) continue;
+        const ConvPixel px = conv_tile_pixel(tl, m, pe.dOW, pe.OW);
+        const int64_t c0 = (int64_t)px.n * pe.Cout_total + (int64_t)zg * pe.Cog;
+        const int64_t ybase = c0 * pe.y_plane + (int64_t)(px.oh + pe.y_halo) * pe.y_wp + px.ow + pe.y_halo;
+        const int64_t mbase = c0 * pe.m_plane + (int64_t)(px.oh + pe.m_halo) * pe.m_wp + px.ow + pe.m_halo;
         float mk[TA][4];
         if (pe.mask) {
 #pragma unroll
@@ -2126,7 +2220,7 @@
 
 template <int BM>
 static int launch_conv_dma(const ConvGeom& g, const float* w, int64_t w_ld, int w_grp_stride, const int* row_tab, int Cog,
-                           int Cout_total, const ConvOut& o, hipStream_t s) {
+                           int Cout_total, const ConvOut& o, hipStream_t s, const vl_conv_rowcls* rcd = nullptr) {
     constexpr int BN = 128, SR = 32;
     constexpr size_t lds = BM == 128 ? (size_t)BM * (BN + 4) * sizeof(float)
                                      : (size_t)2 * SR * ((BM + 63) / 64 * 64 + 16 + 144) * sizeof(float);
@@ -2146,13 +2240,28 @@
         VL_HIP(hipFuncSetAttribute(kern, hipFuncAttributeMaxDynamicSharedMemorySize, (int)lds));
         attr_set = true;
     }
-    const int tiles_i = ceil_div(Cog, BM), tiles_j = ceil_div(g.M, BN);
-    dim3 grid(tiles_i * tiles_j, (unsigned)(Cout_total / Cog), 1);
+    const int tiles_i = ceil_div(Cog, BM);
+    ConvRowClasses rc;
+    memset(&rc, 0, sizeof(rc));
+    if (rcd && rcd->ncls > 1 && g_conv_row_classes) {
+        const int nimg = g.M / g.OHW;
+        rc.ncls = rcd->ncls;
+        for (int c = 0; c < rc.ncls; ++c) {
+            rc.RW[c] = rcd->rows[c] * g.OW; rc.dRW[c] = make_fastdiv(rc.RW[c]); rc.S[c] = nimg * rc.RW[c];
+            rc.oh0[c] = rcd->oh0[c]; rc.K[c] = rcd->K[c]; rc.tab0[c] = rcd->tab0[c]; rc.rt0[c] = rcd->rt0[c];
+            rc.wg0[c + 1] = rc.wg0[c] + tiles_i * ceil_div(rc.S[c], BN);
+        }
+    } else {
+        rc.ncls = 1;
+        rc.RW[0] = g.OHW; rc.dRW[0] = g.dOHW; rc.S[0] = g.M; rc.K[0] = g.K;
+        rc.wg0[1] = tiles_i * ceil_div(g.M, BN);
+    }
+    dim3 grid(rc.wg0[rc.ncls], (unsigned)(Cout_total / Cog), 1);
     const int wide = (o.y_halo == 0 && !o.mask && !kConvNoWideStore && (size_t)BM * (BN + 4) * sizeof(float) <= lds) ? 1 : 0;
     if constexpr (BM == 128) {
-        hipLaunchKernelGGL(conv_dma_kernel<SR>, grid, dim3(NT), lds, s, pa, g, pe, tiles_i, wide);
+        hipLaunchKernelGGL(conv_dma_kernel<SR>, grid, dim3(NT), lds, s, pa, g, pe, rc, tiles_i, wide);
     } else {
-        hipLaunchKernelGGL((conv_dma16_kernel<BM / 16>), grid, dim3(NT), lds, s, pa, g, pe, tiles_i, wide);
+        hipLaunchKernelGGL((conv_dma16_kernel<BM / 16>), grid, dim3(NT), lds, s, pa, g, pe, rc, tiles_i, wide);
     }
     VL_LAUNCH_CHECK();
     return 0;
@@ -2205,7 +2314,7 @@
 
 template <bool PADDED>
 static int dispatch_conv(const ConvGeom& g, const float* w, int64_t w_ld, int w_grp_stride, const int* row_tab, int Cog,
-                         int Cout_total, const ConvOut& o, uint32_t* wsplit, hipStream_t s) {
+                         int Cout_total, const ConvOut& o, uint32_t* wsplit, hipStream_t s, const vl_conv_rowcls* rcd) {
     const int w128 = ceil_div(Cog, 128) * 128, w96 = ceil_div(Cog, 96) * 96, w64 = ceil_div(Cog, 64) * 64;
     if (g_conv_math != 0 && PADDED && g.col_mul == 1 && wsplit != nullptr) {
         if (Cog >= 96) return launch_conv_ring<128>(g, w, w_ld, w_grp_stride, row_tab, Cog, Cout_total, o, wsplit, s);
@@ -2258,16 +2367,16 @@
     }
     if (w128 <= w96 && w128 <= w64) {
         if (PADDED && (int64_t)g.K * w_ld * 4 < MAX_BUF_BYTES && !kConvStaged) {
-            return launch_conv_dma<128>(g, w, w_ld, w_grp_stride, row_tab, Cog, Cout_total, o, s);
+            return launch_conv_dma<128>(g, w, w_ld, w_grp_stride, row_tab, Cog, Cout_total, o, s, rcd);
         }
         return launch_conv<128, 2, 2, PADDED>(g, w, w_ld, w_grp_stride, row_tab, Cog, Cout_total, o, s);
     }
     if (PADDED && ceil_div(Cog, 48) * 48 < w64 && ceil_div(Cog, 48) * 48 < w96 &&
         (int64_t)g.K * w_ld * 4 < MAX_BUF_BYTES && !kConvStaged)
-        return launch_conv_dma<48>(g, w, w_ld, w_grp_stride, row_tab, Cog, Cout_total, o, s);
+        return launch_conv_dma<48>(g, w, w_ld, w_grp_stride, row_tab, Cog, Cout_total, o, s, rcd);
     if (w96 <= w64) {
         if (PADDED && (int64_t)g.K * w_ld * 4 < MAX_BUF_BYTES && !kConvStaged)
-            return launch_conv_dma<96>(g, w, w_ld, w_grp_stride, row_tab, Cog, Cout_total, o, s);
+            return launch_conv_dma<96>(g, w, w_ld, w_grp_stride, row_tab, Cog, Cout_total, o, s, rcd);
         return launch_conv<96, 1, 4, PADDED>(g, w, w_ld, w_grp_stride, row_tab, Cog, Cout_total, o, s);
     }
     return launch_conv<64, 1, 4, PADDED>(g, w, w_ld, w_grp_stride, row_tab, Cog, Cout_total, o, s);
@@ -2298,8 +2407,8 @@
               d->x_phase > 1 ? d->x_phase : 1);
     VL_CHECK(g.total * 4 < MAX_BUF_BYTES, "vl_conv_fwd: input of %lld elements exceeds the buffer-offset range", (long long)g.total);
     ConvOut o{y, bias, nullptr, relu, d->y_halo, 0, d->oh, d->ow};
-    if (d->fwd_padded) return dispatch_conv<true>(g, w, d->cout, d->cog, d->rowtab_fwd, d->cog, d->cout, o, d->wsplit_fwd, (hipStream_t)stream);
-    return dispatch_conv<false>(g, w, d->cout, d->cog, d->rowtab_fwd, d->cog, d->cout, o, d->wsplit_fwd, (hipStream_t)stream);
+    if (d->fwd_padded) return dispatch_conv<true>(g, w, d->cout, d->cog, d->rowtab_fwd, d->cog, d->cout, o, d->wsplit_fwd, (hipStream_t)stream, &d->rc_fwd);
+    return dispatch_conv<false>(g, w, d->cout, d->cog, d->rowtab_fwd, d->cog, d->cout, o, d->wsplit_fwd, (hipStream_t)stream, &d->rc_fwd);
 }
 
 __global__ __launch_bounds__(256) void conv_wt_transpose_kernel(const float* __restrict__ w, float* __restrict__ wt, int KH, int KW,
@@ -2345,8 +2454,8 @@
               d->ptab_bwd, d->ptab2_bwd);
     VL_CHECK(g.total * 4 < MAX_BUF_BYTES, "vl_conv_dgrad: dy of %lld elements exceeds the buffer-offset range", (long long)g.total);
     ConvOut o{dx, nullptr, relu_mask, 0, d->dx_halo, d->x_halo, d->h, d->w};
-    if (d->bwd_padded) return dispatch_conv<true>(g, wt, d->cin, d->cig, d->rowtab_bwd, d->cig, d->cin, o, d->wsplit_bwd, (hipStream_t)stream);
-    return dispatch_conv<false>(g, wt, d->cin, d->cig, d->rowtab_bwd, d->cig, d->cin, o, d->wsplit_bwd, (hipStream_t)stream);
+    if (d->bwd_padded) return dispatch_conv<true>(g, wt, d->cin, d->cig, d->rowtab_bwd, d->cig, d->cin, o, d->wsplit_bwd, (hipStream_t)stream, &d->rc_bwd);
+    return dispatch_conv<false>(g, wt, d->cin, d->cig, d->rowtab_bwd, d->cig, d->cin, o, d->wsplit_bwd, (hipStream_t)stream, &d->rc_bwd);
 }
 
 static void dy_params(const vl_conv_desc* d, const ConvGeom& g, const float* dy, DyParams& pb) {
diff --git a/video-learning-tf_amd/ops.py b/video-learning-tf_amd/ops.py
--- a/video-learning-tf_amd/ops.py
+++ b/video-learning-tf_amd/ops.py
@@ -630,6 +630,10 @@
 
 def conv_math():
     return {v: k for k, v in CONV_MATH.items()}[int(_ffi.lib().vl_conv_math())]
+
+
+def conv_set_row_classes(on=True):
+    _ffi.call("vl_conv_set_row_classes", int(bool(on)))
 
 
 def relu_grad(d, y, count=None):
```

Measured after the change: 1901 clips/s (median of 6 runs). 1.6% higher.
